# chrisquince/DESMAN

Hardware: AMD Instinct MI355X
Metric: Gibbs iterations/sec (VxS updates/s) at V=10k S=64 G=8 (higher is better)
Workload: dtype f64; 1 GPU; synthetic V=10000 x S=64, G=8, full Gibbs iteration, 1 chain per GPU (configs[2]); V=10000, S=64, G=8, chains=1, tau_rng=mt19937

## Files before the change

### desman_amd/_lib.py

```python
import ctypes as C
import os

import numpy as np

_HERE = os.path.dirname(os.path.abspath(__file__))
LIB_PATH = os.environ.get("DESMAN_HIP_LIB") or os.path.join(_HERE, "lib", "libdesman_hip.so")
AB_LIB_PATH = os.path.join(_HERE, "lib", "libdesman_hip_ab.so")
HEADER_PATH = os.path.join(os.path.dirname(_HERE), "include", "desman_hip.h")

DSM_OK = 0
RNG_MT19937, RNG_PHILOX = 0, 1
STATS_AGG = 2
K_NAMES = ("stats", "dirichlet", "tau", "finalize", "mt", "nmft_a", "nmft_gamma", "nmft_b", "stats2", "stats_big", "stats_pat")


class DesmanHipError(RuntimeError):
    pass


_i64p = np.ctypeslib.ndpointer(np.int64, flags="C_CONTIGUOUS")
_f64p = np.ctypeslib.ndpointer(np.float64, flags="C_CONTIGUOUS")
_u64p = np.ctypeslib.ndpointer(np.uint64, flags="C_CONTIGUOUS")
_u32p = np.ctypeslib.ndpointer(np.uint32, flags="C_CONTIGUOUS")
_i32p = np.ctypeslib.ndpointer(np.int32, flags="C_CONTIGUOUS")
_vp, _i, _d = C.c_void_p, C.c_int, C.c_double

SIGNATURES = {
    "dsm_last_error": (C.c_char_p, []),
    "dsm_device_count": (_i, []),
    "dsm_version": (C.c_char_p, []),
    "dsm_initRNG": (_i, []),
    "dsm_setRNG": (_i, [C.c_ulong]),
    "dsm_freeRNG": (_i, []),
    "dsm_sample_tau": (_i, [_i64p, _f64p, _f64p, _i64p, _i, _i, _i]),
    "c_initRNG": (None, []),
    "c_setRNG": (None, [C.c_ulong]),
    "c_freeRNG": (None, []),
    "c_sample_tau": (_i, [_i64p, _f64p, _f64p, _i64p, _i, _i, _i]),
    "dsm_getRNG_state": (_i, [_u32p]),
    "dsm_setRNG_state": (_i, [_u32p]),
    "dsm_ctx_create": (_i, [C.POINTER(_vp), _i]),
    "dsm_ctx_destroy": (_i, [_vp]),
    "dsm_ctx_sync": (_i, [_vp]),
    "dsm_ctx_set_counts": (_i, [_vp, _i64p, _i, _i]),
    "dsm_ctx_set_state": (_i, [_vp, _i64p, _f64p, _f64p, _i]),
    "dsm_ctx_get_state": (_i, [_vp, _vp, _vp, _vp]),
    "dsm_ctx_set_gamma_eta": (_i, [_vp, _vp, _vp]),
    "dsm_ctx_set_priors": (_i, [_vp, _d, _d, _d]),
    "dsm_ctx_seed": (_i, [_vp, C.c_ulong, C.c_uint64]),
    "dsm_ctx_set_tau_rng": (_i, [_vp, _i]),
    "dsm_ctx_get_mt_state": (_i, [_vp, _u32p]),
    "dsm_ctx_set_mt_state": (_i, [_vp, _u32p]),
    "dsm_mt_seed_state": (_i, [C.c_ulong, _u32p]),
    "dsm_ctx_debug_mt_fill": (_i, [_vp, C.c_size_t, _u32p]),
    "dsm_ctx_sample_tau": (_i, [_vp, C.POINTER(_i), _vp]),
    "dsm_ctx_sample_stats": (_i, [_vp, C.c_uint32, _u64p, _u64p]),
    "dsm_ctx_stats_spec": (_i, [_vp]),
    "dsm_ctx_sweep_stats": (_i, [_vp, C.POINTER(C.c_uint64), C.POINTER(C.c_uint64), _i]),
    "dsm_ctx_set_tau_screen": (_i, [_vp, _i]),
    "dsm_ctx_set_tau_neartie": (_i, [_vp, _i]),
    "dsm_ctx_set_nmft_fused": (_i, [_vp, _i]),
    "dsm_ctx_set_nmft_persist": (_i, [_vp, _i]),
    "dsm_ctx_tau_launch_info": (_i, [_vp, C.POINTER(_i), C.POINTER(_i)]),
    "dsm_ctx_debug_log2f": (_i, [_vp, _vp, _vp, C.c_size_t]),
    "dsm_debug_fdiv": (_i, [_i, _f64p, _f64p, _f64p, _i]),
    "dsm_release_device_caches": (_i, []),
    "dsm_ctx_force_stats_spec": (_i, [_vp, _i]),
    "dsm_ctx_debug_stage1": (_i, [_vp, C.c_uint32, _vp, _u64p]),
    "dsm_ctx_debug_binom": (_i, [_vp, _i, C.c_uint32, _f64p, C.c_uint64, _i, _u32p, _i]),
    "dsm_ctx_draw_gamma_eta": (_i, [_vp, C.c_uint32, _u64p, _u64p, _f64p, _f64p]),
    "dsm_ctx_loglik": (_i, [_vp, C.POINTER(_d), C.POINTER(_d)]),
    "dsm_ctx_gibbs_update": (_i, [_vp, _i]),
    "dsm_ctx_get_counters": (_i, [_vp, C.POINTER(C.c_uint64), C.POINTER(C.c_uint32)]),
    "dsm_ctx_set_counters": (_i, [_vp, C.c_uint64, C.c_uint32]),
    "dsm_ctx_get_screen_state": (_i, [_vp, _u32p]),
    "dsm_ctx_set_screen_state": (_i, [_vp, _u32p]),
    "dsm_ctx_gibbs_update_sharded": (_i, [_vp, _i, _i, _i, _vp, _vp]),
    "dsm_ctx_gibbs_update_sharded_comm": (_i, [_vp, _i, _i, _i, _vp]),
    "dsm_comm_unique_id": (_i, [_vp]),
    "dsm_comm_create": (_i, [C.POINTER(_vp), _vp, _i, _i, _i]),
    "dsm_comm_destroy": (_i, [_vp]),
    "dsm_comm_rank": (_i, [_vp]),
    "dsm_comm_world": (_i, [_vp]),
    "dsm_comm_allgather_f64": (_i, [_vp, _f64p, _f64p, C.c_size_t]),
    "dsm_comm_allreduce_f64": (_i, [_vp, _vp, C.c_size_t, _i]),
    "dsm_comm_barrier": (_i, [_vp]),
    "dsm_device_read": (_i, [_i, _vp, _vp, C.c_size_t]),
    "dsm_device_write": (_i, [_i, _vp, _vp, C.c_size_t]),
    "dsm_batch_gibbs_update": (_i, [C.POINTER(_vp), _i, _i]),
    "dsm_batch_update_tau": (_i, [C.POINTER(_vp), _i, _i, C.POINTER(_vp), C.POINTER(_vp)]),
    "dsm_batch_nmft_factorize": (_i, [C.POINTER(_vp), _i, _i, _d, _i, C.POINTER(_i), _vp]),
    "dsm_ctx_update_tau": (_i, [_vp, _i, _f64p, _f64p]),
    "dsm_ctx_get_trace": (_i, [_vp, _vp, _vp, _vp, _vp, _vp]),
    "dsm_ctx_get_star": (_i, [_vp, _vp, _vp, _vp, C.POINTER(_d), C.POINTER(_i)]),
    "dsm_ctx_get_tau_sum": (_i, [_vp, _i64p]),
    "dsm_ctx_get_tau_at": (_i, [_vp, _i, _i64p]),
    "dsm_nmft_set": (_i, [_vp, _f64p, _f64p, _i]),
    "dsm_nmft_get": (_i, [_vp, _vp, _vp]),
    "dsm_nmft_factorize": (_i, [_vp, _i, _d, _i, C.POINTER(_i), _vp]),
    "dsm_nmft_objective": (_i, [_vp, C.POINTER(_d)]),
    "dsm_nmft_debug_path": (_i, [_vp, _i, C.POINTER(_i)]),
    "dsm_nmft_get_tau": (_i, [_vp, _i64p]),
    "dsm_lrt_step": (_i, [_i, _f64p, _i32p, _i32p, _f64p, _d, _i, _i, _f64p, _f64p, _f64p]),
    "dsm_assign_tau": (_i, [_i, _i64p, _i, _i, _i, _f64p, _f64p, C.c_uint64, _vp, _vp, _vp, _vp, _vp]),
    "dsm_ctx_assign_tau": (_i, [_vp, _f64p, _f64p, _i, C.c_uint64, _vp, _vp, _vp, _vp, _vp]),
    "dsm_assign_debug_set_chunk": (_i, [_i]),
    "dsm_fit_gamma": (_i, [_i, _i64p, _i, _i, _i, _i64p, _f64p, _i, _d, _i, _vp, _vp, _vp, _vp, _vp, _vp]),
    "dsm_ctx_fit_gamma": (_i, [_vp, _i, _vp, _f64p, _i, _d, _i, _vp, _vp, _vp, _vp, _vp, _vp]),
    "dsm_abund_debug_set_chunk": (_i, [_i]),
    "dsm_fit_gamma_interval": (_i, [_i, _i64p, _i, _i, _i, _i64p, _f64p, _f64p, _d, _i, _d, _d, _vp, _vp, _vp]),
    "dsm_ctx_fit_gamma_interval": (_i, [_vp, _i, _vp, _f64p, _f64p, _d, _i, _d, _d, _vp, _vp, _vp]),
    "dsm_fit_gamma_eta": (_i, [_i, _i64p, _i, _i, _i, _i64p, _f64p, _i, _d, _vp, _vp, _vp, _vp, _vp, _vp, _vp, _vp, _vp]),
    "dsm_ctx_fit_gamma_eta": (_i, [_vp, _i, _vp, _f64p, _i, _d, _vp, _vp, _vp, _vp, _vp, _vp, _vp, _vp, _vp]),
    "dsm_abund_debug_set_eta_batch": (_i, [_i]),
    "dsm_abund_debug_set_eta_stage_max": (_i, [C.c_longlong]),
    "dsm_genes_create": (_i, [C.POINTER(_vp), _i]),
    "dsm_genes_destroy": (_i, [_vp]),
    "dsm_genes_set_data": (_i, [_vp, _vp, _i, _i, _i, _i32p, _f64p]),
    "dsm_genes_set_model": (_i, [_vp, _f64p, _f64p, _f64p, _i, _i, _f64p, _f64p, _f64p]),
    "dsm_genes_set_state": (_i, [_vp, _vp, _vp]),
    "dsm_genes_get_state": (_i, [_vp, _vp, _vp]),
    "dsm_genes_seed": (_i, [_vp, C.c_ulong, C.c_uint64]),
    "dsm_genes_set_gene_base": (_i, [_vp, _i]),
    "dsm_genes_get_mt_state": (_i, [_vp, _u32p]),
    "dsm_genes_set_mt_state": (_i, [_vp, _u32p]),
    "dsm_genes_nmft_tau": (_i, [_vp, _vp, _f64p, _i, _d, _vp]),
    "dsm_genes_sweep_all": (_i, [_vp, _vp, _i, _vp, _vp, _vp]),
    "dsm_genes_step_candidates": (_i, [_vp, _i, _i, _f64p, _vp]),
    "dsm_genes_step_choose": (_i, [_vp, _i, _i, _i]),
    "dsm_genes_update": (_i, [_vp, _i, _i, _vp, _vp, _vp, _vp]),
    "dsm_genes_loglik": (_i, [_vp, _vp]),
    "dsm_genes_get_star": (_i, [_vp, _vp, _vp]),
    "dsm_genes_set_star": (_i, [_vp, _vp, _vp]),
    "dsm_genes_debug_tile": (_i, [_vp, C.POINTER(_i), C.POINTER(_i), C.POINTER(_i), C.POINTER(C.c_size_t)]),
    "dsm_kl_assign": (_i, [_i, _f64p, _f64p, _f64p, _i, _i, _i, _i, _d, C.POINTER(_i), C.POINTER(_d)]),
    "dsm_ctx_set_timing": (_i, [_vp, _i]),
    "dsm_ctx_get_timing": (_i, [_vp, _vp, _vp]),
    "dsm_kernel_name": (C.c_char_p, [_i]),
}

EXCHANGE_FN = C.CFUNCTYPE(C.c_int, C.c_void_p, C.c_void_p, C.c_size_t, C.c_void_p, C.c_size_t)
_lib = None


def _digest(a):
    try:
        import xxhash
        return xxhash.xxh3_128_digest(memoryview(a).cast("B"))
    except ImportError:
        import hashlib
        return hashlib.blake2b(memoryview(a).cast("B"), digest_size=16).digest()


def load():
    global _lib
    if _lib is None:
        if not os.path.exists(LIB_PATH):
            raise DesmanHipError(
                "libdesman_hip.so not built (%s); run `python -c 'import __graft_entry__ as g; g.build()'` "
                "or `make -C desman_amd/csrc`.  There is no CPU fallback." % LIB_PATH)
        try:
            lib = C.CDLL(LIB_PATH)
        except OSError as e:
            raise DesmanHipError("cannot load %s: %s" % (LIB_PATH, e))
        for name, (res, args) in SIGNATURES.items():
            fn = getattr(lib, name)
            fn.restype = res
            fn.argtypes = args
        _lib = lib
    return _lib


def check(rc):
    if rc != DSM_OK:
        raise DesmanHipError("libdesman_hip: error %d: %s" % (rc, load().dsm_last_error().decode()))
    return rc


def mt_seed_state(seed):
    st = np.empty(625, dtype=np.uint32)
    check(load().dsm_mt_seed_state(int(seed) & 0xFFFFFFFFFFFFFFFF, st))
    return st


def release_device_caches():
    check(load().dsm_release_device_caches())


def debug_fdiv(kind, a, b):
    a = np.ascontiguousarray(a, dtype=np.float64).reshape(-1)
    b = np.ascontiguousarray(b, dtype=np.float64).reshape(-1)
    out = np.empty_like(a)
    check(load().dsm_debug_fdiv(int(kind), a, b, out, a.size))
    return out


def lrt_step(ffreq, maxA, maxB, eta, upperP, optimise, p, device=0):
    ffreq = np.ascontiguousarray(ffreq, dtype=np.float64)
    V = ffreq.shape[0]
    p = np.ascontiguousarray(p, dtype=np.float64).copy()
    MLL = np.empty(V); BLL = np.empty(V)
    check(load().dsm_lrt_step(int(device), ffreq, np.ascontiguousarray(maxA, dtype=np.int32),
                              np.ascontiguousarray(maxB, dtype=np.int32), np.ascontiguousarray(eta, dtype=np.float64),
                              float(upperP), int(bool(optimise)), V, p, MLL, BLL))
    return p, MLL, BLL


def device_count():
    return load().dsm_device_count()


ASSIGN_MAX_G = 10


def _assign_model(gamma, eta, S):
    gamma = np.ascontiguousarray(gamma, dtype=np.float64)
    eta = np.ascontiguousarray(eta, dtype=np.float64)
    if gamma.ndim != 2 or gamma.shape[0] != S or eta.shape != (4, 4):
        raise ValueError("assign_tau: gamma must be [S=%d, G] and eta [4, 4]; got %s, %s" % (S, gamma.shape, eta.shape))
    return gamma, eta
# ... 187 lines not shown
        self.G = gamma.shape[1]

    def get_state(self):
        tau = np.empty((self.V, self.G, 4), dtype=np.int64)
        gamma = np.empty((self.S, self.G))
        eta = np.empty((4, 4))
        check(self.lib.dsm_ctx_get_state(self._h, _ptr(tau), _ptr(gamma), _ptr(eta)))
        return tau, gamma, eta

    def set_gamma_eta(self, gamma=None, eta=None):
        g = None if gamma is None else np.ascontiguousarray(gamma, dtype=np.float64)
        e = None if eta is None else np.ascontiguousarray(eta, dtype=np.float64)
        check(self.lib.dsm_ctx_set_gamma_eta(self._h, _ptr(g), _ptr(e)))

    def set_priors(self, alpha=0.1, delta=0.1, epsilon=1e-6):
        check(self.lib.dsm_ctx_set_priors(self._h, alpha, delta, epsilon))

    def seed(self, mt_seed, ctr_seed=None):
        if ctr_seed is None:
            ctr_seed = (int(mt_seed) * 0x9E3779B97F4A7C15 + 0x243F6A8885A308D3) & 0xFFFFFFFFFFFFFFFF
        check(self.lib.dsm_ctx_seed(self._h, int(mt_seed) & 0xFFFFFFFFFFFFFFFF, int(ctr_seed)))

    def get_mt_state(self):
        st = np.empty(625, dtype=np.uint32)
        check(self.lib.dsm_ctx_get_mt_state(self._h, st))
        return st

    def checkpoint(self):
        tau, gamma, eta = self.get_state()
        key, it = self.counters()
        try:
            mt = self.get_mt_state()
        except DesmanHipError:
            mt = np.zeros(0, dtype=np.uint32)
        return dict(tau=tau, gamma=gamma, eta=eta, mt_state=mt, ctr_seed=np.uint64(key), iter_ctr=np.uint32(it), screen=self.screen_state())

    def counters(self):
        key, it = C.c_uint64(0), C.c_uint32(0)
        check(self.lib.dsm_ctx_get_counters(self._h, C.byref(key), C.byref(it)))
        return int(key.value), int(it.value)

    def screen_state(self):
        out = np.zeros(2, dtype=np.uint32)
        check(self.lib.dsm_ctx_get_screen_state(self._h, out))
        return out

    def set_screen_state(self, words):
        check(self.lib.dsm_ctx_set_screen_state(self._h, np.ascontiguousarray(words, dtype=np.uint32)))

    def restore(self, ck):
        self.set_state(np.ascontiguousarray(ck["tau"], dtype=np.int64), np.ascontiguousarray(ck["gamma"], dtype=np.float64),
                       np.ascontiguousarray(ck["eta"], dtype=np.float64))
        mt = np.asarray(ck["mt_state"], dtype=np.uint32)
        if mt.size == 625:
            self.set_mt_state(np.ascontiguousarray(mt))
        check(self.lib.dsm_ctx_set_counters(self._h, int(ck["ctr_seed"]), int(ck["iter_ctr"])))
        self.set_screen_state(ck["screen"] if "screen" in ck else np.zeros(2, dtype=np.uint32))

    def set_mt_state(self, st):
        check(self.lib.dsm_ctx_set_mt_state(self._h, np.ascontiguousarray(st, dtype=np.uint32)))

    def debug_mt_fill(self, n):
        out = np.empty(int(n), dtype=np.uint32)
        check(self.lib.dsm_ctx_debug_mt_fill(self._h, int(n), out))
        return out

    def set_tau_rng(self, mode):
        check(self.lib.dsm_ctx_set_tau_rng(self._h, int(mode)))

    def assign_tau(self, gamma, eta, seed=None):
        gamma, eta = _assign_model(gamma, eta, self.S)
        G = gamma.shape[1]
        out = _assign_out(self.V, G, seed)
        check(self.lib.dsm_ctx_assign_tau(self._h, gamma, eta, G, int(seed or 0) & 0xFFFFFFFFFFFFFFFF, _ptr(out["map_state"]),
                                          _ptr(out["conf"]), _ptr(out["logz"]), _ptr(out["marg"]), _ptr(out.get("draw_state"))))
        return out

    def fit_gamma(self, eta, tau=None, max_iter=FIT_MAX_ITER, tol=FIT_TOL, presence=False):
        eta = _fit_eta(eta)
        t = None if tau is None else _fit_tau(tau, self.V)
        G = self.G if t is None else t.shape[1]
        out = _fit_out(self.S, G, presence)
        check(self.lib.dsm_ctx_fit_gamma(self._h, G, _ptr(t), eta, int(max_iter), float(tol), int(bool(presence)), _ptr(out["gamma"]),
                                         _ptr(out["loglik"]), _ptr(out["deviance"]), _ptr(out["iters"]), _ptr(out["converged"]),
                                         _ptr(out.get("lr_absent"))))
        return out

    def fit_gamma_eta(self, eta0, tau=None, max_iter=FIT_MAX_ITER, tol=FIT_TOL):
        eta0 = _fit_eta(eta0)
        t = None if tau is None else _fit_tau(tau, self.V)
        G = self.G if t is None else t.shape[1]
        out, scal, ptrs = _fit_eta_out(self.S, G)
        check(self.lib.dsm_ctx_fit_gamma_eta(self._h, G, _ptr(t), eta0, int(max_iter), float(tol), *ptrs))
        return _fit_eta_result(out, scal)

    def fit_gamma_interval(self, eta, gamma_hat, tau=None, level=0.95, q=None, max_iter=FIT_MAX_ITER, tol=FIT_TOL, ctol=FIT_CTOL):
        eta = _fit_eta(eta)
        t = None if tau is None else _fit_tau(tau, self.V)
        G = self.G if t is None else t.shape[1]
        g, q, out = _interval_args(gamma_hat, self.S, G, level, q)
        check(self.lib.dsm_ctx_fit_gamma_interval(self._h, G, _ptr(t), eta, g, q, int(max_iter), float(tol), float(ctol), _ptr(out["lo"]),
                                                  _ptr(out["hi"]), _ptr(out["flags"])))
        return out

    def sample_tau(self, want_logp=False):
        n = _i(0)
        logp = np.empty((self.V, self.G, 4)) if want_logp else None
        check(self.lib.dsm_ctx_sample_tau(self._h, C.byref(n), _ptr(logp)))
        return (n.value, logp) if want_logp else n.value

    def sample_stats(self, it):
        mu = np.zeros((self.S, self.G), dtype=np.uint64)
        E = np.zeros((4, 4), dtype=np.uint64)
        check(self.lib.dsm_ctx_sample_stats(self._h, int(it), mu, E))
        return mu, E

    def debug_log2f(self, x):
        x = np.ascontiguousarray(x, dtype=np.float32)
        out = np.empty_like(x)
        check(self.lib.dsm_ctx_debug_log2f(self._h, x.ctypes.data, out.ctypes.data, x.size))
        return out

    def set_tau_neartie(self, mode=-1):
        check(self.lib.dsm_ctx_set_tau_neartie(self._h, int(mode)))

    def set_tau_screen(self, on):
        check(self.lib.dsm_ctx_set_tau_screen(self._h, 1 if on else 0))

    def tau_launch_info(self):
        a, b = _i(0), _i(0)
        check(self.lib.dsm_ctx_tau_launch_info(self._h, C.byref(a), C.byref(b)))
        return a.value, b.value

    def set_nmft_persist(self, mode=-1):
        check(self.lib.dsm_ctx_set_nmft_persist(self._h, int(mode)))

    def set_nmft_fused(self, mode=-1):
        check(self.lib.dsm_ctx_set_nmft_fused(self._h, int(mode)))

    def sweep_stats(self, reset=False):
        a, b = C.c_uint64(0), C.c_uint64(0)
        check(self.lib.dsm_ctx_sweep_stats(self._h, C.byref(a), C.byref(b), 1 if reset else 0))
        return a.value, b.value

    def stats_spec(self):
        r = self.lib.dsm_ctx_stats_spec(self._h)
        if r < 0:
            check(r)
        return r

    def force_stats_spec(self, spec=0):
        check(self.lib.dsm_ctx_force_stats_spec(self._h, int(spec)))

    def debug_stage1(self, it):
        nt = np.zeros((self.S, 1 << self.G), dtype=np.uint32)
        E = np.zeros((4, 4), dtype=np.uint64)
        check(self.lib.dsm_ctx_debug_stage1(self._h, int(it), nt.ctypes.data, E))
        return nt, E

    def debug_binom(self, kind, n, w, seed, nsamp, spec=STATS_AGG):
        w4 = np.zeros(4)
        w4[:len(w)] = w
        out = np.zeros((nsamp, 4) if kind == 2 else nsamp, dtype=np.uint32)
        check(self.lib.dsm_ctx_debug_binom(self._h, int(kind), int(n), w4, int(seed), int(nsamp), out.reshape(-1), int(spec)))
        return out

    def draw_gamma_eta(self, it, sum_mu, esum):
        g = np.empty((self.S, self.G)); e = np.empty((4, 4))
        check(self.lib.dsm_ctx_draw_gamma_eta(self._h, int(it), np.ascontiguousarray(sum_mu, dtype=np.uint64),
                                              np.ascontiguousarray(esum, dtype=np.uint64), g, e))
        return g, e

    def loglik(self):
        ll, lp = _d(0), _d(0)
        check(self.lib.dsm_ctx_loglik(self._h, C.byref(ll), C.byref(lp)))
        return ll.value, lp.value

    def gibbs_update(self, n_iter):
        check(self.lib.dsm_ctx_gibbs_update(self._h, int(n_iter)))
        self.n_trace = int(n_iter)

    def gibbs_update_sharded(self, n_iter, v_offset, v_total, exchange):
        err = []

        def cb(user, tab, n_tab, vec, n_vec):
            try:
                exchange(tab or 0, int(n_tab), vec, int(n_vec))
                return 0
            except BaseException as e:
                err.append(e)
                return 1
        fn = EXCHANGE_FN(cb)
        rc = self.lib.dsm_ctx_gibbs_update_sharded(self._h, int(n_iter), int(v_offset), int(v_total), C.cast(fn, _vp), None)
        if err:
            raise err[0]
        check(rc)
        self.n_trace = int(n_iter)

    def gibbs_update_sharded_comm(self, n_iter, v_offset, v_total, comm):
        check(self.lib.dsm_ctx_gibbs_update_sharded_comm(self._h, int(n_iter), int(v_offset), int(v_total), comm._h))
        self.n_trace = int(n_iter)

    @staticmethod
    def batch_gibbs_update(ctxs, n_iter):
        ctxs = list(ctxs)
        arr = (_vp * len(ctxs))(*[c._h.value for c in ctxs])
        check(load().dsm_batch_gibbs_update(arr, len(ctxs), int(n_iter)))
        for c in ctxs:
            c.n_trace = int(n_iter)

    def update_tau(self, gamma_store, eta_store):
        g = np.ascontiguousarray(gamma_store, dtype=np.float64)
        e = np.ascontiguousarray(eta_store, dtype=np.float64)
        check(self.lib.dsm_ctx_update_tau(self._h, g.shape[0], g, e))
        self.n_trace = g.shape[0]

    def get_trace(self):
        n = self.n_trace
        ll = np.empty(n); lp = np.empty(n); nch = np.empty(n, dtype=np.int32)
        g = np.empty((n, self.S, self.G)); e = np.empty((n, 4, 4))
        check(self.lib.dsm_ctx_get_trace(self._h, _ptr(ll), _ptr(lp), _ptr(nch), _ptr(g), _ptr(e)))
        return dict(ll=ll, lp=lp, nchange=nch, gamma=g, eta=e)

    def get_star(self):
        tau = np.empty((self.V, self.G, 4), dtype=np.int64)
        g = np.empty((self.S, self.G)); e = np.empty((4, 4))
        lp, it = _d(0), _i(0)
        check(self.lib.dsm_ctx_get_star(self._h, _ptr(tau), _ptr(g), _ptr(e), C.byref(lp), C.byref(it)))
        return dict(tau=tau, gamma=g, eta=e, lp=lp.value, it=it.value)

    def get_tau_sum(self):
        out = np.empty((self.V, self.G, 4), dtype=np.int64)
        check(self.lib.dsm_ctx_get_tau_sum(self._h, out))
        return out

    def get_tau_at(self, it):
        out = np.empty((self.V, self.G, 4), dtype=np.int64)
        check(self.lib.dsm_ctx_get_tau_at(self._h, int(it), out))
        return out

    def nmft_set(self, tau, gamma):
        tau = np.ascontiguousarray(tau, dtype=np.float64)
        gamma = np.ascontiguousarray(gamma, dtype=np.float64)
        G = gamma.shape[0]
        if tau.shape != (4 * self.V, G) or gamma.shape[1] != self.S:
            raise ValueError("NMFT factor shapes do not match the count tensor")
        check(self.lib.dsm_nmft_set(self._h, tau, gamma, G))
        self.nG = G

    def nmft_get(self):
        tau = np.empty((4 * self.V, self.nG)); gamma = np.empty((self.nG, self.S))
        check(self.lib.dsm_nmft_get(self._h, _ptr(tau), _ptr(gamma)))
        return tau, gamma

    def nmft_factorize(self, max_iter=5000, min_change=1e-5, fix_gamma=False):
        n = _i(0)
        tr = np.full(max_iter + 1, np.nan)
        check(self.lib.dsm_nmft_factorize(self._h, int(max_iter), float(min_change), int(bool(fix_gamma)),
                                          C.byref(n), _ptr(tr)))
        return n.value, tr[: n.value + 1]

    @staticmethod
    def batch_update_tau(ctxs, gamma_stores, eta_stores):
        ctxs = list(ctxs)
        gs = [np.ascontiguousarray(g, dtype=np.float64) for g in gamma_stores]
        es = [np.ascontiguousarray(e, dtype=np.float64) for e in eta_stores]
        n = gs[0].shape[0]
        if any(g.shape[0] != n for g in gs) or any(e.shape[0] != n for e in es):
            raise ValueError("batch_update_tau: traces of equal length expected")
        arr = (_vp * len(ctxs))(*[c._h.value for c in ctxs])
        gp = (_vp * len(ctxs))(*[g.ctypes.data for g in gs])
        ep = (_vp * len(ctxs))(*[e.ctypes.data for e in es])
        check(load().dsm_batch_update_tau(arr, len(ctxs), int(n), gp, ep))
        for c in ctxs:
            c.n_trace = int(n)

    @staticmethod
    def batch_nmft_factorize(ctxs, max_iter=5000, min_change=1e-5, fix_gamma=False):
        ctxs = list(ctxs)
        arr = (_vp * len(ctxs))(*[c._h.value for c in ctxs])
        n = (_i * len(ctxs))()
        tr = np.full((len(ctxs), max_iter + 1), np.nan)
        check(load().dsm_batch_nmft_factorize(arr, len(ctxs), int(max_iter), float(min_change), int(bool(fix_gamma)), n,
                                              tr.ctypes.data_as(_vp)))
        return [(int(n[k]), tr[k, : n[k] + 1].copy()) for k in range(len(ctxs))]

    def nmft_objective(self):
        d = _d(0)
        check(self.lib.dsm_nmft_objective(self._h, C.byref(d)))
        return d.value

    def nmft_debug_path(self, fix_gamma=False):
        out = (_i * 8)()
        check(self.lib.dsm_nmft_debug_path(self._h, int(bool(fix_gamma)), out))
        fam, nt, kb, ncb, nwv, grid, lds, flags = (int(x) for x in out)
        return {"family": ("two-pass", "mfma", "split", "persist")[fam], "NT": nt, "KB": kb, "NCB": ncb, "NWV": nwv, "grid": grid,
                "lds": lds, "xpar": bool(flags & 1), "gstep": bool(flags & 2), "VT": (flags >> 8) & 255, "cus": flags >> 16}

    def nmft_get_tau(self):
        out = np.empty((self.V, self.nG, 4), dtype=np.int64)
        check(self.lib.dsm_nmft_get_tau(self._h, out))
        return out

    def set_timing(self, on):
        check(self.lib.dsm_ctx_set_timing(self._h, int(bool(on))))

# ... 134 lines not shown
```

### desman_amd/csrc/api.hip

```cpp
#include <math.h>
#include <stdarg.h>
#include <stdio.h>
#include <string.h>

#include <algorithm>
#include <mutex>
#include <numeric>
#include <thread>

#include "dsm_host.h"
#include "log_table.h"

static thread_local char g_err[512] = "";

void dsm_set_error(const char *fmt, ...)
{
    va_list ap;
    va_start(ap, fmt);
    vsnprintf(g_err, sizeof g_err, fmt, ap);
    va_end(ap);
}

extern "C" const char *dsm_last_error(void) { return g_err; }
extern "C" const char *dsm_version(void) { return "desman_hip 0.1 (gfx950)"; }
// ... 42 lines not shown
        c->k_ms[s.k] += ms;
        c->free_events.push_back(s.e0);
        c->free_events.push_back(s.e1);
    }
    c->spans.clear();
    return DSM_OK;
}

extern "C" int dsm_ctx_set_timing(dsm_ctx *c, int on)
{
    if (!c) return DSM_ERR_ARG;
    int r = collect_spans(c);
    c->timing = on != 0;
    for (int k = 0; k < DSM_K_COUNT; ++k) { c->k_ms[k] = 0; c->k_launches[k] = 0; }
    return r;
}

extern "C" int dsm_ctx_get_timing(dsm_ctx *c, double *ms_total, int64_t *launches)
{
    if (!c) return DSM_ERR_ARG;
    int r = collect_spans(c);
    if (r) return r;
    for (int k = 0; k < DSM_K_COUNT; ++k) {
        if (ms_total) ms_total[k] = c->k_ms[k];
        if (launches) launches[k] = c->k_launches[k];
    }
    return DSM_OK;
}

template <typename T>
static int dev_alloc(T **p, size_t n)
{
    if (*p) { (void)hipFree(*p); *p = nullptr; }
    if (n == 0) n = 1;
    hipError_t e = hipMalloc((void **)p, n * sizeof(T));
    if (e != hipSuccess) { dsm_set_error("hipMalloc(%zu B) failed: %s", n * sizeof(T), hipGetErrorString(e)); return DSM_ERR_NOMEM; }
    return DSM_OK;
}
template <typename T>
static void dev_free(T **p) { if (*p) { (void)hipFree(*p); *p = nullptr; } }

template <typename T>
struct Scratch {
    T *p = nullptr;
    ~Scratch() { if (p) (void)hipFree(p); }
    int alloc(size_t n) { return dev_alloc(&p, n); }
    operator T *() const { return p; }
    Scratch() = default;
    Scratch(const Scratch &) = delete;
    Scratch &operator=(const Scratch &) = delete;
};

#define TRY(x) do { int _r = (x); if (_r != DSM_OK) return _r; } while (0)
#define BIND(c) HIP_TRY(hipSetDevice((c)->device))

static int need(dsm_ctx *c, bool counts, bool state)
{
    if (!c) { dsm_set_error("null context"); return DSM_ERR_ARG; }
    if (counts && !c->cnt_vs) { dsm_set_error("no count tensor: call dsm_ctx_set_counts first"); return DSM_ERR_STATE; }
    if (state && !c->have_state) { dsm_set_error("no chain state: call dsm_ctx_set_state first"); return DSM_ERR_STATE; }
    return DSM_OK;
}

static int esum_reset(dsm_ctx *c)
{
    HIP_TRY(hipMemsetAsync(c->esum, 0, (16 + 16 * DSM_ESUM_PARTS) * sizeof(unsigned long long), c->stream));
    return DSM_OK;
}

static int reset_blk_order(dsm_ctx *c)
{
    static const std::vector<uint32_t> ident = [] { std::vector<uint32_t> v((size_t)2 * DSM_MAX_GRID); for (size_t i = 0; i < v.size(); ++i) v[i] = (uint32_t)(i % DSM_MAX_GRID); return v; }();
    c->blk_order_n[0] = c->blk_order_n[1] = 0;
    if (!c->blk_order) return DSM_OK;
    HIP_TRY(hipMemcpyAsync(c->blk_order, ident.data(), ident.size() * sizeof(uint32_t), hipMemcpyHostToDevice, c->stream));
    return DSM_OK;
}

extern "C" int dsm_ctx_create(dsm_ctx **out, int device)
{
    if (!out) return DSM_ERR_ARG;
    *out = nullptr;
    int n = dsm_device_count();
    if (n <= 0) { dsm_set_error("no HIP device visible"); return DSM_ERR_NODEVICE; }
    if (device < 0 || device >= n) { dsm_set_error("device %d out of range (0..%d)", device, n - 1); return DSM_ERR_ARG; }
    HIP_TRY(hipSetDevice(device));
    hipDeviceProp_t prop;
    HIP_TRY(hipGetDeviceProperties(&prop, device));
    if (strncmp(prop.gcnArchName, "gfx950", 6) != 0) {
        dsm_set_error("device %d is %s; this library is built for gfx950 only", device, prop.gcnArchName);
        return DSM_ERR_NODEVICE;
    }
    dsm_ctx *c = new dsm_ctx();
    c->device = device;
    HIP_TRY(hipStreamCreateWithFlags(&c->stream, hipStreamNonBlocking));
    if (getenv("DESMAN_HIP_ONE_STREAM")) c->stream_rng = c->stream;
    else {
        int lo = 0, hi = 0;
        HIP_TRY(hipDeviceGetStreamPriorityRange(&lo, &hi));
        HIP_TRY(hipStreamCreateWithPriority(&c->stream_rng, hipStreamNonBlocking, hi));
    }
    for (int i = 0; i < 2; ++i) {
        HIP_TRY(hipEventCreateWithFlags(&c->ev_u_ready[i], hipEventDisableTiming));
        HIP_TRY(hipEventCreateWithFlags(&c->ev_u_free[i], hipEventDisableTiming));
    }
    TRY(dev_alloc(&c->mt_state, 625));
    TRY(dev_alloc(&c->ll_partial, 2 * DSM_MAX_GRID));
    TRY(dev_alloc(&c->nchange, 2));
    TRY(dev_alloc(&c->sweep_stats, 2));
    HIP_TRY(hipMemsetAsync(c->sweep_stats, 0, 2 * sizeof(unsigned long long), c->stream));
    TRY(dev_alloc(&c->step_cnt, (size_t)2 * 2 * DSM_MAX_GRID));
    HIP_TRY(hipMemsetAsync(c->step_cnt, 0, (size_t)2 * 2 * DSM_MAX_GRID * sizeof(uint32_t), c->stream));
    TRY(dev_alloc(&c->blk_order, (size_t)2 * DSM_MAX_GRID));
    TRY(reset_blk_order(c));
    TRY(dev_alloc(&c->screen_ctl, 4));
    HIP_TRY(hipMemsetAsync(c->screen_ctl, 0, 4 * sizeof(uint32_t), c->stream));
    TRY(dev_alloc(&c->prior, 2 * (DSM_MAX_S + 4)));
    TRY(dev_alloc(&c->scalars, 8));
    TRY(dev_alloc(&c->star, 2));
    TRY(dev_alloc(&c->eta, 16));
    TRY(dev_alloc(&c->eta_new, 16));
    TRY(dev_alloc(&c->eta_star, 16));
    TRY(dev_alloc(&c->esum, 16 + 16 * DSM_ESUM_PARTS));
    TRY(dev_alloc(&c->log_tab, 2 * DSM_LOG_TAB_N + DSM_EXP_TAB_N));
    HIP_TRY(hipMemcpyAsync(c->log_tab, dsm_log_table_host, sizeof dsm_log_table_host, hipMemcpyHostToDevice, c->stream));
    HIP_TRY(hipMemcpyAsync(c->log_tab + 2 * DSM_LOG_TAB_N, dsm_exp_table_host, sizeof dsm_exp_table_host, hipMemcpyHostToDevice, c->stream));
    HIP_TRY(hipMemsetAsync(c->nchange, 0, 2 * sizeof(int), c->stream));
    TRY(esum_reset(c));
    HIP_TRY(hipStreamSynchronize(c->stream));
    *out = c;
    return DSM_OK;
}

static void free_traces(dsm_ctx *c)
{
    dev_free(&c->tau_trace); dev_free(&c->ll_trace); dev_free(&c->lp_trace); dev_free(&c->nchange_trace);
    dev_free(&c->gamma_trace); dev_free(&c->eta_trace); dev_free(&c->gamma_in); dev_free(&c->eta_in);
    c->in_cap = 0;
    c->n_trace = 0;
    c->trace_cap = 0;
}

extern "C" int dsm_ctx_destroy(dsm_ctx *c)
{
    if (!c) return DSM_OK;
    (void)hipSetDevice(c->device);
    (void)hipStreamSynchronize(c->stream);
    collect_spans(c);
    for (auto e : c->free_events) (void)hipEventDestroy(e);
    free_traces(c);
    dev_free(&c->cnt_vs); dev_free(&c->items); dev_free(&c->nitems); dev_free(&c->tau);
    dev_free(&c->pat_rep); dev_free(&c->pat_x); dev_free(&c->pat_list); c->pat_rep_len = c->pat_x_len = 0;
    if (c->h_rare) { (void)hipHostFree(c->h_rare); c->h_rare = nullptr; }
    dev_free(&c->s2_scratch);
    dev_free(&c->blk_tab); stats_release_ntab(c); dev_free(&c->big_list); dev_free(&c->big_count);
    dev_free(&c->gamma); dev_free(&c->eta);
    dev_free(&c->eta_new); dev_free(&c->sum_mu); dev_free(&c->esum); dev_free(&c->mt_state); dev_free(&c->mt_jstates); dev_free(&c->u_raw);
    dev_free(&c->ll_partial); dev_free(&c->nchange); dev_free(&c->sweep_stats); dev_free(&c->step_cnt); dev_free(&c->blk_order); dev_free(&c->screen_ctl); dev_free(&c->prior); dev_free(&c->prior_all); dev_free(&c->scalars); dev_free(&c->star);
    dev_free(&c->gamma_star); dev_free(&c->eta_star); dev_free(&c->log_tab); dev_free(&c->shard_vec); dev_free(&c->np_part); if (c->np_bar) { (void)hipFree(c->np_bar); c->np_bar = nullptr; } dev_free(&c->F); dev_free(&c->ntau); dev_free(&c->ntau2); dev_free(&c->ngam); dev_free(&c->ngam_raw);
    dev_free(&c->npart); dev_free(&c->nstat); dev_free(&c->ngam2); dev_free(&c->ngam_raw2);
    for (int i = 0; i < 2; ++i) { (void)hipEventDestroy(c->ev_u_ready[i]); (void)hipEventDestroy(c->ev_u_free[i]); }
    if (c->stream_rng != c->stream) (void)hipStreamDestroy(c->stream_rng);
    (void)hipStreamDestroy(c->stream);
    delete c;
    return DSM_OK;
}

extern "C" int dsm_ctx_sync(dsm_ctx *c)
{
    if (!c) return DSM_ERR_ARG;
    BIND(c);
    HIP_TRY(hipStreamSynchronize(c->stream));
    HIP_TRY(hipStreamSynchronize(c->stream_rng));
    return DSM_OK;
}

extern "C" int dsm_ctx_set_counts(dsm_ctx *c, const int64_t *variants, int V, int S)
{
    if (!c || !variants || V < 1 || S < 1) { dsm_set_error("set_counts: bad arguments"); return DSM_ERR_ARG; }
    if (S > DSM_MAX_S) { dsm_set_error("S=%d exceeds DSM_MAX_S=%d", S, DSM_MAX_S); return DSM_ERR_UNSUPPORTED; }
    if ((int64_t)V * S >= ((int64_t)1 << 32)) { dsm_set_error("V*S must be below 2^32"); return DSM_ERR_UNSUPPORTED; }
    BIND(c);
    HIP_TRY(hipStreamSynchronize(c->stream));
    HIP_TRY(hipStreamSynchronize(c->stream_rng));
    const size_t n = (size_t)V * S;
    c->V = V; c->S = S;
    c->have_state = false;
    c->G = 0;
    TRY(dev_alloc(&c->cnt_vs, n * 4));
    TRY(dev_alloc(&c->nitems, (size_t)S));
    TRY(dev_alloc(&c->tau, (size_t)V));
    dev_free(&c->F); dev_free(&c->ntau); dev_free(&c->ntau2); dev_free(&c->ngam); dev_free(&c->ngam_raw); c->nG = 0;
    free_traces(c);
    Scratch<int64_t> d_in; Scratch<int> d_flag; Scratch<double> d_part; Scratch<unsigned long long> d_depth;
    const int nblk = (int)((n + 255) / 256 < 1024 ? (n + 255) / 256 : 1024);
    TRY(d_in.alloc(n * 4));
    TRY(d_flag.alloc(1));
    TRY(d_part.alloc((size_t)nblk));
    TRY(d_depth.alloc((size_t)S));
    HIP_TRY(hipMemcpyAsync(d_in, variants, n * 4 * sizeof(int64_t), hipMemcpyHostToDevice, c->stream));
    HIP_TRY(hipMemsetAsync(d_flag, 0, sizeof(int), c->stream));
    HIP_TRY(hipMemsetAsync(d_depth, 0, (size_t)S * sizeof(unsigned long long), c->stream));
    TRY(k_convert_counts(c, d_in, d_flag, d_part, nblk, d_depth));
    std::vector<double> part(nblk);
    std::vector<unsigned long long> dep((size_t)S);
    int flag = 0;
    HIP_TRY(hipMemcpyAsync(part.data(), d_part, nblk * sizeof(double), hipMemcpyDeviceToHost, c->stream));
    HIP_TRY(hipMemcpyAsync(dep.data(), d_depth, (size_t)S * sizeof(unsigned long long), hipMemcpyDeviceToHost, c->stream));
    HIP_TRY(hipMemcpyAsync(&flag, d_flag, sizeof(int), hipMemcpyDeviceToHost, c->stream));
    HIP_TRY(hipStreamSynchronize(c->stream));
    c->items_built = false;
    c->max_items = 0;
    c->blk_gmax = 0;
    c->stats_grid = 0;
    dev_free(&c->pat_x); c->pat_x_len = 0;
    TRY(reset_blk_order(c));
    HIP_TRY(hipMemsetAsync(c->screen_ctl, 0, 4 * sizeof(uint32_t), c->stream));
    dev_free(&c->items);
    c->depth.assign((size_t)S, 0);
    c->max_depth = 0;
    for (int s = 0; s < S; ++s) { c->depth[s] = (int64_t)dep[s]; c->max_depth = std::max<uint64_t>(c->max_depth, dep[s]); }
    if (flag) {
        dev_free(&c->cnt_vs); dev_free(&c->items);
        dsm_set_error("set_counts: negative count or depth above 2^31-1");
        return DSM_ERR_ARG;
    }
    double s = 0.0;
    for (double p : part) s += p;
    c->ll_const = s;
    return DSM_OK;
}

int build_stats_items(dsm_ctx *c)
{
    const int V = c->V, S = c->S;
    std::vector<int32_t> cnt((size_t)V * S * 4);
    HIP_TRY(hipMemcpyAsync(cnt.data(), c->cnt_vs, cnt.size() * sizeof(int32_t), hipMemcpyDeviceToHost, c->stream));
    HIP_TRY(hipStreamSynchronize(c->stream));
    const int64_t cells = (int64_t)V * S;
    const int CH = cells <= 65536 ? 64 : cells <= 262144 ? 128 : 0;
    c->chunked = CH != 0;
    std::vector<int32_t> nit(S);
    std::vector<std::vector<std::pair<int32_t, int32_t>>> lst((size_t)S);
    std::vector<int32_t> top(S, 0);
    for (int s = 0; s < S; ++s) lst[s].reserve((size_t)V * 2);
    for (int v = 0; v < V; ++v) {
        const int32_t *row = cnt.data() + (size_t)v * S * 4;
        for (int s = 0; s < S; ++s)
            for (int b = 0; b < 4; ++b) {
                const int64_t x = row[s * 4 + b];
                if (x <= 0) continue;
                if (!CH) {
                    lst[s].emplace_back((int32_t)x, v * 4 + b);
                    if (x > top[s]) top[s] = (int32_t)x;
                } else {
                    for (int64_t j = 0; j * CH < x; ++j) {
                        const int32_t nrd = (int32_t)(x - j * CH < CH ? x - j * CH : CH);
                        lst[s].emplace_back(nrd | (int32_t)(j << 12), v * 4 + b);
                        if (nrd > top[s]) top[s] = nrd;
                    }
                }
            }
    }
    int max_items = 0;
    for (int s = 0; s < S; ++s) max_items = std::max(max_items, (int)lst[s].size());
    c->item_stride = max_items > 0 ? max_items : 1;
    std::vector<int32_t> items((size_t)S * c->item_stride * 2, 0);
    TRY(dev_alloc(&c->items, items.size()));
    std::vector<int32_t> first;
    const int32_t rd_mask = CH ? 0xfff : 0x7fffffff;
    for (int s = 0; s < S; ++s) {
        const auto &l = lst[s];
        nit[s] = (int32_t)l.size();
        int32_t *dst = items.data() + (size_t)s * c->item_stride * 2;
        if (top[s] <= (1 << 20)) {
            first.assign((size_t)top[s] + 2, 0);
            for (const auto &e : l) first[e.first & rd_mask]++;
            int32_t run = 0;
            for (int32_t cval = top[s]; cval >= 1; --cval) { const int32_t h = first[cval]; first[cval] = run; run += h; }
            for (const auto &e : l) { const int32_t k = first[e.first & rd_mask]++; dst[2 * k] = e.second; dst[2 * k + 1] = e.first; }
        } else {
            std::vector<std::pair<int32_t, int32_t>> t(l);
            std::stable_sort(t.begin(), t.end(), [](const std::pair<int32_t, int32_t> &p, const std::pair<int32_t, int32_t> &q) { return p.first > q.first; });
            for (size_t k = 0; k < t.size(); ++k) { dst[2 * k] = t[k].second; dst[2 * k + 1] = t[k].first; }
        }
    }
    c->max_items = max_items;
    c->nitems_h = nit;
    c->blk_gmax = 0;
    HIP_TRY(hipMemcpyAsync(c->items, items.data(), items.size() * sizeof(int32_t), hipMemcpyHostToDevice, c->stream));
    HIP_TRY(hipMemcpyAsync(c->nitems, nit.data(), (size_t)S * sizeof(int32_t), hipMemcpyHostToDevice, c->stream));
    HIP_TRY(hipStreamSynchronize(c->stream));
    c->items_built = true;
    return DSM_OK;
}

static int ensure_state_buffers(dsm_ctx *c, int G)
{
    if (G < 1 || G > DSM_MAX_G) { dsm_set_error("G=%d outside 1..%d", G, DSM_MAX_G); return DSM_ERR_UNSUPPORTED; }
    if (G != c->G || !c->gamma) {
        c->G = G;
        const size_t sg = (size_t)c->S * G;
        TRY(dev_alloc(&c->gamma, sg));
        TRY(dev_alloc(&c->gamma_star, sg));
        TRY(dev_alloc(&c->sum_mu, sg));
        HIP_TRY(hipMemsetAsync(c->sum_mu, 0, sg * sizeof(unsigned long long), c->stream));
        c->stats_grid = 0;
        c->u_cap = (size_t)c->V * G;
        c->u_chunk_words = c->u_cap * std::max<size_t>(1, std::min<size_t>(DSM_U_CHUNK, ((size_t)16 << 20) / std::max<size_t>(1, c->u_cap)));
        TRY(dev_alloc(&c->u_raw, 2 * c->u_chunk_words));
        free_traces(c);
    }
    return DSM_OK;
}

extern "C" int dsm_ctx_set_state(dsm_ctx *c, const int64_t *tau, const double *gamma, const double *eta, int G)
{
    TRY(need(c, true, false));
    if (!tau || !gamma || !eta) { dsm_set_error("set_state: null pointer"); return DSM_ERR_ARG; }
    BIND(c);
    HIP_TRY(hipStreamSynchronize(c->stream));
    TRY(ensure_state_buffers(c, G));
    const size_t nt = (size_t)c->V * G * 4;
    Scratch<int64_t> d_t;
    TRY(d_t.alloc(nt));
    HIP_TRY(hipMemcpyAsync(d_t, tau, nt * sizeof(int64_t), hipMemcpyHostToDevice, c->stream));
    TRY(k_pack_tau(c, d_t, c->tau, c->V, G));
    HIP_TRY(hipMemcpyAsync(c->gamma, gamma, (size_t)c->S * G * sizeof(double), hipMemcpyHostToDevice, c->stream));
    c->tau_rare_n = tau_rare_from_host(gamma, c->S, G);
    HIP_TRY(hipMemcpyAsync(c->eta, eta, 16 * sizeof(double), hipMemcpyHostToDevice, c->stream));
    HIP_TRY(hipStreamSynchronize(c->stream));
    c->have_state = true;
    return DSM_OK;
}

extern "C" int dsm_ctx_set_gamma_eta(dsm_ctx *c, const double *gamma, const double *eta)
{
    TRY(need(c, true, true));
    BIND(c);
    if (gamma) HIP_TRY(hipMemcpyAsync(c->gamma, gamma, (size_t)c->S * c->G * sizeof(double), hipMemcpyHostToDevice, c->stream));
    if (gamma) c->tau_rare_n = tau_rare_from_host(gamma, c->S, c->G);
    if (eta) HIP_TRY(hipMemcpyAsync(c->eta, eta, 16 * sizeof(double), hipMemcpyHostToDevice, c->stream));
    HIP_TRY(hipStreamSynchronize(c->stream));
    return DSM_OK;
}

static int fetch_tau(dsm_ctx *c, const uint64_t *d_packed, int64_t *host_onehot)
{
    const size_t nt = (size_t)c->V * c->G * 4;
    Scratch<int64_t> d_t;
    TRY(d_t.alloc(nt));
    TRY(k_unpack_tau(c, d_packed, d_t, c->V, c->G));
    HIP_TRY(hipMemcpyAsync(host_onehot, d_t, nt * sizeof(int64_t), hipMemcpyDeviceToHost, c->stream));
    HIP_TRY(hipStreamSynchronize(c->stream));
    return DSM_OK;
}

extern "C" int dsm_ctx_get_state(dsm_ctx *c, int64_t *tau, double *gamma, double *eta)
{
    TRY(need(c, true, true));
    BIND(c);
    if (tau) TRY(fetch_tau(c, c->tau, tau));
    if (gamma) HIP_TRY(hipMemcpyAsync(gamma, c->gamma, (size_t)c->S * c->G * sizeof(double), hipMemcpyDeviceToHost, c->stream));
    if (eta) HIP_TRY(hipMemcpyAsync(eta, c->eta, 16 * sizeof(double), hipMemcpyDeviceToHost, c->stream));
    HIP_TRY(hipStreamSynchronize(c->stream));
    return DSM_OK;
}

extern "C" int dsm_ctx_set_priors(dsm_ctx *c, double alpha, double delta, double epsilon)
{
    if (!c || !(alpha > 0) || !(delta > 0) || !(epsilon >= 0)) { dsm_set_error("set_priors: bad value"); return DSM_ERR_ARG; }
    c->alpha = alpha; c->delta = delta; c->epsilon = epsilon;
    return DSM_OK;
}

static void mt_seed_host(uint32_t *st, unsigned long seed)
{
    if (seed == 0) seed = 4357;
    st[0] = (uint32_t)(seed & 0xffffffffUL);
    for (int i = 1; i < 624; ++i) st[i] = 1812433253u * (st[i - 1] ^ (st[i - 1] >> 30)) + (uint32_t)i;
    st[624] = 624;
}

static int seed_mt(dsm_ctx *c, unsigned long seed)
{
    uint32_t st[625];
    mt_seed_host(st, seed);
    HIP_TRY(hipStreamSynchronize(c->stream_rng));
    HIP_TRY(hipMemcpyAsync(c->mt_state, st, sizeof st, hipMemcpyHostToDevice, c->stream));
    HIP_TRY(hipStreamSynchronize(c->stream));
    c->mt_seeded = true;
    return DSM_OK;
}

extern "C" int dsm_ctx_seed(dsm_ctx *c, unsigned long mt_seed, uint64_t ctr_seed)
{
    if (!c) return DSM_ERR_ARG;
    BIND(c);
    c->ctr_seed = ctr_seed;
    c->iter_ctr = 0;
    return seed_mt(c, mt_seed);
}

extern "C" int dsm_ctx_get_screen_state(dsm_ctx *c, uint32_t *out2)
{
    if (!c || !out2) { dsm_set_error("get_screen_state: null argument"); return DSM_ERR_ARG; }
    BIND(c);
    HIP_TRY(hipMemcpyAsync(out2, c->screen_ctl, 2 * sizeof(uint32_t), hipMemcpyDeviceToHost, c->stream));
    HIP_TRY(hipStreamSynchronize(c->stream));
    return DSM_OK;
}
extern "C" int dsm_ctx_set_screen_state(dsm_ctx *c, const uint32_t *in2)
{
    if (!c || !in2) { dsm_set_error("set_screen_state: null argument"); return DSM_ERR_ARG; }
    BIND(c);
    HIP_TRY(hipStreamSynchronize(c->stream));
    HIP_TRY(hipMemcpy(c->screen_ctl, in2, 2 * sizeof(uint32_t), hipMemcpyHostToDevice));
    return DSM_OK;
}

extern "C" int dsm_ctx_get_counters(dsm_ctx *c, uint64_t *ctr_seed, uint32_t *iter_ctr)
{
    if (!c || !ctr_seed || !iter_ctr) { dsm_set_error("get_counters: null argument"); return DSM_ERR_ARG; }
    *ctr_seed = c->ctr_seed; *iter_ctr = c->iter_ctr;
    return DSM_OK;
}
extern "C" int dsm_ctx_set_counters(dsm_ctx *c, uint64_t ctr_seed, uint32_t iter_ctr)
{
    if (!c) { dsm_set_error("set_counters: null context"); return DSM_ERR_ARG; }
    c->ctr_seed = ctr_seed; c->iter_ctr = iter_ctr;
    return DSM_OK;
}

extern "C" int dsm_mt_seed_state(unsigned long seed, uint32_t *state625)
{
    if (!state625) return DSM_ERR_ARG;
    mt_seed_host(state625, seed);
    return DSM_OK;
}

extern "C" int dsm_ctx_get_mt_state(dsm_ctx *c, uint32_t *state625)
{
    if (!c || !state625) return DSM_ERR_ARG;
    if (!c->mt_seeded) { dsm_set_error("tau RNG not seeded"); return DSM_ERR_STATE; }
    BIND(c);
    HIP_TRY(hipStreamSynchronize(c->stream_rng));
    HIP_TRY(hipMemcpyAsync(state625, c->mt_state, 625 * sizeof(uint32_t), hipMemcpyDeviceToHost, c->stream));
    HIP_TRY(hipStreamSynchronize(c->stream));
    return DSM_OK;
}

extern "C" int dsm_ctx_set_mt_state(dsm_ctx *c, const uint32_t *state625)
{
    if (!c || !state625 || state625[624] > 624) { dsm_set_error("set_mt_state: bad state"); return DSM_ERR_ARG; }
    BIND(c);
    HIP_TRY(hipStreamSynchronize(c->stream_rng));
    HIP_TRY(hipMemcpyAsync(c->mt_state, state625, 625 * sizeof(uint32_t), hipMemcpyHostToDevice, c->stream));
    HIP_TRY(hipStreamSynchronize(c->stream));
    c->mt_seeded = true;
    return DSM_OK;
}

extern "C" int dsm_ctx_debug_mt_fill(dsm_ctx *c, size_t n, uint32_t *out)
{
    if (!c || (!out && n)) { dsm_set_error("debug_mt_fill: bad arguments"); return DSM_ERR_ARG; }
    if (!c->mt_seeded) { dsm_set_error("tau RNG not seeded"); return DSM_ERR_STATE; }
    if (n == 0) return DSM_OK;
    BIND(c);
    Scratch<uint32_t> d;
    TRY(d.alloc(n));
    HIP_TRY(hipStreamSynchronize(c->stream_rng));
    TRY(k_mt_fill(c, d, n, c->stream));
    HIP_TRY(hipMemcpyAsync(out, d, n * sizeof(uint32_t), hipMemcpyDeviceToHost, c->stream));
    HIP_TRY(hipStreamSynchronize(c->stream));
    return DSM_OK;
}

extern "C" int dsm_ctx_set_tau_rng(dsm_ctx *c, int mode)
{
    if (!c || (mode != DSM_RNG_MT19937 && mode != DSM_RNG_PHILOX)) { dsm_set_error("bad rng mode"); return DSM_ERR_ARG; }
    c->tau_rng = mode;
    return DSM_OK;
}

struct SweepWords {
    dsm_ctx *c;
    int total, filled = 0, nchunk = 0;
    int first[2] = {0, 0}, len[2] = {0, 0};
    int max_len = 1;
    SweepWords(dsm_ctx *ctx, int n_sweeps) : c(ctx), total(n_sweeps)
    {
        const size_t per = std::max<size_t>(1, c->u_cap);
        max_len = (int)std::max<size_t>(1, std::min<size_t>(DSM_U_CHUNK, c->u_chunk_words / per));
    }
    bool active() const { return c->tau_rng == DSM_RNG_MT19937; }
    int fill_next()
    {
        static const int grow[] = {1, 2, 3, 4, 6, 8};
        int want = grow[std::min(nchunk, 5)];
        want = std::min(std::min(want, max_len), total - filled);
        const int slot = nchunk & 1;
        uint32_t *buf = c->u_raw + (size_t)slot * c->u_chunk_words;
        HIP_TRY(hipStreamWaitEvent(c->stream_rng, c->ev_u_free[slot], 0));
        TRY(k_mt_fill(c, buf, (size_t)want * c->u_cap, c->stream_rng));
        HIP_TRY(hipEventRecord(c->ev_u_ready[slot], c->stream_rng));
        first[slot] = filled; len[slot] = want;
        filled += want; ++nchunk;
        return DSM_OK;
    }
    int prefetch()
    {
        if (!active() || filled > 0 || total < 1) return DSM_OK;
        if (!c->mt_seeded) { dsm_set_error("tau RNG not seeded: call dsm_ctx_seed / dsm_setRNG"); return DSM_ERR_STATE; }
        return fill_next();
    }
    int acquire(int it, const uint32_t **u)
    {
        *u = nullptr;
        if (!active()) return DSM_OK;
        if (!c->mt_seeded) { dsm_set_error("tau RNG not seeded: call dsm_ctx_seed / dsm_setRNG"); return DSM_ERR_STATE; }
        if (it >= filled) TRY(fill_next());
        int slot = (it >= first[0] && it < first[0] + len[0] && len[0]) ? 0 : 1;
        if (!(it >= first[slot] && it < first[slot] + len[slot])) { dsm_set_error("sweep words asked out of order"); return DSM_ERR_STATE; }
        if (it == first[slot]) {
            if (filled < total) TRY(fill_next());
            HIP_TRY(hipStreamWaitEvent(c->stream, c->ev_u_ready[slot], 0));
        }
        *u = c->u_raw + (size_t)slot * c->u_chunk_words + (size_t)(it - first[slot]) * c->u_cap;
        return DSM_OK;
    }
    int release(int it)
    {
        if (!active()) return DSM_OK;
        for (int slot = 0; slot < 2; ++slot)
            if (len[slot] && it == first[slot] + len[slot] - 1) HIP_TRY(hipEventRecord(c->ev_u_free[slot], c->stream));
        return DSM_OK;
    }
};

extern "C" int dsm_ctx_sample_tau(dsm_ctx *c, int *nchange, double *logp_out)
{
    TRY(need(c, true, true));
    BIND(c);
    Scratch<double> d_logp;
    const size_t nl = (size_t)c->V * c->G * 4;
    if (logp_out) TRY(d_logp.alloc(nl));
    const uint32_t *u = nullptr;
    SweepWords words(c, 1);
    HIP_TRY(hipMemsetAsync(c->nchange, 0, sizeof(int), c->stream));
    TRY(words.acquire(0, &u));
    TRY(k_tau_sweep(c, 1, c->gamma, c->eta, c->eta, nullptr, d_logp, c->iter_ctr++, nullptr, u));
    TRY(words.release(0));
    int n = 0;
    HIP_TRY(hipMemcpyAsync(&n, c->nchange, sizeof(int), hipMemcpyDeviceToHost, c->stream));
    if (logp_out) HIP_TRY(hipMemcpyAsync(logp_out, d_logp, nl * sizeof(double), hipMemcpyDeviceToHost, c->stream));
    HIP_TRY(hipMemsetAsync(c->nchange, 0, sizeof(int), c->stream));
    HIP_TRY(hipStreamSynchronize(c->stream));
    if (nchange) *nchange = n;
    return DSM_OK;
}

extern "C" int dsm_ctx_sample_stats(dsm_ctx *c, uint32_t iter, uint64_t *sum_mu, uint64_t *esum)
{
    TRY(need(c, true, true));
    BIND(c);
    const size_t sg = (size_t)c->S * c->G;
    HIP_TRY(hipMemsetAsync(c->sum_mu, 0, sg * sizeof(unsigned long long), c->stream));
    TRY(stats_ensure_ntab(c));
    TRY(esum_reset(c));
    TRY(k_stats(c, iter));
    TRY(k_esum_fold(c));
    if (sum_mu) HIP_TRY(hipMemcpyAsync(sum_mu, c->sum_mu, sg * sizeof(uint64_t), hipMemcpyDeviceToHost, c->stream));
    if (esum) HIP_TRY(hipMemcpyAsync(esum, c->esum, 16 * sizeof(uint64_t), hipMemcpyDeviceToHost, c->stream));
    HIP_TRY(hipMemsetAsync(c->sum_mu, 0, sg * sizeof(unsigned long long), c->stream));
    TRY(esum_reset(c));
    HIP_TRY(hipStreamSynchronize(c->stream));
    return DSM_OK;
}

extern "C" int dsm_ctx_stats_spec(dsm_ctx *c)
{
    if (!c || c->G < 1) { dsm_set_error("stats_spec: no chain state"); return DSM_ERR_STATE; }
    return stats_spec(c);
}

extern "C" int dsm_ctx_force_stats_spec(dsm_ctx *c, int spec)
{
    if (!c || spec < 0 || spec > 4) { dsm_set_error("force_stats_spec: 0 (rule), 1, 2, 3 or 4"); return DSM_ERR_ARG; }
    c->force_stats_spec = spec;
    return DSM_OK;
}

extern "C" int dsm_ctx_debug_stage1(dsm_ctx *c, uint32_t iter, uint32_t *ntab, uint64_t *esum)
{
    TRY(need(c, true, true));
    if (stats_spec(c) < 2) { dsm_set_error("debug_stage1: the aggregated specification does not apply to this shape (force it with dsm_ctx_force_stats_spec)"); return DSM_ERR_UNSUPPORTED; }
    BIND(c);
    TRY(esum_reset(c));
    TRY(k_stats_stage1(c, iter));
    TRY(k_esum_fold(c));
    const size_t NH = (size_t)1 << c->G, S = (size_t)c->S;
    const size_t ld = (size_t)c->ntab_ld;
    std::vector<uint32_t> t((size_t)c->ntab_rep * NH * ld);
    HIP_TRY(hipMemcpyAsync(t.data(), c->ntab, t.size() * sizeof(uint32_t), hipMemcpyDeviceToHost, c->stream));
    if (esum) HIP_TRY(hipMemcpyAsync(esum, c->esum, 16 * sizeof(uint64_t), hipMemcpyDeviceToHost, c->stream));
    HIP_TRY(hipMemsetAsync(c->ntab, 0, t.size() * sizeof(uint32_t), c->stream));
    TRY(esum_reset(c));
    HIP_TRY(hipMemsetAsync(c->big_count, 0, DSM_BIG_NT * DSM_BIG_NL * DSM_BIG_STRIDE * sizeof(uint32_t), c->stream));
    HIP_TRY(hipStreamSynchronize(c->stream));
    if (ntab)
        for (size_t h = 0; h < NH; ++h)
            for (size_t s = 0; s < S; ++s) {
                uint32_t v = 0;
                for (int r = 0; r < c->ntab_rep; ++r) v += t[((size_t)r * NH + ((h * DSM_NTAB_HMUL + (s >> 4) * DSM_NTAB_SWZ) & (NH - 1))) * ld + s];
                ntab[s * NH + h] = v;
            }
    return DSM_OK;
}

extern "C" int dsm_ctx_debug_binom(dsm_ctx *c, int kind, uint32_t n, const double *w4, uint64_t seed, int nsamp, uint32_t *out, int spec)
{
    if (!c || !w4 || !out || nsamp < 1 || kind < 0 || kind > 2 || spec < 2 || spec > 3) { dsm_set_error("debug_binom: bad arguments"); return DSM_ERR_ARG; }
    BIND(c);
    const size_t len = (size_t)nsamp * (kind == 2 ? 4 : 1);
    Scratch<uint32_t> d;
    TRY(d.alloc(len));
    TRY(k_binom_test(c, kind, n, w4, seed, nsamp, d, spec));
    HIP_TRY(hipMemcpyAsync(out, d, len * sizeof(uint32_t), hipMemcpyDeviceToHost, c->stream));
    HIP_TRY(hipStreamSynchronize(c->stream));
    return DSM_OK;
}

extern "C" int dsm_ctx_draw_gamma_eta(dsm_ctx *c, uint32_t iter, const uint64_t *sum_mu, const uint64_t *esum,
                                      double *gamma_out, double *eta_out)
{
    TRY(need(c, true, true));
    if (!sum_mu || !esum) { dsm_set_error("draw_gamma_eta: null sums"); return DSM_ERR_ARG; }
    BIND(c);
    const size_t sg = (size_t)c->S * c->G;
    Scratch<double> d_g, d_e;
    TRY(d_g.alloc(sg));
    TRY(d_e.alloc(16));
    HIP_TRY(hipMemcpyAsync(c->sum_mu, sum_mu, sg * sizeof(uint64_t), hipMemcpyHostToDevice, c->stream));
    HIP_TRY(hipMemcpyAsync(c->esum, esum, 16 * sizeof(uint64_t), hipMemcpyHostToDevice, c->stream));
    TRY(k_dirichlet(c, iter, d_g, nullptr, d_e, nullptr, c->prior, -1, 0, nullptr));
    if (gamma_out) HIP_TRY(hipMemcpyAsync(gamma_out, d_g, sg * sizeof(double), hipMemcpyDeviceToHost, c->stream));
    if (eta_out) HIP_TRY(hipMemcpyAsync(eta_out, d_e, 16 * sizeof(double), hipMemcpyDeviceToHost, c->stream));
    HIP_TRY(hipStreamSynchronize(c->stream));
    return DSM_OK;
}

static int eval_state(dsm_ctx *c, const double *gamma, const double *eta, uint64_t *trace_slot, int star_mode)
{
    int nb = 0;
    TRY(k_prior(c, gamma, eta, c->prior));
    TRY(k_tau_sweep(c, 2, gamma, eta, eta, trace_slot, nullptr, 0, &nb, nullptr));
    return k_finalize(c, nb, -1, star_mode, c->prior, gamma, eta);
}

extern "C" int dsm_ctx_loglik(dsm_ctx *c, double *ll, double *lp)
{
    TRY(need(c, true, true));
    BIND(c);
    double sc[2];
    TRY(eval_state(c, c->gamma, c->eta, nullptr, 2));
    HIP_TRY(hipMemcpyAsync(sc, c->scalars, sizeof sc, hipMemcpyDeviceToHost, c->stream));
    HIP_TRY(hipStreamSynchronize(c->stream));
    if (ll) *ll = sc[0];
    if (lp) *lp = sc[1];
    return DSM_OK;
}

static int alloc_traces(dsm_ctx *c, int n)
{
    const size_t sg = (size_t)c->S * c->G;
    if (n > c->trace_cap || !c->tau_trace) {
        free_traces(c);
        const int want = n;
        if (n < 512 && (size_t)513 * c->V * sizeof(uint64_t) <= ((size_t)1 << 30)) n = 512;
        TRY(dev_alloc(&c->tau_trace, (size_t)(n + 1) * c->V));
        TRY(dev_alloc(&c->ll_trace, (size_t)n));
        TRY(dev_alloc(&c->lp_trace, (size_t)n));
        TRY(dev_alloc(&c->nchange_trace, (size_t)n));
        TRY(dev_alloc(&c->gamma_trace, (size_t)n * sg));
        TRY(dev_alloc(&c->eta_trace, (size_t)n * 16));
        c->trace_cap = n;
        n = want;
    }
    c->n_trace = n;
    return DSM_OK;
}

thread_local BatchCtl g_batch;

struct Chains {
    dsm_ctx *const *c;
    int K;
    bool batched;
    struct Home { hipStream_t stream, stream_rng; bool timing; int nmft_fused; };
    std::vector<Home> home;
    dsm_ctx *lead() const { return c[0]; }
    ~Chains()
    {
        if (home.empty()) return;
        (void)hipStreamSynchronize(lead()->stream);
        (void)hipStreamSynchronize(lead()->stream_rng);
        for (size_t k = 0; k < home.size(); ++k) {
            c[k]->stream = home[k].stream; c[k]->stream_rng = home[k].stream_rng; c[k]->timing = home[k].timing; c[k]->nmft_fused = home[k].nmft_fused;
        }
    }
    template <class Fits> int open(bool state, bool nmft, Fits fits)
    {
        if (!c || K < 1 || K > DSM_MAX_BATCH) { dsm_set_error("batch of %d chains (1..%d)", K, DSM_MAX_BATCH); return DSM_ERR_ARG; }
        for (int k = 0; k < K; ++k) {
            TRY(need(c[k], true, state));
            const dsm_ctx *a = c[0], *b = c[k];
            if (b->device != a->device || b->V != a->V || b->S != a->S) { dsm_set_error("batch: chain %d differs from chain 0 in device or shape", k); return DSM_ERR_ARG; }
            TRY(fits(a, b, k));
            for (int j = 0; j < k; ++j) if (c[j] == b) { dsm_set_error("batch: chain %d listed twice", k); return DSM_ERR_ARG; }
        }
        BIND(lead());
        for (int k = 0; batched && k < K; ++k) {
            HIP_TRY(hipStreamSynchronize(c[k]->stream));
            HIP_TRY(hipStreamSynchronize(c[k]->stream_rng));
            home.push_back(Home{c[k]->stream, c[k]->stream_rng, c[k]->timing, c[k]->nmft_fused});
            c[k]->stream = lead()->stream; c[k]->stream_rng = lead()->stream_rng; c[k]->timing = false;
            if (nmft) c[k]->nmft_fused = home[0].nmft_fused;
        }
        return DSM_OK;
    }
    template <class F> int each(F f) const
    {
        for (int k = 0; k < K; ++k) TRY(f(c[k], k));
        return DSM_OK;
    }
    template <class F> int launch(F f) const
    {
        int r = DSM_OK;
        for (int k = 0; k < K && r == DSM_OK; ++k) {
            if (batched) g_batch = BatchCtl{K, k};
            r = f(c[k], k);
        }
        g_batch = BatchCtl{};
        return r;
    }
};

static int same_G_and_rng(const dsm_ctx *a, const dsm_ctx *b, int k)
{
    if (b->G != a->G || b->tau_rng != a->tau_rng) { dsm_set_error("batch: chain %d differs from chain 0 in shape or tau RNG", k); return DSM_ERR_ARG; }
    return DSM_OK;
}

static double *prior_slot(dsm_ctx *c, int it) { return c->prior + (it & 1) * (DSM_MAX_S + 4); }

static int gibbs_update(dsm_ctx *const *ctxs, int K, bool batched, int n_iter)
{
    if (n_iter < 0) { dsm_set_error("n_iter < 0"); return DSM_ERR_ARG; }
    Chains ch{ctxs, K, batched};
    TRY(ch.open(true, false, [](const dsm_ctx *a, const dsm_ctx *b, int k) -> int {
        TRY(same_G_and_rng(a, b, k));
        if (stats_spec(b) == stats_spec(a)) return DSM_OK;
        dsm_set_error("batch: chain %d runs mu/E specification %d, chain 0 specification %d (different tables or different dsm_ctx_force_stats_spec)", k, stats_spec(b), stats_spec(a));
        return DSM_ERR_ARG;
    }));
    dsm_ctx *const lead = ch.lead();
    const int spec = stats_spec(lead);
    const bool agg = spec >= 2;
    const bool fuse_s2 = agg && lead->G < 10;
    const size_t sg = (size_t)lead->S * lead->G;
    std::vector<SweepWords> words;
    words.reserve(K);
    std::vector<int> nb_prev(K, 0);
    std::vector<uint32_t> ic(K);
    std::vector<const uint32_t *> u(K, nullptr);
    TRY(ch.each([&](dsm_ctx *c, int) -> int {
        TRY(alloc_traces(c, n_iter));
        HIP_TRY(hipMemsetAsync(c->nchange, 0, sizeof(int), c->stream));
        TRY(eval_state(c, c->gamma, c->eta, c->tau_trace, 1));
        TRY(stats_ensure_ntab(c));
        if (!batched) TRY(k_tau_neartie_hint(c));
        words.emplace_back(c, n_iter);
        return DSM_OK;
    }));
    TRY(ch.launch([&](dsm_ctx *, int k) { return words[k].prefetch(); }));
    for (int it = 0; it < n_iter; ++it) {
        if (!batched && it && (it & 63) == 0 && lead->tau_neartie_mode == -1) { TRY(k_tau_rare_count(lead, true)); TRY(k_tau_neartie_hint(lead)); }
        TRY(ch.launch([&](dsm_ctx *c, int k) { ic[k] = c->iter_ctr++; return agg ? k_stats_stage1(c, ic[k]) : k_stats_v1(c, ic[k]); }));
        if (agg && !fuse_s2) TRY(ch.launch([&](dsm_ctx *c, int k) { return k_stats_stage2(c, ic[k]); }));
        TRY(ch.launch([&](dsm_ctx *c, int k) {
            return k_dirichlet(c, ic[k], c->gamma, c->gamma_trace + (size_t)it * sg, c->eta_new, c->eta_trace + (size_t)it * 16,
                               prior_slot(c, it), it - 1, nb_prev[k], prior_slot(c, it - 1), fuse_s2 ? 1 : 0);
        }));
        TRY(ch.launch([&](dsm_ctx *, int k) { return words[k].acquire(it, &u[k]); }));
        TRY(ch.launch([&](dsm_ctx *c, int k) {
            return k_tau_sweep(c, 3, c->gamma, c->eta, c->eta_new, c->tau_trace + (size_t)(it + 1) * c->V, nullptr, ic[k], &nb_prev[k], u[k]);
        }));
        TRY(ch.each([&](dsm_ctx *c, int k) -> int {
            TRY(words[k].release(it));
            std::swap(c->eta, c->eta_new);
            return DSM_OK;
        }));
    }
    const bool want_rare = !batched && n_iter > 0 && lead->tau_neartie_mode == -1;
    if (want_rare && !lead->h_rare) HIP_TRY(hipHostMalloc((void **)&lead->h_rare, sizeof(int), hipHostMallocDefault));
    if (n_iter > 0)
        TRY(ch.each([&](dsm_ctx *c, int k) {
            return k_finalize(c, nb_prev[k], n_iter - 1, 0, prior_slot(c, n_iter - 1), c->gamma_trace + (size_t)(n_iter - 1) * sg,
                              c->eta_trace + (size_t)(n_iter - 1) * 16, 0, want_rare ? c->h_rare : nullptr);
        }));
    HIP_TRY(hipStreamSynchronize(lead->stream));
    if (want_rare) lead->tau_rare_n = *lead->h_rare;
    return DSM_OK;
}

extern "C" int dsm_ctx_gibbs_update(dsm_ctx *c, int n_iter) { return gibbs_update(&c, 1, false, n_iter); }

extern "C" int dsm_batch_gibbs_update(dsm_ctx *const *ctxs, int K, int n_iter) { return gibbs_update(ctxs, K, true, n_iter); }

struct dsm_comm;
int comm_enqueue_exchange(dsm_comm *m, uint32_t *tab, size_t n_tab, double *vec, size_t n_vec, hipStream_t stream);
int comm_device(const dsm_comm *m);

static int gibbs_update_sharded(dsm_ctx *c, int n_iter, int v_offset, int v_total, dsm_exchange_fn exchange, void *user, dsm_comm *comm)
{
    TRY(need(c, true, true));
    c->tau_neartie_on = false;
    if (n_iter < 0 || (!exchange && !comm) || v_offset < 0 || v_total < v_offset + c->V) { dsm_set_error("gibbs_update_sharded: bad arguments"); return DSM_ERR_ARG; }
    if (comm && comm_device(comm) != c->device) { dsm_set_error("gibbs_update_sharded: the communicator lives on device %d, the context on %d", comm_device(comm), c->device); return DSM_ERR_ARG; }
    if (c->tau_rng != DSM_RNG_PHILOX) { dsm_set_error("gibbs_update_sharded: needs counter-based tau uniforms (DSM_RNG_PHILOX)"); return DSM_ERR_STATE; }
    BIND(c);
    const int keep_force = c->force_stats_spec;
    if (c->force_stats_spec < 2) c->force_stats_spec = DSM_STATS_AGG;
    struct Guard { dsm_ctx *c; int f; ~Guard() { c->shard_on = false; c->force_stats_spec = f; } } guard{c, keep_force};
    if (stats_spec(c) < 2) { dsm_set_error("gibbs_update_sharded: the aggregated mu/E pass does not apply to this shape (G <= 16)"); return DSM_ERR_UNSUPPORTED; }
    if (!c->shard_vec) TRY(dev_alloc(&c->shard_vec, (size_t)18));
    c->shard_on = true; c->shard_voff = v_offset; c->shard_vtot = v_total;
    TRY(alloc_traces(c, n_iter));
    const size_t sg = (size_t)c->S * c->G;
    HIP_TRY(hipMemsetAsync(c->nchange, 0, sizeof(int), c->stream));
    TRY(esum_reset(c));
    auto swap_vec = [&](uint32_t *tab, size_t n_tab) -> int {
        if (comm) return comm_enqueue_exchange(comm, tab, n_tab, c->shard_vec, (size_t)18, c->stream);
        HIP_TRY(hipStreamSynchronize(c->stream));
        if (exchange(user, tab, n_tab, c->shard_vec, (size_t)18) != 0) { dsm_set_error("gibbs_update_sharded: the exchange callback failed"); return DSM_ERR_STATE; }
        return DSM_OK;
    };
    {
        int nb = 0;
        TRY(k_prior(c, c->gamma, c->eta, c->prior));
        TRY(k_tau_sweep(c, 2, c->gamma, c->eta, c->eta, c->tau_trace, nullptr, 0, &nb, nullptr));
        TRY(k_shard_pack(c, nb));
        TRY(swap_vec(nullptr, 0));
        TRY(k_finalize(c, nb, -1, 1, c->prior, c->gamma, c->eta));
        TRY(esum_reset(c));
    }
    TRY(stats_ensure_ntab(c));
    double *const P[2] = {c->prior, c->prior + (DSM_MAX_S + 4)};
    int nb_prev = 0;
    for (int it = 0; it < n_iter; ++it) {
        const uint32_t ic = c->iter_ctr++;
        const bool fuse_s2 = c->G < 10;
        TRY(k_stats_stage1(c, ic));
        TRY(k_shard_pack(c, nb_prev));
        TRY(swap_vec(c->ntab, c->ntab_len));
        TRY(k_shard_unpack(c));
        if (!fuse_s2) TRY(k_stats_stage2(c, ic));
        TRY(k_dirichlet(c, ic, c->gamma, c->gamma_trace + (size_t)it * sg, c->eta_new, c->eta_trace + (size_t)it * 16,
                        P[it & 1], it - 1, nb_prev, P[(it - 1) & 1], fuse_s2 ? 1 : 0));
        TRY(k_tau_sweep(c, 3, c->gamma, c->eta, c->eta_new, c->tau_trace + (size_t)(it + 1) * c->V, nullptr, ic, &nb_prev, nullptr));
        std::swap(c->eta, c->eta_new);
    }
    if (n_iter > 0) {
        TRY(k_shard_pack(c, nb_prev));
        TRY(swap_vec(nullptr, 0));
        TRY(k_finalize(c, nb_prev, n_iter - 1, 0, P[(n_iter - 1) & 1], c->gamma_trace + (size_t)(n_iter - 1) * sg,
                       c->eta_trace + (size_t)(n_iter - 1) * 16));
        TRY(esum_reset(c));
    }
    HIP_TRY(hipStreamSynchronize(c->stream));
    return DSM_OK;
}

extern "C" int dsm_ctx_gibbs_update_sharded(dsm_ctx *c, int n_iter, int v_offset, int v_total, dsm_exchange_fn exchange, void *user)
{
    if (!exchange) { dsm_set_error("gibbs_update_sharded: no exchange callback"); return DSM_ERR_ARG; }
    return gibbs_update_sharded(c, n_iter, v_offset, v_total, exchange, user, nullptr);
}

extern "C" int dsm_ctx_gibbs_update_sharded_comm(dsm_ctx *c, int n_iter, int v_offset, int v_total, dsm_comm *comm)
{
    if (!comm) { dsm_set_error("gibbs_update_sharded_comm: no communicator"); return DSM_ERR_ARG; }
    return gibbs_update_sharded(c, n_iter, v_offset, v_total, nullptr, nullptr, comm);
}

extern "C" int dsm_device_read(int device, const void *dev, void *host, size_t bytes)
{
    HIP_TRY(hipSetDevice(device));
    HIP_TRY(hipMemcpy(host, dev, bytes, hipMemcpyDeviceToHost));
    return DSM_OK;
}
extern "C" int dsm_device_write(int device, void *dev, const void *host, size_t bytes)
{
    HIP_TRY(hipSetDevice(device));
    HIP_TRY(hipMemcpy(dev, host, bytes, hipMemcpyHostToDevice));
    return DSM_OK;
}

static int tau_inputs(dsm_ctx *c, int n_iter, const double *gamma_store, const double *eta_store)
{
    const size_t sg = (size_t)c->S * c->G;
    if (n_iter > c->in_cap || !c->gamma_in) {
        TRY(dev_alloc(&c->gamma_in, (size_t)n_iter * sg));
        TRY(dev_alloc(&c->eta_in, (size_t)n_iter * 16));
        TRY(dev_alloc(&c->prior_all, (size_t)n_iter * (c->S + 4)));
        c->in_cap = n_iter;
    }
    HIP_TRY(hipMemcpyAsync(c->gamma_in, gamma_store, (size_t)n_iter * sg * sizeof(double), hipMemcpyHostToDevice, c->stream));
    HIP_TRY(hipMemcpyAsync(c->eta_in, eta_store, (size_t)n_iter * 16 * sizeof(double), hipMemcpyHostToDevice, c->stream));
    HIP_TRY(hipMemcpyAsync(c->gamma_trace, c->gamma_in, (size_t)n_iter * sg * sizeof(double), hipMemcpyDeviceToDevice, c->stream));
    HIP_TRY(hipMemcpyAsync(c->eta_trace, c->eta_in, (size_t)n_iter * 16 * sizeof(double), hipMemcpyDeviceToDevice, c->stream));
    HIP_TRY(hipMemsetAsync(c->nchange, 0, sizeof(int), c->stream));
    TRY(eval_state(c, c->gamma_in, c->eta_in, c->tau_trace, 1));
    TRY(k_prior_batch(c, c->gamma_in, c->eta_in, n_iter, c->prior_all));
    HIP_TRY(hipMemsetAsync(c->nchange, 0, 2 * sizeof(int), c->stream));
    return DSM_OK;
}

static int update_tau(dsm_ctx *const *ctxs, int K, bool batched, int n_iter, const double *const *gamma_stores, const double *const *eta_stores)
{
    if (n_iter < 1 || !gamma_stores || !eta_stores) { dsm_set_error("update_tau: bad arguments"); return DSM_ERR_ARG; }
    Chains ch{ctxs, K, batched};
    TRY(ch.open(true, false, [&](const dsm_ctx *a, const dsm_ctx *b, int k) {
        if (!gamma_stores[k] || !eta_stores[k]) { dsm_set_error("update_tau: bad arguments"); return DSM_ERR_ARG; }
        return same_G_and_rng(a, b, k);
    }));
    const size_t sg = (size_t)ch.lead()->S * ch.lead()->G;
    std::vector<SweepWords> words;
    words.reserve(K);
    TRY(ch.each([&](dsm_ctx *c, int) -> int { TRY(alloc_traces(c, n_iter)); words.emplace_back(c, n_iter); return DSM_OK; }));
    TRY(ch.launch([&](dsm_ctx *, int k) { return words[k].prefetch(); }));
    TRY(ch.each([&](dsm_ctx *c, int k) { return tau_inputs(c, n_iter, gamma_stores[k], eta_stores[k]); }));
    std::vector<int> nb_prev(K, 0);
    std::vector<const uint32_t *> u(K, nullptr);
    for (int it = 0; it < n_iter; ++it) {
// ... 495 lines not shown
```

### desman_amd/csrc/dsm_host.h

```cpp
#pragma once
#include <hip/hip_runtime.h>
#include <stdint.h>
#include <string>
#include <vector>

#include "../../include/desman_hip.h"

#define DSM_MAX_GRID 4096
#define DSM_ESUM_PARTS 64
#define DSM_BIG_NL 64
#define DSM_BIG_STRIDE 16
#define DSM_BIG_NT 3
#define DSM_U_CHUNK 8

#define DSM_STATS_AGG 2
#define DSM_MAX_BATCH 8

void dsm_set_error(const char *fmt, ...);

#ifdef DSM_AB_SWITCHES
#define DSM_AB_ENV(name) getenv(name)
#else
#define DSM_AB_ENV(name) ((const char *)nullptr)
#endif

struct BatchCtl { int K = 0, k = 0; };
extern thread_local BatchCtl g_batch;
template <class P> struct BatchArgs { P p[DSM_MAX_BATCH]; };
#define LAUNCH_OR_COLLECT(PT, P, NORMAL, BATCHED)                                          \
    do {                                                                                    \
        if (g_batch.K == 0) { NORMAL; }                                                     \
        else {                                                                              \
            static thread_local BatchArgs<PT> acc;                                          \
            acc.p[g_batch.k] = (P);                                                         \
            if (g_batch.k == g_batch.K - 1) { const int K = g_batch.K; (void)K; BATCHED; }  \
        }                                                                                   \
    } while (0)

#define HIP_TRY(expr)                                                                       \
    do {                                                                                    \
        hipError_t _e = (expr);                                                             \
        if (_e != hipSuccess) {                                                             \
            dsm_set_error("%s failed: %s (%s:%d)", #expr, hipGetErrorString(_e), __FILE__, \
                          __LINE__);                                                        \
            return DSM_ERR_HIP;                                                             \
        }                                                                                   \
    } while (0)

struct TimedSpan { int k; hipEvent_t e0, e1; };

struct dsm_ctx {
    int device = 0;
    hipStream_t stream = nullptr;
    hipStream_t stream_rng = nullptr;
    hipEvent_t ev_u_ready[2] = {nullptr, nullptr}, ev_u_free[2] = {nullptr, nullptr};
    int V = 0, S = 0, G = 0;
    int32_t *cnt_vs = nullptr;
    int32_t *items = nullptr;
    int32_t *nitems = nullptr;
    int max_items = 0;
    bool items_built = false;
    uint64_t max_depth = 0;
    int force_stats_spec = 0;
    uint32_t *ntab = nullptr;
    size_t ntab_len = 0;
    unsigned long long *pat_rep = nullptr;
    uint32_t *pat_x = nullptr;
    uint32_t *pat_list = nullptr;
    size_t pat_rep_len = 0, pat_x_len = 0;
    uint32_t pat_gen = 0;
    uint32_t *s2_scratch = nullptr;
    uint32_t *ntab_raw = nullptr;
    int ntab_ld = 0;
    int ntab_rep = 1;
    unsigned long long *big_list = nullptr;
    uint32_t *big_count = nullptr;
    size_t big_cap = 0;
    int stats_grid = 0;
    int stats_grid_key = -1;
    int item_stride = 1;
    bool chunked = false;
    int32_t *blk_tab = nullptr;
    int blk_n = 0, blk_gmax = 0;
    std::vector<int64_t> depth;
    std::vector<int32_t> nitems_h;
    double ll_const = 0.0;
    uint64_t *tau = nullptr;
    double *gamma = nullptr;
    double *eta = nullptr;
    double *eta_new = nullptr;
    bool have_state = false;
    double alpha = 0.1, delta = 0.1, epsilon = 1e-6;
    unsigned long long *sum_mu = nullptr;
    unsigned long long *esum = nullptr;
    uint32_t *mt_state = nullptr;
    uint32_t *mt_jstates = nullptr;
    bool mt_seeded = false;
    uint32_t *u_raw = nullptr;
    size_t u_cap = 0;
    size_t u_chunk_words = 0;
    bool mt_attr_set = false;
    uint64_t ctr_seed = 0x243F6A8885A308D3ull;
    uint32_t iter_ctr = 0;
    int tau_rng = DSM_RNG_MT19937;
    double *ll_partial = nullptr;
    int *nchange = nullptr;
    unsigned long long *sweep_stats = nullptr;
    uint32_t *blk_order = nullptr;
    int tau_resident = 0, tau_resident_key = -1;
    int blk_order_n[2] = {0, 0};
    uint32_t *step_cnt = nullptr;
    uint32_t *screen_ctl = nullptr;
    bool tau_screen = true;
    int tau_neartie_mode = -1;
    bool tau_neartie_on = false;
    int tau_rare_n = 0;
    int *h_rare = nullptr;
    double *prior_all = nullptr;
    double *prior = nullptr;
    double *scalars = nullptr;
    double *log_tab = nullptr;
    int n_trace = 0, trace_cap = 0;
    uint64_t *tau_trace = nullptr;
    double *ll_trace = nullptr, *lp_trace = nullptr;
    int *nchange_trace = nullptr;
    double *gamma_trace = nullptr;
    double *eta_trace = nullptr;
    double *gamma_in = nullptr, *eta_in = nullptr;
    int in_cap = 0;
    double *star = nullptr;
    double *gamma_star = nullptr;
    double *eta_star = nullptr;
    bool shard_on = false;
    int shard_voff = 0, shard_vtot = 0;
    double *shard_vec = nullptr;
    double *F = nullptr;
    double *ntau = nullptr;
    double *ntau2 = nullptr;
    double *ngam = nullptr;
    double *ngam_raw = nullptr;
    int npart_cols = 0;
    double *npart = nullptr;
    double *nstat = nullptr;
    double *ndiv_trace = nullptr;
    int nG = 0;
    int nmft_blocks = 0;
    int nmft_persist = -1;
    double *np_part = nullptr;
    size_t np_cap = 0;
    unsigned *np_bar = nullptr;
    int nmft_fix_gamma = 0;
    int nmft_fused = -1;
    double *ngam2 = nullptr, *ngam_raw2 = nullptr;
    int nmft_gstep = 0, nmft_gstep_parity = 0, nmft_gstep_max_iter = 0;
    double nmft_gstep_min_change = 0.0;
    bool timing = false;
    std::vector<TimedSpan> spans;
    std::vector<hipEvent_t> free_events;
    double k_ms[DSM_K_COUNT] = {0};
    int64_t k_launches[DSM_K_COUNT] = {0};
};

struct KTimer {
    dsm_ctx *c; int k; hipStream_t st; hipEvent_t e0 = nullptr, e1 = nullptr;
    KTimer(dsm_ctx *ctx, int kid, hipStream_t stream = nullptr);
    ~KTimer();
};

int k_convert_counts(dsm_ctx *c, const int64_t *d_in, int *d_flag, double *d_partial, int nblk, unsigned long long *d_depth);
int k_pack_tau(dsm_ctx *c, const int64_t *d_onehot, uint64_t *d_packed, int V, int G);
int k_unpack_tau(dsm_ctx *c, const uint64_t *d_packed, int64_t *d_onehot, int V, int G);
int k_tau_sum(dsm_ctx *c, const uint64_t *trace, int n, int64_t *d_sum);
int k_mt_fill(dsm_ctx *c, uint32_t *out, size_t n, hipStream_t stream);
int k_stats_v1(dsm_ctx *c, uint32_t iter);
int k_log2f_test(dsm_ctx *c, const float *d_in, float *d_out, size_t n);
int build_stats_items(dsm_ctx *c);

#define DSM_NTAB_HMUL 0x9E3779B1u
#define DSM_NTAB_SWZ 17u
int stats_ensure_ntab(dsm_ctx *c);
void stats_release_ntab(dsm_ctx *c);
void mt_jump_release();
int stats_ntab_rep(const dsm_ctx *c);
int stats_spec(const dsm_ctx *c);
static inline int stats_draw_version(int spec) { return spec == 4 ? 2 : spec; }
int k_tau_neartie_hint(dsm_ctx *c);
int k_tau_rare_count(dsm_ctx *c, bool wait);
int tau_rare_from_host(const double *gamma, int S, int G);
int k_stats(dsm_ctx *c, uint32_t iter);
int k_stats_stage1(dsm_ctx *c, uint32_t iter);
int k_stats_stage2(dsm_ctx *c, uint32_t iter);
int k_binom_test(dsm_ctx *c, int kind, uint32_t n, const double *w, uint64_t seed, int nsamp, uint32_t *d_out, int spec);
int k_esum_fold(dsm_ctx *c);
int k_dirichlet(dsm_ctx *c, uint32_t iter, double *gamma_out, double *gamma_trace, double *eta_out, double *eta_trace,
                double *prior_out, int fin_it, int fin_nblocks, const double *fin_prior, int do_s2 = 0);
int k_prior(dsm_ctx *c, const double *gamma, const double *eta, double *prior_out);
int k_prior_batch(dsm_ctx *c, const double *gamma, const double *eta, int n, double *prior_out);
struct TauFinalRider { int nblocks, it; const double *prior, *gamma_src, *eta_src; };
int k_tau_sweep(dsm_ctx *c, int mode, const double *gamma, const double *eta_sweep,
                const double *eta_ll, uint64_t *trace_slot, double *d_logp, uint32_t iter, int *nblocks,
                const uint32_t *u_raw, int slot = 0, const TauFinalRider *rider = nullptr);
int tau_launch_info(dsm_ctx *c, int *launched, int *resident);
int k_shard_pack(dsm_ctx *c, int nblocks);
int k_shard_unpack(dsm_ctx *c);
int k_finalize(dsm_ctx *c, int nblocks, int it, int star_mode, const double *prior, const double *gamma_src,
               const double *eta_src, int slot = 0, int *rare_out = nullptr);

int k_nmft_freq(dsm_ctx *c);
int k_nmft_clamp(dsm_ctx *c);
int k_nmft_pass_a(dsm_ctx *c);
int k_nmft_gamma(dsm_ctx *c, int max_iter, double min_change, int fix_gamma, int adjust, int parity);
int k_nmft_reduce(dsm_ctx *c);
bool nmft_gstep_applies(const dsm_ctx *c, int fix_gamma);
int k_nmft_pass_b(dsm_ctx *c, int adjust);
int k_nmft_get_tau(dsm_ctx *c, uint64_t *d_packed);
int nmft_grid(dsm_ctx *c);
bool nmft_use_wave(const dsm_ctx *c);
bool nmft_use_mfma(const dsm_ctx *c);
bool nmft_use_wide(const dsm_ctx *c);
int nmft_wide_grid(const dsm_ctx *c);
int nmft_mfma_grid(const dsm_ctx *c, bool fix = false);
int k_nmft_wave(dsm_ctx *c, int adjust, int do_update);
int k_nmft_persist(dsm_ctx *c, int max_iter, double min_change, int fix_gamma, int adjust, int *used);
int nmft_debug_path(const dsm_ctx *c, int fix_gamma, int out[8]);
```

### desman_amd/csrc/dsm_stage2.h

```cpp
#pragma once
#include "dsm_binom.h"
#include "log_table.h"

#define S2_MAX_NODES 32
#define S2_MAX_LEVELS 6
#define S2_TAB_ENTRIES 1024
struct S2Plan {
    int nlevels, tab_entries;
    int level_start[S2_MAX_LEVELS + 2];
    signed char lo[S2_MAX_NODES], hi[S2_MAX_NODES], child[S2_MAX_NODES];
    unsigned char idx[S2_MAX_NODES];
    short off[S2_MAX_NODES];
};

struct Stage2Params {
    uint32_t *ntab;
    int rep, ld;
    const double *gamma;
    unsigned long long *sum_mu;
    const double *log_tab;
    int S, G;
    uint32_t k0, k1, iter;
    uint32_t hmul, swz;
    uint32_t *big_count;
    int nsplit;
    uint32_t *scratch, *ticket;
};

S2Plan make_stage2_plan(int G);

#define S2_SMEM_BYTES (DSM_LOG_TAB_N * 16 + DSM_EXP_TAB_N * 8 + DSM_RCP_TAB_N * 8 + 32 * 8 + S2_TAB_ENTRIES * 4 + 32 * 4 + 5 * S2_MAX_NODES * 4)

#ifdef DSM_AB_SWITCHES
__device__ unsigned long long s2_clk[1024 * 8];
#define S2_CLK(row, k) do { if (threadIdx.x == 0 && blockIdx.y == 0 && (row) < 1024) s2_clk[(size_t)(row) * 8 + (k)] = __builtin_amdgcn_s_memrealtime(); } while (0)
#else
#define S2_CLK(row, k) do { } while (0)
#endif
template <int SPEC>
__device__ __forceinline__ const uint32_t *stage2_sample(const Stage2Params &p, const S2Plan &pl, int s, char *smem, bool to_global, int part = 0)
{
    const int G = p.G, tid = threadIdx.x, nthr = blockDim.x;
    double2 *ltab = reinterpret_cast<double2 *>(smem);
    double *etab = reinterpret_cast<double *>(ltab + DSM_LOG_TAB_N);
    double *rcp = etab + DSM_EXP_TAB_N;
    double *gs = rcp + DSM_RCP_TAB_N;
    uint32_t *tab = reinterpret_cast<uint32_t *>(gs + 32);
    uint32_t *leaf = tab + S2_TAB_ENTRIES;
    int *n_lo = reinterpret_cast<int *>(leaf + 32);
    int *n_hi = n_lo + S2_MAX_NODES, *n_off = n_hi + S2_MAX_NODES, *n_idx = n_off + S2_MAX_NODES, *n_child = n_idx + S2_MAX_NODES;

    const int nsplit = p.nsplit > 1 ? p.nsplit : 1;
    S2_CLK(s, 0);
    uint32_t pre_n = 0;
    bool pre_ok = false;
    {
        const int total0 = 1 << G, share0 = nsplit > 1 ? (total0 + nsplit - 1) / nsplit : total0;
        const int j0 = (nsplit > 1 ? part * share0 : 0) + tid, jh0 = nsplit > 1 ? min(total0, part * share0 + share0) : total0;
        if (p.rep == 1 && j0 < jh0 && j0 != 0) {
            pre_n = p.ntab[(size_t)(((uint32_t)j0 * p.hmul + ((uint32_t)s >> 4) * p.swz) & ((1u << G) - 1u)) * (size_t)p.ld + s];
            pre_ok = true;
        }
    }
    if (s == 0 && part == 0 && tid < DSM_BIG_NT * DSM_BIG_NL && p.big_count) p.big_count[tid * DSM_BIG_STRIDE] = 0u;
    if (tid < DSM_LOG_TAB_N) ltab[tid] = reinterpret_cast<const double2 *>(p.log_tab)[tid];
    if (tid < DSM_EXP_TAB_N) etab[tid] = p.log_tab[2 * DSM_LOG_TAB_N + tid];
    for (int k = tid; k < DSM_RCP_TAB_N; k += nthr) rcp[k] = k ? 1.0 / (double)k : 0.0;
    if (tid < 32) {
        gs[tid] = (tid < G) ? p.gamma[(size_t)s * G + tid] : 0.0; leaf[tid] = 0u;
        n_lo[tid] = pl.lo[tid]; n_hi[tid] = pl.hi[tid]; n_off[tid] = pl.off[tid]; n_idx[tid] = pl.idx[tid];
        n_child[tid] = pl.child[tid];
    }
    for (int i = tid; i < S2_TAB_ENTRIES; i += nthr) tab[i] = 0u;
    __syncthreads();
    S2_CLK(s, 1);

    const int nlev = pl.nlevels > 1 ? pl.nlevels - 1 : pl.nlevels;
    for (int level = 0; level < nlev; ++level) {
        const int n0 = pl.level_start[level], n1 = pl.level_start[level + 1];
        const int base = pl.off[n0];
        const int total = (level == 0) ? (1 << G) : (pl.off[n1 - 1] + (1 << (pl.hi[n1 - 1] - pl.lo[n1 - 1]))) - base;
        const int share = (level == 0 && nsplit > 1) ? (total + nsplit - 1) / nsplit : total;
        const int j_lo = (level == 0 && nsplit > 1) ? part * share : 0, j_hi = (level == 0 && nsplit > 1) ? min(total, j_lo + share) : total;
        for (int j = j_lo + tid; j < j_hi; j += nthr) {
            int i = n0;
            for (int k = n0 + 1; k < n1; ++k) if (j + base >= pl.off[k]) i = k;
            const int lo = n_lo[i], hi = n_hi[i], w = hi - lo;
            const uint32_t Hs = (uint32_t)(j + base - n_off[i]);
            if (Hs == 0) continue;
            uint32_t n;
            if (level == 0) {
                uint32_t *cell = p.ntab + (size_t)((Hs * p.hmul + ((uint32_t)s >> 4) * p.swz) & ((1u << G) - 1u)) * (size_t)p.ld + s;
                const size_t cstride = ((size_t)1 << G) * (size_t)p.ld;
                if (p.rep == 8) {
                    uint32_t m[8];
#pragma unroll
                    for (int r = 0; r < 8; ++r) m[r] = __builtin_nontemporal_load(cell + r * cstride);
                    n = 0;
#pragma unroll
                    for (int r = 0; r < 8; ++r) { n += m[r]; if (m[r]) cell[r * cstride] = 0u; }
                } else {
                    n = (pre_ok && j == j_lo + tid) ? pre_n : *cell;
                    if (n) *cell = 0u;
                    for (int r = 1; r < p.rep; ++r) {
                        const uint32_t m = cell[r * cstride];
                        if (m) { cell[r * cstride] = 0u; n += m; }
                    }
                }
            } else n = tab[base + j];
            if (w == 1) {
                if (level == 0) leaf[lo] = n;
                continue;
            }
            if (!n) continue;
            const int wl = w / 2, wh = w - wl, mid = lo + wl;
            const int ch = n_child[i];
            uint32_t *L = tab + n_off[ch], *R = tab + n_off[ch + 1];
            const uint32_t HL = Hs & ((1u << wl) - 1u), HR = Hs >> wl;
            if (wl == 1) L = leaf + lo - 1;
            if (wh == 1) R = leaf + mid - 1;
            if (!HR) { atomicAdd(&L[HL], n); continue; }
            if (!HL) { atomicAdd(&R[HR], n); continue; }
            double wL = 0.0, wR = 0.0;
            for (int jj = 0; jj < wl; ++jj) if ((HL >> jj) & 1u) wL = wL + gs[lo + jj];
            for (int jj = 0; jj < wh; ++jj) if ((HR >> jj) & 1u) wR = wR + gs[mid + jj];
            Xo128 rng = xo_seed(Hs, (uint32_t)s | ((uint32_t)n_idx[i] << 16) | ((uint32_t)level << 24), p.iter, DSM_STREAM_STA2,
                                p.k0, p.k1);
            bool dummy = false;
            const uint32_t k = binom<true, SPEC>(rng, n, wL, wR, rcp, ltab, dummy, DSM_BINV_MEAN_CAP_S2);
            if (k) atomicAdd(&L[HL], k);
            if (n - k) atomicAdd(&R[HR], n - k);
        }
        __syncthreads();
        if (level < 4) S2_CLK(s, 2 + level);
        if (level == 0 && nsplit > 1) {
            const int l1 = pl.level_start[1], l2 = pl.level_start[2];
            const int b1 = pl.off[l1], n1 = (pl.off[l2 - 1] + (1 << (pl.hi[l2 - 1] - pl.lo[l2 - 1]))) - b1;
            uint32_t *row = p.scratch + (size_t)s * S2_TAB_ENTRIES;
            uint32_t sink = 0;
            for (int i = tid; i < n1; i += nthr) { const uint32_t v = tab[b1 + i]; if (v) sink += atomicAdd(&row[i], v); }
            asm volatile("" :: "v"(sink));
            __syncthreads();
            __shared__ int last_wg;
            if (tid == 0) last_wg = (atomicAdd(&p.ticket[s], 1u) == (uint32_t)(nsplit - 1)) ? 1 : 0;
            __syncthreads();
            if (!last_wg) return leaf;
            for (int i = tid; i < n1; i += nthr) tab[b1 + i] = atomicExch(&row[i], 0u);
            if (tid == 0) p.ticket[s] = 0u;
            __syncthreads();
        }
    }
    if (to_global && tid < G && leaf[tid]) p.sum_mu[(size_t)s * G + tid] += leaf[tid];
    return leaf;
}
```

### desman_amd/csrc/kernels_gibbs.hip

```cpp
#include <string.h>

#include <mutex>

#include "dsm_device.h"
#include "dsm_host.h"
#include "dsm_stage2.h"
#include "log_table.h"

__global__ __launch_bounds__(256) void convert_counts_kernel(const int64_t *__restrict__ in,
                                                             int32_t *__restrict__ cnt_vs, int V, int S,
                                                             int *flag, double *partial,
                                                             unsigned long long *__restrict__ depth)
{
    __shared__ double red[256];
    __shared__ unsigned long long dep[DSM_MAX_S];
    for (int i = threadIdx.x; i < S; i += 256) dep[i] = 0ull;
    __syncthreads();
    const size_t n = (size_t)V * S;
    double acc = 0.0;
    for (size_t i = (size_t)blockIdx.x * 256 + threadIdx.x; i < n; i += (size_t)gridDim.x * 256) {
        int4 c;
        int64_t x[4];
        int64_t tot = 0;
        bool bad = false;
// ... 390 lines not shown
    else if (tid >= GMAX && tid < GMAX + 16) { if (acc[tid]) atomicAdd(&esum[tid - GMAX], acc[tid]); }
}

#ifndef DSM_NT_RARE
#define DSM_NT_RARE 0.01f
#endif
struct FinalParams {
    const double *ll_partial; int nblocks;
    double ll_const, tau_prior;
    const double *prior; int S;
    int *nchange;
    int it;
    double *ll_trace, *lp_trace; int *nchange_trace;
    double *star;
    const double *gamma_src; double *gamma_star; int SG;
    const double *eta_src; double *eta_star;
    int star_mode;
    double *scalars;
    const double *ll_given;
    const uint32_t *step_cnt;
    unsigned long long *sweep_stats;
    uint32_t *screen_ctl;
    uint32_t *blk_order;
    int *rare_out; int G;
};

__device__ void finalize_body(const FinalParams &p, double *red, double *redp, int *flag, int tid, int nthr)
{
    double a = 0.0, b = 0.0;
    for (int i = tid; i < p.nblocks; i += nthr) a += p.ll_partial[i];
    for (int i = tid; i < p.S + 4; i += nthr) b += p.prior[i];
    red[tid] = a; redp[tid] = b;
    __syncthreads();
    for (int o = nthr / 2; o >= 1; o >>= 1) {
        if (tid < o) { red[tid] += red[tid + o]; redp[tid] += redp[tid + o]; }
        __syncthreads();
    }
    if (tid == 0) {
        const double ll = p.ll_given ? p.ll_given[0] : p.ll_const + red[0];
        const double lp = ll + redp[0] + p.tau_prior;
        p.scalars[0] = ll; p.scalars[1] = lp;
        const int nch = p.ll_given ? (int)p.ll_given[1] : *p.nchange;
        if (!p.ll_given) *p.nchange = 0;
        if (p.it >= 0) { p.ll_trace[p.it] = ll; p.lp_trace[p.it] = lp; p.nchange_trace[p.it] = nch; }
        int f = 0;
        if (p.star_mode == 1 || (p.star_mode == 0 && lp > p.star[0])) { p.star[0] = lp; p.star[1] = (double)(p.it + 1); f = 1; }
        *flag = f;
    }
    __syncthreads();
    if (*flag) {
        for (int i = tid; i < p.SG; i += nthr) p.gamma_star[i] = p.gamma_src[i];
        if (tid < 16) p.eta_star[tid] = p.eta_src[tid];
    }
    if (p.step_cnt) {
        __syncthreads();
        unsigned long long steps = 0, exact = 0;
        unsigned plain = 0;
        for (int i = tid; i < p.nblocks; i += nthr) {
            const uint32_t a = p.step_cnt[2 * i], b = p.step_cnt[2 * i + 1];
            steps += a;
            if (b == 0xFFFFFFFFu) { plain = 1; exact += a; } else exact += b;
        }
        red[tid] = (double)steps; redp[tid] = (double)exact;
        __syncthreads();
        for (int o = nthr / 2; o >= 1; o >>= 1) {
            if (tid < o) { red[tid] += red[tid + o]; redp[tid] += redp[tid + o]; }
            __syncthreads();
        }
        const unsigned any_plain = __syncthreads_or((int)plain);
        if (tid == 0 && red[0] > 0.0) {
            p.sweep_stats[0] += (unsigned long long)red[0];
            p.sweep_stats[1] += (unsigned long long)redp[0];
            if (any_plain) { if (p.screen_ctl[0] > 0) p.screen_ctl[0] -= 1; }
            else if (5.0 * redp[0] > 4.0 * red[0]) p.screen_ctl[0] = 15;
        }
        if (p.blk_order) {
            __syncthreads();
            int *cnt = reinterpret_cast<int *>(red);
            const int per = (p.nblocks + nthr - 1) / nthr, lo = tid * per, hi = min(p.nblocks, lo + per);
            auto cold = [&](int i) { const uint32_t b = p.step_cnt[2 * i + 1]; return b != 0u && b != 0xFFFFFFFFu; };
            int nc = 0;
            for (int i = lo; i < hi; ++i) nc += cold(i) ? 1 : 0;
            int incl = nc;
            for (int o = 1; o < 64; o <<= 1) { const int y = __shfl_up(incl, o, 64); if ((tid & 63) >= o) incl += y; }
            if ((tid & 63) == 63) cnt[tid >> 6] = incl;
            __syncthreads();
            int before = incl - nc, total = 0;
            for (int k = 0; k < nthr / 64; ++k) { const int x = cnt[k]; if (k < (tid >> 6)) before += x; total += x; }
            int pc = before, pw = total + (lo - before);
            for (int i = lo; i < hi; ++i) { if (cold(i)) p.blk_order[pc++] = (uint32_t)i; else p.blk_order[pw++] = (uint32_t)i; }
        }
    }
}

__global__ __launch_bounds__(256) void finalize_kernel(FinalParams p)
{
    __shared__ double red[256], redp[256];
    __shared__ int flag;
    finalize_body(p, red, redp, &flag, threadIdx.x, 256);
    if (p.rare_out) {
        __syncthreads();
        if (threadIdx.x == 0) flag = 0;
        __syncthreads();
        for (int g = threadIdx.x; g < p.G; g += 256) {
            double m = 0.0;
            for (int s = 0; s < p.S; ++s) m = fmax(m, p.gamma_src[(size_t)s * p.G + g]);
            if ((float)m <= (float)DSM_NT_RARE) atomicAdd(&flag, 1);
        }
        __syncthreads();
        if (threadIdx.x == 0) *p.rare_out = flag;
    }
}

__device__ double gamma_variate(double shape, uint32_t idx, uint32_t iter, uint32_t k0, uint32_t k1)
{
    const double a = (shape < 1.0) ? shape + 1.0 : shape;
    const double d = a - 1.0 / 3.0;
    const double c = 1.0 / sqrt(9.0 * d);
    double res = 0.0, uboost = 1.0;
    for (uint32_t attempt = 0; attempt < 4096u; ++attempt) {
        uint32_t r0[4], r1[4];
        philox4x32_10(idx, 2u * attempt, iter, DSM_STREAM_DIRI, k0, k1, r0);
        philox4x32_10(idx, 2u * attempt + 1u, iter, DSM_STREAM_DIRI, k0, k1, r1);
        const double u1 = u01_open(r0[0], r0[1]), u2 = u01_open(r0[2], r0[3]);
        const double u3 = u01_open(r1[0], r1[1]);
        uboost = u01_open(r1[2], r1[3]);
        const double x = sqrt(-2.0 * log(u1)) * cos(6.283185307179586 * u2);
        double vv = 1.0 + c * x;
        if (vv <= 0.0) continue;
        vv = vv * vv * vv;
        const double x2 = x * x;
        if (u3 < 1.0 - 0.0331 * x2 * x2 || log(u3) < 0.5 * x2 + d * (1.0 - vv + log(vv))) {
            res = d * vv;
            break;
        }
    }
    if (shape < 1.0) res *= pow(uboost, 1.0 / shape);
    return res;
}

struct DirParams {
    unsigned long long *sum_mu, *esum;
    int S, G;
    double alpha, delta, epsilon, lgc_gamma, lgc_eta;
    uint32_t k0, k1, iter;
    int zero_after;
    double *gamma_out, *gamma_trace, *eta_out, *eta_trace, *rowprior;
    int do_fin;
    FinalParams fin;
    int do_s2;
    Stage2Params s2;
};

__device__ __forceinline__ void dirichlet_body(const DirParams &q, const S2Plan &plan)
{
    unsigned long long *__restrict__ sum_mu = q.sum_mu, *__restrict__ esum = q.esum;
    const int S = q.S, G = q.G;
    const double alpha = q.alpha, delta = q.delta, epsilon = q.epsilon, lgc_gamma = q.lgc_gamma, lgc_eta = q.lgc_eta;
    const uint32_t k0 = q.k0, k1 = q.k1, iter = q.iter;
    const int zero_after = q.zero_after;
    double *__restrict__ gamma_out = q.gamma_out, *__restrict__ gamma_trace = q.gamma_trace;
    double *__restrict__ eta_out = q.eta_out, *__restrict__ eta_trace = q.eta_trace, *__restrict__ rowprior = q.rowprior;
    const int do_fin = q.do_fin, do_s2 = q.do_s2;
    const FinalParams &fin = q.fin;
    const Stage2Params &s2 = q.s2;
    __shared__ __attribute__((aligned(16))) char smem_d[S2_SMEM_BYTES];
    if (do_fin && (int)blockIdx.x == S + 4) {
        double *red = reinterpret_cast<double *>(smem_d), *redp = red + 256;
        int *flag = reinterpret_cast<int *>(redp + 256);
        finalize_body(fin, red, redp, flag, threadIdx.x, 256);
        return;
    }
    const int row = blockIdx.x;
    const bool is_gamma = row < S;
    const uint32_t *leaf = nullptr;
    if (do_s2 && is_gamma)
        leaf = do_s2 >= 3 ? stage2_sample<3>(s2, plan, row, smem_d, false) : stage2_sample<2>(s2, plan, row, smem_d, false);
    if (!is_gamma) {
        static_assert(DSM_ESUM_PARTS * 4 == 256, "one thread per (copy, observed base)");
        unsigned long long *ef = reinterpret_cast<unsigned long long *>(smem_d);
        if (threadIdx.x < 4) ef[threadIdx.x] = 0ull;
        __syncthreads();
        const int ob = threadIdx.x & 3, k = threadIdx.x >> 2;
        unsigned long long *pp = esum + 16 + k * 16 + ob * 4 + (row - S);
        const unsigned long long v = *pp;
        if (v) { *pp = 0ull; atomicAdd(&ef[ob], v); }
        __syncthreads();
    }
    S2_CLK(row, 6);
    if (threadIdx.x >= 64) return;
    const int lane = threadIdx.x;
    const int n = is_gamma ? G : 4;
    const int SG = S * G;
    double y = 0.0;
    if (lane < n) {
        double shape;
        uint32_t vid;
        if (is_gamma) { vid = (uint32_t)(row * G + lane); shape = alpha + (double)(sum_mu[vid] + (leaf ? (unsigned long long)leaf[lane] : 0ull)); }
        else { const int a = row - S; vid = (uint32_t)(SG + a * 4 + lane); shape = delta + (double)(esum[lane * 4 + a] + reinterpret_cast<const unsigned long long *>(smem_d)[lane]); }
        y = gamma_variate(shape, vid, iter, k0, k1);
        if (zero_after) { if (is_gamma) sum_mu[row * G + lane] = 0ull; else esum[lane * 4 + (row - S)] = 0ull; }
    }
    double x = y / group_allreduce_sum<64>(y);
    if (is_gamma) {
        if (lane < n && x < epsilon) x = epsilon;
        x = x / group_allreduce_sum<64>(lane < n ? x : 0.0);
    }
    const double a1 = is_gamma ? alpha : delta;
    const double lsum = group_allreduce_sum<64>(lane < n ? (a1 - 1.0) * log(x) : 0.0);
    if (lane == 0) rowprior[row] = (is_gamma ? lgc_gamma : lgc_eta) + lsum;
    if (lane < n) {
        if (is_gamma) { gamma_out[row * G + lane] = x; if (gamma_trace) gamma_trace[row * G + lane] = x; }
        else { eta_out[(row - S) * 4 + lane] = x; if (eta_trace) eta_trace[(row - S) * 4 + lane] = x; }
    }
    S2_CLK(row, 7);
}
#ifdef DSM_AB_SWITCHES
extern "C" int dsm_debug_s2_clocks(unsigned long long *out, int nrows)
{
    if (nrows > 1024) nrows = 1024;
    if (hipMemcpyFromSymbol(out, HIP_SYMBOL(s2_clk), (size_t)nrows * 8 * sizeof(unsigned long long)) != hipSuccess) return -1;
    return 8;
}
#endif

struct DirBatch { DirParams p[DSM_MAX_BATCH]; S2Plan plan; };
__global__ __launch_bounds__(256) void dirichlet_kernel(DirParams q, S2Plan plan) { dirichlet_body(q, plan); }
__global__ __launch_bounds__(256) void dirichlet_kernel_b(DirBatch b) { dirichlet_body(b.p[blockIdx.y], b.plan); }
static_assert(sizeof(DirBatch) <= 4096, "kernarg segment");

__global__ __launch_bounds__(256) void prior_kernel(const double *__restrict__ gamma, const double *__restrict__ eta,
                                                    int S, int G, double alpha, double delta, double lgc_gamma,
                                                    double lgc_eta, double *__restrict__ rowprior)
{
    for (int r = blockIdx.x * 256 + threadIdx.x; r < S + 4; r += gridDim.x * 256) {
        double lsum = 0.0;
        if (r < S) { for (int g = 0; g < G; ++g) lsum += (alpha - 1.0) * log(gamma[(size_t)r * G + g]); rowprior[r] = lgc_gamma + lsum; }
        else { for (int b = 0; b < 4; ++b) lsum += (delta - 1.0) * log(eta[(r - S) * 4 + b]); rowprior[r] = lgc_eta + lsum; }
    }
}

struct TauParams {
    const int32_t *cnt_vs;
    uint64_t *tau;
    uint64_t *trace;
    const double *gamma, *eta_sweep, *eta_ll;
    const uint32_t *u_raw;
    double *logp;
    double *ll_partial;
    const double *log_tab;
    int *nchange;
    uint32_t *step_cnt;
    const uint32_t *screen_ctl;
    int screen;
    int nt_skip;
    int V, S, G;
    int v_off;
    uint32_t k0, k1, iter;
    const uint32_t *order;
    int do_fin;
    FinalParams fin;
};

#ifdef TAU_NO_LEAN
#define TAU_LEAN(LPV, NSL) false
#else
#ifdef TAU_LEAN2
#define TAU_LEAN(LPV, NSL) ((LPV) >= 32 && ((NSL) == 2 || (NSL) == 3 || (NSL) == 6 || (NSL) == 8))
#else
#define TAU_LEAN(LPV, NSL) ((LPV) >= 32 && ((NSL) == 3 || (NSL) == 6 || (NSL) == 8))
#endif
#endif

template <int LPV, int NSL, bool SWEEP, bool LL, bool NT = false>
__device__ __forceinline__ void tau_body(const TauParams &p)
{
    extern __shared__ __attribute__((aligned(16))) char smem_t[];
    const int nblk = (int)gridDim.x - p.do_fin;
    if (p.do_fin && (int)blockIdx.x == nblk) {
        double *fr = reinterpret_cast<double *>(smem_t);
        finalize_body(p.fin, fr, fr + 256, reinterpret_cast<int *>(fr + 512), threadIdx.x, 256);
        return;
    }
    constexpr bool LEAN = TAU_LEAN(LPV, NSL) && SWEEP;
    const int bid = p.order ? (int)p.order[blockIdx.x] : (int)blockIdx.x;
    constexpr int SP = LPV * NSL;
    constexpr int GPB = 256 / LPV;
    double *gT = reinterpret_cast<double *>(smem_t);
    double *eS = gT + (size_t)p.G * SP;
    double *eL = eS + 16;
    double *red = eL + 16;
    int *redi = reinterpret_cast<int *>(red + 4);
    double2 *ltab = reinterpret_cast<double2 *>(red + 6);
    float *gT32 = reinterpret_cast<float *>(ltab + DSM_LOG_TAB_N);
    float *eS32 = gT32 + (size_t)p.G * SP;
    uint32_t *gmaxb = reinterpret_cast<uint32_t *>(eS32 + 24);
    const int tid = threadIdx.x, G = p.G, S = p.S;
    if (tid < DSM_LOG_TAB_N) ltab[tid] = reinterpret_cast<const double2 *>(p.log_tab)[tid];
    if constexpr (NT) {
        if (tid < 32) gmaxb[tid] = 0u;
        __syncthreads();
    }
    for (int i = tid; i < G * SP; i += 256) {
        const int g = i / SP, s = i % SP;
        const double x = (s < S) ? p.gamma[(size_t)s * G + g] : 1.0;
        gT[i] = x;
        if (SWEEP) gT32[i] = (float)x;
        if constexpr (NT) { if (s < S && g < 32) atomicMax(&gmaxb[g], __float_as_uint((float)x)); }
    }
    if (tid < 16) { eS[tid] = p.eta_sweep[tid]; eL[tid] = p.eta_ll[tid]; if (SWEEP) eS32[tid] = (float)p.eta_sweep[tid]; }
    if (SWEEP && tid < 4) {
        float m = (float)p.eta_sweep[tid], mx = m;
        for (int a = 1; a < 4; ++a) { m = fminf(m, (float)p.eta_sweep[a * 4 + tid]); mx = fmaxf(mx, (float)p.eta_sweep[a * 4 + tid]); }
        eS32[16 + tid] = m;
        if constexpr (NT) eS32[20 + tid] = mx * 1.000001f;
    }
    __syncthreads();

    const int grp = tid / LPV, lig = tid % LPV;
    double ll_acc = 0.0;
    int nchg = 0;
    int n_steps = 0, n_exact = 0;
    const bool screen_on = SWEEP && p.logp == nullptr && p.screen && *p.screen_ctl == 0u;

    for (int v = bid * GPB + grp; v < p.V; v += nblk * GPB) {
        ISA_MARK("variant_setup");
        uint64_t t = p.tau[v];
        int xi[LEAN ? 1 : NSL][4];
        float xs[LEAN ? NSL : 1][4];
        double xf[LEAN ? 1 : NSL][4];
#pragma unroll
        for (int j = 0; j < NSL; ++j) {
            int ligl = lig;
            if constexpr (LEAN) asm volatile("" : "+v"(ligl));
            const int s = ligl + j * LPV;
            int4 c = make_int4(0, 0, 0, 0);
            if (s < S) c = reinterpret_cast<const int4 *>(p.cnt_vs)[(size_t)v * S + s];
            if constexpr (LEAN) {
                xs[j][0] = (float)c.x; xs[j][1] = (float)c.y; xs[j][2] = (float)c.z; xs[j][3] = (float)c.w;
            } else {
                xi[j][0] = c.x; xi[j][1] = c.y; xi[j][2] = c.z; xi[j][3] = c.w;
#pragma unroll
                for (int b = 0; b < 4; ++b) xf[j][b] = (double)(float)xi[j][b];
            }
        }
        if (SWEEP) {
            double l_cur = 0.0;
            double pre[LEAN ? 1 : NSL][4];
            dsm_f2 pre32[LEAN ? NSL : 1][2];
#pragma unroll
            for (int j = 0; j < NSL; ++j) {
                if constexpr (LEAN) { pre32[j][0] = (dsm_f2){0.0f, 0.0f}; pre32[j][1] = (dsm_f2){0.0f, 0.0f}; }
                else {
#pragma unroll
                    for (int b = 0; b < 4; ++b) pre[j][b] = 0.0;
                }
            }
            bool have_cur = false;
            n_steps += G;
            const bool screen = screen_on;
            float xtot = 0.0f;
            if (screen) {
#pragma unroll
                for (int j = 0; j < NSL; ++j)
#pragma unroll
                    for (int b = 0; b < 4; ++b) { if constexpr (LEAN) xtot += xs[j][b]; else xtot += (float)xi[j][b]; }
                float z1 = 0.0f, z2 = 0.0f, z3 = 0.0f;
                group_allreduce_sum4_f32<LPV>(xtot, z1, z2, z3);
                xtot *= 1.0001f;
            }
            for (int g = 0; g < G; ++g) {
                double gg[NSL];
                if constexpr (!LEAN) {
#pragma unroll
                    for (int j = 0; j < NSL; ++j) gg[j] = gT[g * SP + lig + j * LPV];
                }
                ISA_MARK("step_setup");
                const int told = (int)((t >> (2 * g)) & 3);
                uint32_t uw;
                const size_t ui = (size_t)v * G + g;
// ... 233 lines not shown
    HIP_TRY(hipGetLastError());
    return DSM_OK;
}

int k_pack_tau(dsm_ctx *c, const int64_t *d_onehot, uint64_t *d_packed, int V, int G)
{
    hipLaunchKernelGGL(pack_tau_kernel, dim3((V + 255) / 256), dim3(256), 0, c->stream, d_onehot, d_packed, V, G);
    HIP_TRY(hipGetLastError());
    return DSM_OK;
}

int k_unpack_tau(dsm_ctx *c, const uint64_t *d_packed, int64_t *d_onehot, int V, int G)
{
    const size_t n = (size_t)V * G;
    hipLaunchKernelGGL(unpack_tau_kernel, dim3((unsigned)((n + 255) / 256)), dim3(256), 0, c->stream, d_packed,
                       d_onehot, V, G);
    HIP_TRY(hipGetLastError());
    return DSM_OK;
}

int k_tau_sum(dsm_ctx *c, const uint64_t *trace, int n, int64_t *d_sum)
{
    const size_t m = (size_t)c->V * c->G;
    hipLaunchKernelGGL(tau_sum_kernel, dim3((unsigned)((m + 255) / 256)), dim3(256), 0, c->stream, trace, n, c->V,
                       c->G, d_sum);
    HIP_TRY(hipGetLastError());
    return DSM_OK;
}

int k_mt_fill(dsm_ctx *c, uint32_t *out, size_t n, hipStream_t stream)
{
    if (n == 0) return DSM_OK;
    KTimer tm(c, DSM_K_MT, stream);
    const size_t hog = (size_t)140 * 1024;
    if (!c->mt_attr_set) {
        HIP_TRY(hipFuncSetAttribute((const void *)mt_fill_wide_kernel, hipFuncAttributeMaxDynamicSharedMemorySize, (int)hog));
        c->mt_attr_set = true;
    }
    if (!g_batch.K && n >= 6 * MTJ_D) {
        size_t made = 0;
        { const int r = mt_fill_parallel(c, out, n, stream, &made); if (r != DSM_OK) return r; }
        out += made; n -= made;
        if (n == 0) return DSM_OK;
    }
    if (g_batch.K) {
        static thread_local BatchArgs<MtArgs> acc;
        acc.p[g_batch.k] = MtArgs{c->mt_state, out, n};
        if (g_batch.k == g_batch.K - 1)
            hipLaunchKernelGGL(mt_fill_wide_kernel_b, dim3(g_batch.K), dim3(1024), 0, stream, acc);
    } else
        hipLaunchKernelGGL(mt_fill_wide_kernel, dim3(1), dim3(1024), hog, stream, c->mt_state, out, n);
    HIP_TRY(hipGetLastError());
    return DSM_OK;
}

int k_stats_v1(dsm_ctx *c, uint32_t iter)
{
    if (!c->items_built) { int r = build_stats_items(c); if (r != DSM_OK) return r; }
    KTimer tm(c, DSM_K_STATS);
    if (c->max_items == 0) return DSM_OK;
    static const int sizes[] = {1, 2, 3, 4, 5, 6, 7, 8, 10, 12, 14, 16, 20, 24, 28, 32};
    int gm = 32;
    for (int z : sizes) if (c->G <= z) { gm = z; break; }
    const void *fn = nullptr;
    const bool exact = (c->G == gm);
#define STATS_FN(GM) if (gm == GM) fn = exact ? (const void *)stats_kernel<GM, true> : (const void *)stats_kernel<GM, (GM <= 8)>
    STATS_FN(1); STATS_FN(2); STATS_FN(3); STATS_FN(4); STATS_FN(5); STATS_FN(6); STATS_FN(7); STATS_FN(8);
    STATS_FN(10); STATS_FN(12); STATS_FN(14); STATS_FN(16); STATS_FN(20); STATS_FN(24); STATS_FN(28); STATS_FN(32);
#undef STATS_FN
    const int key = gm * 2 + (exact ? 1 : 0);
    if (c->blk_gmax != key) {
        int occ = 0;
        HIP_TRY(hipOccupancyMaxActiveBlocksPerMultiprocessor(&occ, fn, 256, 0));
        hipDeviceProp_t prop;
        HIP_TRY(hipGetDeviceProperties(&prop, c->device));
        if (occ < 1) occ = 1;
        const int S = c->S, budget = std::max(S, occ * prop.multiProcessorCount);
        double tot = 0.0;
        for (int s = 0; s < S; ++s) tot += (double)c->depth[s];
        std::vector<int32_t> nb(S, 1);
        int used = S;
        if (tot > 0)
            for (int s = 0; s < S; ++s) {
                int extra = (int)((double)(budget - S) * (double)c->depth[s] / tot);
                const int most = (c->nitems_h[s] + 255) / 256;
                if (1 + extra > most) extra = std::max(0, most - 1);
                nb[s] += extra; used += extra;
            }
        std::vector<int32_t> tab;
        tab.reserve((size_t)used * 3);
        int maxnb = 0;
        for (int s = 0; s < S; ++s) maxnb = std::max(maxnb, nb[s]);
        for (int j = 0; j < maxnb; ++j)
            for (int s = 0; s < S; ++s)
                if (j < nb[s]) { tab.push_back(s); tab.push_back(j); tab.push_back(nb[s]); }
        if (c->blk_tab) { (void)hipFree(c->blk_tab); c->blk_tab = nullptr; }
        HIP_TRY(hipMalloc((void **)&c->blk_tab, tab.size() * sizeof(int32_t)));
        HIP_TRY(hipMemcpyAsync(c->blk_tab, tab.data(), tab.size() * sizeof(int32_t), hipMemcpyHostToDevice, c->stream));
        HIP_TRY(hipStreamSynchronize(c->stream));
        c->blk_n = used;
        c->blk_gmax = key;
    }
    const dim3 grid(c->blk_n), block(256);
    const uint32_t k0 = (uint32_t)c->ctr_seed, k1 = (uint32_t)(c->ctr_seed >> 32);
#define LAUNCH_STATS(GM, EX)                                                                                          \
    hipLaunchKernelGGL((stats_kernel<GM, EX>), grid, block, 0, c->stream, reinterpret_cast<const int2 *>(c->items),   \
                       c->nitems, c->blk_tab, c->tau, c->gamma, c->eta,                                               \
                       c->V, c->S, c->G, c->item_stride, c->chunked ? 1 : 0, k0, k1, iter, c->sum_mu, c->esum)
#define STATS_CASE(GM) if (gm == GM) { if (exact) LAUNCH_STATS(GM, true); else LAUNCH_STATS(GM, (GM <= 8)); }
    STATS_CASE(1); STATS_CASE(2); STATS_CASE(3); STATS_CASE(4); STATS_CASE(5); STATS_CASE(6); STATS_CASE(7);
    STATS_CASE(8); STATS_CASE(10); STATS_CASE(12); STATS_CASE(14); STATS_CASE(16); STATS_CASE(20); STATS_CASE(24);
    STATS_CASE(28); STATS_CASE(32);
#undef STATS_CASE
#undef LAUNCH_STATS
    HIP_TRY(hipGetLastError());
    return DSM_OK;
}

static void dirichlet_consts(const dsm_ctx *c, double *lgc_gamma, double *lgc_eta)
{
    *lgc_gamma = lgamma(c->alpha * c->G) - c->G * lgamma(c->alpha);
    *lgc_eta = lgamma(c->delta * 4) - 4 * lgamma(c->delta);
}

static FinalParams make_final(dsm_ctx *c, int nblocks, int it, int star_mode, const double *prior, const double *gamma_src,
                              const double *eta_src, int slot = 0)
{
    FinalParams p;
    p.ll_partial = c->ll_partial + (size_t)slot * DSM_MAX_GRID; p.nblocks = nblocks;
    p.ll_const = c->ll_const;
    p.tau_prior = (double)(c->shard_on ? c->shard_vtot : c->V) * (double)c->G * log(1.0 / 4.0);
    p.ll_given = c->shard_on ? c->shard_vec : nullptr;
    p.prior = prior; p.S = c->S; p.nchange = c->nchange + slot; p.it = it;
    p.ll_trace = c->ll_trace; p.lp_trace = c->lp_trace; p.nchange_trace = c->nchange_trace;
    p.star = c->star; p.gamma_src = gamma_src; p.gamma_star = c->gamma_star; p.SG = c->S * c->G;
    p.eta_src = eta_src; p.eta_star = c->eta_star;
    p.star_mode = star_mode; p.scalars = c->scalars;
    p.step_cnt = c->step_cnt + (size_t)slot * 2 * DSM_MAX_GRID; p.sweep_stats = c->sweep_stats; p.screen_ctl = c->screen_ctl + slot;
    static const bool order_on = !(getenv("DESMAN_HIP_TAU_ORDER") && atoi(getenv("DESMAN_HIP_TAU_ORDER")) == 0);
    p.blk_order = nullptr;
    p.rare_out = nullptr; p.G = c->G;
    if (order_on && c->blk_order && nblocks > 0 && nblocks <= DSM_MAX_GRID) {
        if (c->tau_resident_key != c->S * 64 + c->G) {
            int launched = 0, resident = 0;
            if (tau_launch_info(c, &launched, &resident) == DSM_OK) { c->tau_resident = resident; c->tau_resident_key = c->S * 64 + c->G; }
        }
        if (c->tau_resident > 0 && nblocks > c->tau_resident) { p.blk_order = c->blk_order + (size_t)slot * DSM_MAX_GRID; c->blk_order_n[slot] = nblocks; }
        else c->blk_order_n[slot] = 0;
    }
    return p;
}

int k_dirichlet(dsm_ctx *c, uint32_t iter, double *gamma_out, double *gamma_trace, double *eta_out, double *eta_trace,
                double *prior_out, int fin_it, int fin_nblocks, const double *fin_prior, int do_s2)
{
    KTimer tm(c, DSM_K_DIRICH);
    double lg, le;
    dirichlet_consts(c, &lg, &le);
    const uint32_t k0 = (uint32_t)c->ctr_seed, k1 = (uint32_t)(c->ctr_seed >> 32);
    const int do_fin = fin_it >= 0 ? 1 : 0;
    FinalParams fin = {};
    if (do_fin)
        fin = make_final(c, fin_nblocks, fin_it, 0, fin_prior, c->gamma_trace + (size_t)fin_it * c->S * c->G,
                         c->eta_trace + (size_t)fin_it * 16);
    Stage2Params s2 = {};
    if (do_s2) {
        s2.ntab = c->ntab; s2.rep = c->ntab_rep; s2.ld = c->ntab_ld; s2.gamma = c->gamma; s2.sum_mu = c->sum_mu; s2.log_tab = c->log_tab;
        s2.S = c->S; s2.G = c->G; s2.k0 = k0; s2.k1 = k1; s2.iter = iter; s2.hmul = DSM_NTAB_HMUL; s2.swz = DSM_NTAB_SWZ;
        s2.big_count = c->big_count;
    }
    DirParams q;
    q.sum_mu = c->sum_mu; q.esum = c->esum; q.S = c->S; q.G = c->G;
    q.alpha = c->alpha; q.delta = c->delta; q.epsilon = c->epsilon; q.lgc_gamma = lg; q.lgc_eta = le;
    q.k0 = k0; q.k1 = k1; q.iter = iter; q.zero_after = 1;
    q.gamma_out = gamma_out; q.gamma_trace = gamma_trace; q.eta_out = eta_out; q.eta_trace = eta_trace; q.rowprior = prior_out;
    q.do_fin = do_fin; q.fin = fin; q.do_s2 = do_s2 ? stats_draw_version(stats_spec(c)) : 0; q.s2 = s2;
    if (g_batch.K == 0) {
        const S2Plan plan = do_s2 ? make_stage2_plan(c->G) : S2Plan{};
        hipLaunchKernelGGL(dirichlet_kernel, dim3(c->S + 4 + do_fin), dim3(256), 0, c->stream, q, plan);
    } else {
        static thread_local DirBatch acc;
        acc.p[g_batch.k] = q;
        if (g_batch.k == g_batch.K - 1) {
            acc.plan = do_s2 ? make_stage2_plan(c->G) : S2Plan{};
            hipLaunchKernelGGL(dirichlet_kernel_b, dim3(c->S + 4 + do_fin, g_batch.K), dim3(256), 0, c->stream, acc);
        }
    }
    HIP_TRY(hipGetLastError());
    return DSM_OK;
}

__global__ __launch_bounds__(256) void prior_batch_kernel(const double *__restrict__ gamma, const double *__restrict__ eta,
                                                          int n, int S, int G, double alpha, double delta,
                                                          double lgc_gamma, double lgc_eta, double *__restrict__ rowprior)
{
    const int rows = S + 4;
    for (size_t i = (size_t)blockIdx.x * 256 + threadIdx.x; i < (size_t)n * rows; i += (size_t)gridDim.x * 256) {
        const int it = (int)(i / rows), r = (int)(i % rows);
        double lsum = 0.0;
        if (r < S) {
            const double *g = gamma + ((size_t)it * S + r) * G;
            for (int k = 0; k < G; ++k) lsum += (alpha - 1.0) * log(g[k]);
            rowprior[i] = lgc_gamma + lsum;
        } else {
            const double *e = eta + (size_t)it * 16 + (r - S) * 4;
            for (int b = 0; b < 4; ++b) lsum += (delta - 1.0) * log(e[b]);
            rowprior[i] = lgc_eta + lsum;
        }
    }
}

int k_prior_batch(dsm_ctx *c, const double *gamma, const double *eta, int n, double *prior_out)
{
    double lg, le;
    dirichlet_consts(c, &lg, &le);
    const size_t tot = (size_t)n * (c->S + 4);
    const int grid = (int)std::min<size_t>((tot + 255) / 256, 1024);
    hipLaunchKernelGGL(prior_batch_kernel, dim3(grid), dim3(256), 0, c->stream, gamma, eta, n, c->S, c->G, c->alpha, c->delta,
                       lg, le, prior_out);
    HIP_TRY(hipGetLastError());
    return DSM_OK;
}

int k_prior(dsm_ctx *c, const double *gamma, const double *eta, double *prior_out)
{
    double lg, le;
    dirichlet_consts(c, &lg, &le);
    hipLaunchKernelGGL(prior_kernel, dim3(1), dim3(256), 0, c->stream, gamma, eta, c->S, c->G, c->alpha, c->delta, lg,
                       le, prior_out);
    HIP_TRY(hipGetLastError());
    return DSM_OK;
}

__global__ __launch_bounds__(256) void gamma_rare_kernel(const double *__restrict__ gamma, int S, int G, int *__restrict__ out)
{
    __shared__ int cnt;
    if (threadIdx.x == 0) cnt = 0;
    __syncthreads();
    for (int g = threadIdx.x; g < G; g += 256) {
        double m = 0.0;
        for (int s = 0; s < S; ++s) m = fmax(m, gamma[(size_t)s * G + g]);
        if ((float)m <= (float)DSM_NT_RARE) atomicAdd(&cnt, 1);
    }
    __syncthreads();
    if (threadIdx.x == 0) *out = cnt;
}
int k_tau_neartie_hint(dsm_ctx *c)
{
    c->tau_neartie_on = false;
    if (c->tau_neartie_mode == 0 || g_batch.K || c->shard_on || !c->tau_screen || c->G < 2) return DSM_OK;
    c->tau_neartie_on = c->tau_neartie_mode == 1 || (c->tau_rare_n > 0 && c->tau_rare_n < c->G);
    return DSM_OK;
}
int tau_rare_from_host(const double *gamma, int S, int G)
{
    int n = 0;
    for (int g = 0; g < G; ++g) {
        double m = 0.0;
        for (int s = 0; s < S; ++s) m = std::max(m, gamma[(size_t)s * G + g]);
        n += (float)m <= (float)DSM_NT_RARE;
    }
    return n;
}
int k_tau_rare_count(dsm_ctx *c, bool wait)
{
    if (!c->h_rare) HIP_TRY(hipHostMalloc((void **)&c->h_rare, sizeof(int), hipHostMallocDefault));
    hipLaunchKernelGGL(gamma_rare_kernel, dim3(1), dim3(256), 0, c->stream, c->gamma, c->S, c->G, c->nchange + 1);
    HIP_TRY(hipGetLastError());
    HIP_TRY(hipMemcpyAsync(c->h_rare, c->nchange + 1, sizeof(int), hipMemcpyDeviceToHost, c->stream));
    HIP_TRY(hipMemsetAsync(c->nchange + 1, 0, sizeof(int), c->stream));
    if (wait) { HIP_TRY(hipStreamSynchronize(c->stream)); c->tau_rare_n = *c->h_rare; }
    return DSM_OK;
}

template <int LPV, int NSL>
static void launch_tau(dsm_ctx *c, int mode, const TauParams &p, int grid, size_t sh)
{
    const int g2 = grid + p.do_fin;
    if (g_batch.K) {
        static thread_local BatchArgs<TauParams> acc;
        acc.p[g_batch.k] = p;
        if (g_batch.k == g_batch.K - 1)
            hipLaunchKernelGGL((tau_kernel_b<LPV, NSL, true, true>), dim3(g2, g_batch.K), dim3(256), sh, c->stream, acc);
        return;
    }
    if (mode == 3 && c->tau_neartie_on) hipLaunchKernelGGL((tau_kernel_nt<LPV, NSL>), dim3(g2), dim3(256), sh, c->stream, p);
    else if (mode == 3) hipLaunchKernelGGL((tau_kernel<LPV, NSL, true, true>), dim3(g2), dim3(256), sh, c->stream, p);
    else if (mode == 1) hipLaunchKernelGGL((tau_kernel<LPV, NSL, true, false>), dim3(g2), dim3(256), sh, c->stream, p);
    else hipLaunchKernelGGL((tau_kernel<LPV, NSL, false, true>), dim3(g2), dim3(256), sh, c->stream, p);
}

static int tau_shape(int S, int *lpv, int *nsl)
{
    int LPV, NSL;
    if (S <= 16) { LPV = 16; NSL = 1; }
    else if (S <= 32) { LPV = 16; NSL = 2; }
    else if (S <= 48) { LPV = 16; NSL = 3; }
    else if (S <= 64) { LPV = 32; NSL = 2; }
    else if (S > 64 && S <= 96) { LPV = 32; NSL = 3; }
    else {
        LPV = 64;
        const int need = (S + 63) / 64;
        NSL = need <= 4 ? need : (need <= 6 ? 6 : 8);
        if (need > 8) { dsm_set_error("S=%d exceeds DSM_MAX_S=%d", S, DSM_MAX_S); return DSM_ERR_UNSUPPORTED; }
    }
    *lpv = LPV; *nsl = NSL;
    return DSM_OK;
}
static size_t tau_lds_bytes(int G, int LPV, int NSL)
{
    return ((size_t)G * LPV * NSL + 16 + 16 + 6 + 2 * DSM_LOG_TAB_N) * sizeof(double) +
           ((size_t)G * LPV * NSL + 24 + 32) * sizeof(float);
}

int k_tau_sweep(dsm_ctx *c, int mode, const double *gamma, const double *eta_sweep, const double *eta_ll,
                uint64_t *trace_slot, double *d_logp, uint32_t iter, int *nblocks, const uint32_t *u_raw, int slot,
                const TauFinalRider *rider)
{
    KTimer tm(c, DSM_K_TAU);
    const int S = c->S, G = c->G, V = c->V;
    int LPV, NSL;
    { const int rc = tau_shape(S, &LPV, &NSL); if (rc != DSM_OK) return rc; }
    const int gpb = 256 / LPV;
    int grid = (V + gpb - 1) / gpb;
    if (grid > DSM_MAX_GRID) grid = DSM_MAX_GRID;
    {
        static const int genv = DSM_AB_ENV("DESMAN_HIP_TAU_GRID") ? atoi(DSM_AB_ENV("DESMAN_HIP_TAU_GRID")) : 0;
        if (genv > 0 && genv < grid) grid = genv;
    }
    if (grid < 1) grid = 1;
    TauParams p;
    p.cnt_vs = c->cnt_vs; p.tau = c->tau; p.trace = trace_slot;
// ... 94 lines not shown
```

### desman_amd/csrc/kernels_stats.hip

```cpp
#include "dsm_binom.h"
#include "dsm_host.h"
#include "log_table.h"

#include <string.h>

#include <algorithm>
#include <vector>

#ifdef DSM_AB_SWITCHES
#define STATS_DBG(p, mask) ((p).dbg & (mask))
#else
#define STATS_DBG(p, mask) 0
#endif
#ifdef DSM_AB_SWITCHES
#define S1_NCLK 16
__device__ unsigned long long s1_clk[8192 * S1_NCLK];
#define S1_CLK(k) do { if ((threadIdx.x & 63) == 0 && blockIdx.y == 0) s1_clk[(size_t)(blockIdx.x * 4 + (threadIdx.x >> 6)) * S1_NCLK + (k)] = __builtin_amdgcn_s_memrealtime(); } while (0)
extern "C" int dsm_debug_s1_clocks(unsigned long long *out, int nwaves)
{
    if (nwaves > 8192) nwaves = 8192;
    if (hipMemcpyFromSymbol(out, HIP_SYMBOL(s1_clk), (size_t)nwaves * S1_NCLK * sizeof(unsigned long long)) != hipSuccess) return -1;
    return S1_NCLK;
}
#else
// ... 425 lines not shown
}
template <int SPEC>
__global__ __launch_bounds__(1024) void stats_stage2_kernel_b(Stage2Batch b)
{
    __shared__ __attribute__((aligned(16))) char smem2[S2_SMEM_BYTES];
    stage2_sample<SPEC>(b.p[blockIdx.y], b.plan, blockIdx.x, smem2, true);
}

template <int SPEC>
__global__ __launch_bounds__(256) void binom_test_kernel(int kind, uint32_t n, double wa, double wb, double w2, double w3,
                                                         uint32_t k0, uint32_t k1, int nsamp, const double *log_tab,
                                                         uint32_t *out)
{
    __shared__ double2 ltab[DSM_LOG_TAB_N + DSM_EXP_TAB_N / 2];
    __shared__ double rcp[DSM_RCP_TAB_N];
    const int tid = threadIdx.x;
    ltab[tid] = reinterpret_cast<const double2 *>(log_tab)[tid];
    if (tid < DSM_EXP_TAB_N / 2) ltab[DSM_LOG_TAB_N + tid] = reinterpret_cast<const double2 *>(log_tab)[DSM_LOG_TAB_N + tid];
    for (int k = tid; k < DSM_RCP_TAB_N; k += blockDim.x) rcp[k] = k ? 1.0 / (double)k : 0.0;
    __syncthreads();
    const int i = blockIdx.x * 256 + tid;
    if (i >= nsamp) return;
    Xo128 rng = xo_seed((uint32_t)i, 0u, 0u, DSM_STREAM_TEST, k0, k1);
    bool dummy = false;
    if (kind != 2) out[i] = binom<true, SPEC>(rng, n, wa, wb, rcp, ltab, dummy, kind == 0 ? DSM_BINV_MEAN_CAP : DSM_BINV_MEAN_CAP_S2);
    else {
        const double W[4] = {wa, wb, w2, w3};
        uint32_t m[4];
        mult4<true, SPEC>(rng, n, W, m, rcp, ltab, dummy);
        out[i * 4 + 0] = m[0]; out[i * 4 + 1] = m[1]; out[i * 4 + 2] = m[2]; out[i * 4 + 3] = m[3];
    }
}

static int stats_agg_lpv(int S)
{
    int best = 64;
    for (int l : {32, 16}) if ((S + l - 1) / l * l < (S + best - 1) / best * best) best = l;
    return best;
}

int stats_spec(const dsm_ctx *c)
{
    int force = c->force_stats_spec;
    if (force == 0) {
        const char *e = getenv("DESMAN_HIP_STATS_SPEC");
        if (e && (e[0] == '1' || e[0] == '2' || e[0] == '3' || e[0] == '4') && e[1] == 0) force = e[0] - '0';
    }
    if (force == 1) return 1;
    if (c->G < 1 || c->G > 16) return 1;
    if (((size_t)1 << c->G) * (size_t)c->S * 4 > ((size_t)64 << 20)) return 1;
    if (c->max_depth >= ((uint64_t)1 << 32)) return 1;
    const bool pat_ok = c->G <= 8 && !c->shard_on;
    if (force == 4) return pat_ok ? 4 : 2;
    if (force >= 2) return force;
    double reads = 0.0;
    for (int64_t d : c->depth) reads += (double)d;
    const int lpv = stats_agg_lpv(c->S);
    const double cells = (double)c->V * (double)((c->S + lpv - 1) / lpv * lpv);
    const double g = (double)c->G;
    const double t1 = 25.0 + (0.25 + 0.02 * g + 0.0029 * g * g) * 1e-6 * reads;
    const double stage2 = 14.0 + (c->G >= 10 ? 0.012 * (double)(1u << c->G) : 0.0);
    const int rep = stats_ntab_rep(c);
    const double per = 3.0 * (double)c->V / (double)(1u << c->G);
    const double t2 = 24.0 + stage2 + 0.062e-3 * cells + (rep == 1 ? 0.03 * per : 0.003 * per / rep);
    if (pat_ok && force == 0 && t2 < t1) {
        const bool small_g = (c->G <= 2 && cells >= 0.5e6) || (c->G == 3 && cells >= 1.0e6);
        const bool mid_g = c->G >= 4 && cells >= 2.5e6 && 64.0 * (double)((size_t)1 << c->G) <= (double)c->V;
        if (small_g || mid_g) return 4;
    }
    return t2 < t1 ? DSM_STATS_AGG : 1;
}

int stats_ntab_rep(const dsm_ctx *c)
{
    const double per = 3.0 * (double)(c->shard_on ? c->shard_vtot : c->V) / (double)((size_t)1 << c->G);
    if (per <= 128.0) return 1;
    const double lines = (double)((((size_t)1 << c->G) * (size_t)c->S * 4 + 63) / 64);
    int rep = 2;
    while (lines * rep < 384.0 && rep < 64 && (size_t)(2 * rep) * ((size_t)1 << c->G) * (size_t)c->S * 4 <= ((size_t)64 << 20)) rep *= 2;
    return rep;
}

void stats_release_ntab(dsm_ctx *c)
{
    if (c->ntab_raw) (void)hipFree(c->ntab_raw);
    c->ntab_raw = nullptr; c->ntab = nullptr; c->ntab_len = 0;
}
static int ensure_ntab(dsm_ctx *c)
{
    const int rep = stats_ntab_rep(c), ld = c->S;
    const size_t need = (size_t)rep * ((size_t)1 << c->G) * (size_t)ld;
    if (c->ntab && c->ntab_len == need && c->ntab_ld == ld && c->ntab_rep == rep) return DSM_OK;
    stats_release_ntab(c);
    c->ntab_rep = rep; c->ntab_ld = ld;
    const char *eo = DSM_AB_ENV("DESMAN_HIP_NTAB_OFF");
    const size_t off = eo ? ((size_t)strtoull(eo, nullptr, 0) & ~(size_t)255) : 0;
    const size_t spare = off + 4096;
    hipError_t e = hipMalloc((void **)&c->ntab_raw, need * sizeof(uint32_t) + spare);
    if (e != hipSuccess) { dsm_set_error("hipMalloc(%zu B) failed: %s", need * 4 + spare, hipGetErrorString(e)); return DSM_ERR_NOMEM; }
    c->ntab = reinterpret_cast<uint32_t *>(((uintptr_t)c->ntab_raw + 4095) & ~(uintptr_t)4095) + off / 4;
    c->ntab_len = need;
    HIP_TRY(hipMemsetAsync(c->ntab, 0, need * sizeof(uint32_t), c->stream));
    return DSM_OK;
}

int stats_ensure_ntab(dsm_ctx *c)
{
    return stats_spec(c) < 2 ? DSM_OK : ensure_ntab(c);
}

static int ensure_big_list(dsm_ctx *c, size_t seg)
{
    const size_t need = seg * DSM_BIG_NT * DSM_BIG_NL;
    if (c->big_list && c->big_cap == need) return DSM_OK;
    if (c->big_list) { (void)hipFree(c->big_list); c->big_list = nullptr; }
    if (!c->big_count) {
        hipError_t e = hipMalloc((void **)&c->big_count, DSM_BIG_NT * DSM_BIG_NL * DSM_BIG_STRIDE * sizeof(uint32_t));
        if (e != hipSuccess) { dsm_set_error("hipMalloc failed: %s", hipGetErrorString(e)); return DSM_ERR_NOMEM; }
    }
    hipError_t e = hipMalloc((void **)&c->big_list, need * sizeof(unsigned long long));
    if (e != hipSuccess) { dsm_set_error("hipMalloc(%zu B) failed: %s", need * 8, hipGetErrorString(e)); return DSM_ERR_NOMEM; }
    c->big_cap = need;
    HIP_TRY(hipMemsetAsync(c->big_count, 0, DSM_BIG_NT * DSM_BIG_NL * DSM_BIG_STRIDE * sizeof(uint32_t), c->stream));
    return DSM_OK;
}

static int ensure_pat(dsm_ctx *c)
{
    const size_t nrep = (size_t)1 << (2 * c->G), nx = (size_t)c->V * 4 * (size_t)c->S;
    if (!c->pat_rep || c->pat_rep_len != nrep) {
        if (c->pat_rep) { (void)hipFree(c->pat_rep); c->pat_rep = nullptr; }
        hipError_t e = hipMalloc((void **)&c->pat_rep, nrep * sizeof(unsigned long long));
        if (e != hipSuccess) { dsm_set_error("hipMalloc(%zu B) failed: %s", nrep * 8, hipGetErrorString(e)); return DSM_ERR_NOMEM; }
        c->pat_rep_len = nrep;
        c->pat_gen = 0;
        HIP_TRY(hipMemsetAsync(c->pat_rep, 0xFF, nrep * sizeof(unsigned long long), c->stream));
    }
    if (!c->pat_list || c->pat_rep_len != nrep || c->pat_gen == 0) {
        if (c->pat_list) { (void)hipFree(c->pat_list); c->pat_list = nullptr; }
        hipError_t e = hipMalloc((void **)&c->pat_list, (nrep + 2) * sizeof(uint32_t));
        if (e != hipSuccess) { dsm_set_error("hipMalloc(%zu B) failed: %s", (nrep + 2) * 4, hipGetErrorString(e)); return DSM_ERR_NOMEM; }
        HIP_TRY(hipMemsetAsync(c->pat_list + nrep, 0, 2 * sizeof(uint32_t), c->stream));
    }
    if (!c->pat_x || c->pat_x_len != nx) {
        if (c->pat_x) { (void)hipFree(c->pat_x); c->pat_x = nullptr; }
        hipError_t e = hipMalloc((void **)&c->pat_x, nx * sizeof(uint32_t));
        if (e != hipSuccess) { dsm_set_error("hipMalloc(%zu B) failed: %s", nx * 4, hipGetErrorString(e)); return DSM_ERR_NOMEM; }
        c->pat_x_len = nx;
        HIP_TRY(hipMemsetAsync(c->pat_x, 0, nx * sizeof(uint32_t), c->stream));
    }
    return DSM_OK;
}

int k_stats_stage1(dsm_ctx *c, uint32_t iter)
{
    int r = ensure_ntab(c);
    if (r != DSM_OK) return r;
    const int S = c->S, G = c->G, V = c->V;
    const int LPV = stats_agg_lpv(S);
    const int NCH = (S + LPV - 1) / LPV, SP = NCH * LPV, NG = 64 / LPV;
    const int spec_full = stats_spec(c);
    const bool pat = spec_full == 4;
    const int spec = stats_draw_version(spec_full);
    const size_t sh = ((size_t)G * SP + (spec >= 3 ? 2 * DSM_LOG_TAB_N + DSM_EXP_TAB_N : 0) + DSM_RCP_TAB_N + 16) * sizeof(double) +
                      16 * 256 * sizeof(uint32_t);
    if (sh > 160 * 1024) { dsm_set_error("stats_agg: gamma tile (%zu B) exceeds LDS", sh); return DSM_ERR_UNSUPPORTED; }
    const void *fn = nullptr, *fn_b = nullptr;
#define AGG_CASE(L, SP_) if (LPV == L && spec == SP_) { fn = (const void *)stats_agg_kernel<L, SP_>; fn_b = (const void *)stats_agg_kernel_b<L, SP_>; }
    AGG_CASE(16, 2) AGG_CASE(32, 2) AGG_CASE(64, 2) AGG_CASE(16, 3) AGG_CASE(32, 3) AGG_CASE(64, 3)
#undef AGG_CASE
    if (pat) {
        fn = LPV == 16 ? (const void *)stats_pat_kernel<16> : LPV == 32 ? (const void *)stats_pat_kernel<32> : (const void *)stats_pat_kernel<64>;
        fn_b = LPV == 16 ? (const void *)stats_pat_kernel_b<16> : LPV == 32 ? (const void *)stats_pat_kernel_b<32> : (const void *)stats_pat_kernel_b<64>;
    }
    if (!fn) { dsm_set_error("stats_agg: no kernel for spec %d", spec); return DSM_ERR_UNSUPPORTED; }
    if (c->stats_grid == 0 || c->stats_grid_key != spec_full) {
        int occ = 0;
        HIP_TRY(hipOccupancyMaxActiveBlocksPerMultiprocessor(&occ, fn, 256, sh));
        hipDeviceProp_t prop;
        HIP_TRY(hipGetDeviceProperties(&prop, c->device));
        const int wgs = std::min(6, std::max(1, occ));
        const int n_xcd = prop.multiProcessorCount % 8 == 0 && prop.multiProcessorCount >= 64 ? 8 : 1;
        const long passes4 = (((long)V * NCH + NG - 1) / NG) / std::max(1L, (long)wgs * prop.multiProcessorCount);
        const int leave = (c->tau_rng == DSM_RNG_MT19937 && passes4 <= 12) ? n_xcd : 0;
        c->stats_grid = wgs * std::max(1, prop.multiProcessorCount - leave);
        c->stats_grid_key = spec_full;
    }
    const long ntask = ((long)V * NCH + NG - 1) / NG;
    const long max_waves = (long)c->stats_grid * 4 / (g_batch.K ? g_batch.K : 1);
    const long waves = std::min<long>(ntask, max_waves);
    const int grid = (int)std::max<long>(1, (waves + 3) / 4);
    const long per_wg = ((ntask + waves - 1) / waves) * 4 * 64 * 4;
    const size_t seg = (size_t)std::min<long>((long)V * S * 4, ((grid + DSM_BIG_NL - 1) / DSM_BIG_NL) * per_wg);
    r = ensure_big_list(c, seg);
    if (r != DSM_OK) return r;
    StatsAggParams p;
    p.cnt_vs = c->cnt_vs; p.tau = c->tau; p.gamma = c->gamma; p.eta = c->eta;
    p.V = V; p.S = S; p.G = G; p.big_seg = seg;
    p.v_off = c->shard_on ? c->shard_voff : 0; p.V_tot = c->shard_on ? c->shard_vtot : V;
    p.k0 = (uint32_t)c->ctr_seed; p.k1 = (uint32_t)(c->ctr_seed >> 32); p.iter = iter;
    p.ntab = c->ntab; p.rep = c->ntab_rep; p.ld = c->ntab_ld; p.esum = c->esum; p.log_tab = c->log_tab;
    p.xcd = 0;
    p.hmul = DSM_NTAB_HMUL; p.swz = DSM_NTAB_SWZ;
    p.big_list = c->big_list; p.big_count = c->big_count;
    p.pat_rep = nullptr; p.pat_x = nullptr; p.pat_list = nullptr; p.pat_n = nullptr;
    if (pat) {
        r = ensure_pat(c);
        if (r != DSM_OK) return r;
        p.pat_rep = c->pat_rep; p.pat_x = c->pat_x;
        KTimer tm(c, DSM_K_STATSPAT);
        const uint32_t hi = 0xFFFFFFFFu - (++c->pat_gen);
        const int words = 1 << (2 * G);
        uint32_t *n_this = c->pat_list + words + (c->pat_gen & 1u), *n_next = c->pat_list + words + ((c->pat_gen + 1u) & 1u);
        p.pat_list = c->pat_list; p.pat_n = n_this;
        if (G <= 6) hipLaunchKernelGGL(pat_rep_lds_kernel, dim3(std::max(1, std::min(64, V / 4096))), dim3(1024), 0, c->stream, c->tau, V, G, c->pat_rep, hi);
        else hipLaunchKernelGGL(pat_rep_kernel, dim3((V + 255) / 256), dim3(256), 0, c->stream, c->tau, V, G, c->pat_rep, hi);
        hipLaunchKernelGGL(pat_list_kernel, dim3((words + 255) / 256), dim3(256), 0, c->stream, c->pat_rep, words, hi, c->pat_list, n_this, n_next);
        const size_t ncell = (size_t)V * S;
        const int lpw = G <= 3 ? 64 : 32;
        const size_t lds = ((size_t)1 << (2 * G)) * 4 * lpw * sizeof(uint32_t);
        if (G <= 4 && lds <= 128 * 1024 && V >= 4096) {
            const int nchunk = (S + lpw - 1) / lpw;
            const int nvsplit = std::max(1, std::min(256 / nchunk, V / (16 * (64 / lpw) * 8)));
            const void *fl = lpw == 64 ? (const void *)pat_agg_lds_kernel<64> : (const void *)pat_agg_lds_kernel<32>;
            static bool attr_done[2] = {false, false};
            if (!attr_done[lpw == 32]) { HIP_TRY(hipFuncSetAttribute(fl, hipFuncAttributeMaxDynamicSharedMemorySize, 128 * 1024)); attr_done[lpw == 32] = true; }
            const int32_t *cv = c->cnt_vs; const uint64_t *tp = c->tau; const unsigned long long *rp = c->pat_rep; uint32_t *xp = c->pat_x;
            int Vv = V, Ss = S, Gg = G, nvs = nvsplit;
            void *args[] = {(void *)&cv, (void *)&tp, (void *)&Vv, (void *)&Ss, (void *)&Gg, (void *)&rp, (void *)&xp, (void *)&nvs};
            HIP_TRY(hipLaunchKernel(fl, dim3(nchunk * nvsplit), dim3(1024), args, lds, c->stream));
        } else
            hipLaunchKernelGGL(pat_agg_kernel, dim3((unsigned)std::min<size_t>((ncell + 255) / 256, 16384)), dim3(256), 0, c->stream,
                               c->cnt_vs, c->tau, V, S, G, c->pat_rep, c->pat_x);
        HIP_TRY(hipGetLastError());
    }
    {
        static const char *e = DSM_AB_ENV("DESMAN_HIP_LEAN_CAP");
        p.lean_cap = e ? atof(e) : DSM_LEAN_CAP;
        static const int dbg = DSM_AB_ENV("DESMAN_HIP_STATS_DBG") ? atoi(DSM_AB_ENV("DESMAN_HIP_STATS_DBG")) : 0;
        p.dbg = dbg;
        if (!(p.lean_cap > 0.0 && p.lean_cap <= DSM_BINV_MEAN_CAP)) p.lean_cap = DSM_LEAN_CAP;
    }
    const int big_wgs = 16;
    const int big_grid = DSM_BIG_NT * DSM_BIG_NL *
        (int)std::max<long>(1, std::min<long>((ntask * 64 * 4 / DSM_BIG_NL + 255) / 256, g_batch.K ? std::max(2, big_wgs / g_batch.K) : big_wgs));
    if (g_batch.K) {
        static thread_local BatchArgs<StatsAggParams> acc;
        acc.p[g_batch.k] = p;
        if (g_batch.k == g_batch.K - 1) {
            const dim3 g(grid, g_batch.K);
            void *args[] = {(void *)&acc};
            HIP_TRY(hipLaunchKernel(fn_b, g, dim3(256), args, sh, c->stream));
            if (spec >= 3) hipLaunchKernelGGL(stats_big_kernel_b<3>, dim3(big_grid, g_batch.K), dim3(256), 0, c->stream, acc);
            else hipLaunchKernelGGL(stats_big_kernel_b<2>, dim3(big_grid, g_batch.K), dim3(256), 0, c->stream, acc);
        }
        HIP_TRY(hipGetLastError());
        return DSM_OK;
    }
    {
        KTimer tm(c, DSM_K_STATS);
        void *args[] = {(void *)&p};
        HIP_TRY(hipLaunchKernel(fn, dim3(grid), dim3(256), args, sh, c->stream));
    }
    KTimer tm(c, DSM_K_STATSBIG);
    if (spec >= 3) hipLaunchKernelGGL(stats_big_kernel<3>, dim3(big_grid), dim3(256), 0, c->stream, p);
    else hipLaunchKernelGGL(stats_big_kernel<2>, dim3(big_grid), dim3(256), 0, c->stream, p);
    HIP_TRY(hipGetLastError());
    return DSM_OK;
}

S2Plan make_stage2_plan(int G)
{
    S2Plan pl;
    memset(&pl, 0, sizeof pl);
    int n = 0, off = 0;
    pl.lo[0] = 0; pl.hi[0] = G; pl.off[0] = 0; pl.idx[0] = 0; pl.child[0] = -1;
    n = 1;
    int lvl_begin = 0, lvl_end = 1, level = 0;
    pl.level_start[0] = 0;
    while (lvl_begin < lvl_end) {
        for (int i = lvl_begin; i < lvl_end; ++i) {
            const int w = pl.hi[i] - pl.lo[i];
            if (w == 1) { pl.child[i] = -1; continue; }
            const int wl = w / 2, mid = pl.lo[i] + wl;
            pl.child[i] = n;
            pl.lo[n] = pl.lo[i]; pl.hi[n] = mid; pl.off[n] = off; pl.idx[n] = 2 * pl.idx[i]; off += 1 << wl; ++n;
            pl.lo[n] = mid; pl.hi[n] = pl.hi[i]; pl.off[n] = off; pl.idx[n] = 2 * pl.idx[i] + 1; off += 1 << (w - wl); ++n;
        }
        lvl_begin = lvl_end; lvl_end = n;
        pl.level_start[++level] = lvl_begin;
    }
    pl.nlevels = level;
    pl.tab_entries = off;
    return pl;
}

int k_stats_stage2(dsm_ctx *c, uint32_t iter)
{
    KTimer tm(c, DSM_K_STATS2);
    Stage2Params p;
    p.ntab = c->ntab; p.rep = c->ntab_rep; p.ld = c->ntab_ld; p.gamma = c->gamma; p.sum_mu = c->sum_mu; p.log_tab = c->log_tab;
    p.S = c->S; p.G = c->G; p.hmul = DSM_NTAB_HMUL; p.swz = DSM_NTAB_SWZ;
    p.k0 = (uint32_t)c->ctr_seed; p.k1 = (uint32_t)(c->ctr_seed >> 32); p.iter = iter;
    p.big_count = c->big_count;
    const int nthr = c->G >= 10 ? 1024 : 256;
    const bool v3 = stats_draw_version(stats_spec(c)) >= 3;
    p.nsplit = 1; p.scratch = nullptr; p.ticket = nullptr;
    if (g_batch.K == 0 && c->G >= 11) {
        if (!c->s2_scratch) {
            hipError_t e = hipMalloc((void **)&c->s2_scratch, ((size_t)DSM_MAX_S * (S2_TAB_ENTRIES + 1)) * sizeof(uint32_t));
            if (e != hipSuccess) { dsm_set_error("hipMalloc failed: %s", hipGetErrorString(e)); return DSM_ERR_NOMEM; }
            HIP_TRY(hipMemsetAsync(c->s2_scratch, 0, ((size_t)DSM_MAX_S * (S2_TAB_ENTRIES + 1)) * sizeof(uint32_t), c->stream));
        }
        p.nsplit = c->G >= 12 ? 4 : 2;
        p.scratch = c->s2_scratch; p.ticket = c->s2_scratch + (size_t)DSM_MAX_S * S2_TAB_ENTRIES;
    }
    if (g_batch.K == 0) {
        if (v3) hipLaunchKernelGGL(stats_stage2_kernel<3>, dim3(c->S * p.nsplit), dim3(nthr), 0, c->stream, p, make_stage2_plan(c->G));
        else hipLaunchKernelGGL(stats_stage2_kernel<2>, dim3(c->S * p.nsplit), dim3(nthr), 0, c->stream, p, make_stage2_plan(c->G));
    } else {
        static thread_local Stage2Batch acc;
        acc.p[g_batch.k] = p;
        if (g_batch.k == g_batch.K - 1) {
            acc.plan = make_stage2_plan(c->G);
            if (v3) hipLaunchKernelGGL(stats_stage2_kernel_b<3>, dim3(c->S, g_batch.K), dim3(nthr), 0, c->stream, acc);
            else hipLaunchKernelGGL(stats_stage2_kernel_b<2>, dim3(c->S, g_batch.K), dim3(nthr), 0, c->stream, acc);
        }
    }
    HIP_TRY(hipGetLastError());
    return DSM_OK;
}

int k_stats(dsm_ctx *c, uint32_t iter)
{
    if (stats_spec(c) >= 2) {
        int r = k_stats_stage1(c, iter);
        if (r != DSM_OK) return r;
        return k_stats_stage2(c, iter);
    }
    return k_stats_v1(c, iter);
}

int k_binom_test(dsm_ctx *c, int kind, uint32_t n, const double *w, uint64_t seed, int nsamp, uint32_t *d_out, int spec)
{
    if (spec >= 3) hipLaunchKernelGGL(binom_test_kernel<3>, dim3((nsamp + 255) / 256), dim3(256), 0, c->stream, kind, n, w[0], w[1], w[2], w[3],
                                      (uint32_t)seed, (uint32_t)(seed >> 32), nsamp, c->log_tab, d_out);
    else hipLaunchKernelGGL(binom_test_kernel<2>, dim3((nsamp + 255) / 256), dim3(256), 0, c->stream, kind, n, w[0], w[1], w[2], w[3],
                       (uint32_t)seed, (uint32_t)(seed >> 32), nsamp, c->log_tab, d_out);
    HIP_TRY(hipGetLastError());
    return DSM_OK;
}
```

### include/desman_hip.h

```cpp
#ifndef DESMAN_HIP_H
#define DESMAN_HIP_H

#include <stdint.h>

#ifdef __cplusplus
extern "C" {
#endif

#define DSM_OK               0
#define DSM_ERR_HIP         -1
#define DSM_ERR_ARG         -2
#define DSM_ERR_STATE       -3
#define DSM_ERR_UNSUPPORTED -4
#define DSM_ERR_NOMEM       -5
#define DSM_ERR_NODEVICE    -6
#define DSM_ERR_COMM        -7

#define DSM_MAX_G  32
#define DSM_MAX_S  512

#define DSM_RNG_MT19937 0
#define DSM_RNG_PHILOX  1

const char *dsm_last_error(void);
int dsm_device_count(void);
const char *dsm_version(void);

int dsm_initRNG(void);
int dsm_setRNG(unsigned long seed);
int dsm_freeRNG(void);
int dsm_sample_tau(int64_t *tau, const double *pi, const double *eta,
                   const int64_t *variants, int nV, int nG, int nS);
void c_initRNG(void);
void c_setRNG(unsigned long seed);
void c_freeRNG(void);
int c_sample_tau(long *tau, double *pi, double *eta, long *variants, int nV, int nG, int nS);
int dsm_getRNG_state(uint32_t *state625);
int dsm_setRNG_state(const uint32_t *state625);

typedef struct dsm_ctx dsm_ctx;

int dsm_ctx_create(dsm_ctx **out, int device);
int dsm_ctx_destroy(dsm_ctx *ctx);
int dsm_ctx_sync(dsm_ctx *ctx);

int dsm_ctx_set_counts(dsm_ctx *ctx, const int64_t *variants, int V, int S);

int dsm_ctx_set_state(dsm_ctx *ctx, const int64_t *tau, const double *gamma,
                      const double *eta, int G);
int dsm_ctx_get_state(dsm_ctx *ctx, int64_t *tau, double *gamma, double *eta);
int dsm_ctx_set_gamma_eta(dsm_ctx *ctx, const double *gamma, const double *eta);

int dsm_ctx_set_priors(dsm_ctx *ctx, double alpha, double delta, double epsilon);

int dsm_ctx_seed(dsm_ctx *ctx, unsigned long mt_seed, uint64_t ctr_seed);
int dsm_ctx_set_tau_rng(dsm_ctx *ctx, int mode );
int dsm_ctx_get_mt_state(dsm_ctx *ctx, uint32_t *state625);
int dsm_ctx_set_mt_state(dsm_ctx *ctx, const uint32_t *state625);
int dsm_ctx_debug_mt_fill(dsm_ctx *ctx, size_t n, uint32_t *out);
int dsm_mt_seed_state(unsigned long seed, uint32_t *state625);

int dsm_ctx_sample_tau(dsm_ctx *ctx, int *nchange, double *logp_out);

int dsm_ctx_sample_stats(dsm_ctx *ctx, uint32_t iter, uint64_t *sum_mu, uint64_t *esum);
int dsm_ctx_stats_spec(dsm_ctx *ctx);
int dsm_ctx_force_stats_spec(dsm_ctx *ctx, int spec);
int dsm_ctx_debug_stage1(dsm_ctx *ctx, uint32_t iter, uint32_t *ntab, uint64_t *esum);
int dsm_ctx_debug_binom(dsm_ctx *ctx, int kind, uint32_t n, const double *w4, uint64_t seed, int nsamp,
                        uint32_t *out, int spec);

int dsm_ctx_draw_gamma_eta(dsm_ctx *ctx, uint32_t iter, const uint64_t *sum_mu,
                           const uint64_t *esum, double *gamma_out, double *eta_out);

int dsm_ctx_loglik(dsm_ctx *ctx, double *ll, double *lp);

int dsm_ctx_gibbs_update(dsm_ctx *ctx, int n_iter);
int dsm_batch_gibbs_update(dsm_ctx *const *ctxs, int n_ctx, int n_iter);
int dsm_ctx_update_tau(dsm_ctx *ctx, int n_iter, const double *gamma_store,
                       const double *eta_store);
int dsm_batch_update_tau(dsm_ctx *const *ctxs, int n_ctx, int n_iter, const double *const *gamma_stores,
                         const double *const *eta_stores);

int dsm_ctx_get_trace(dsm_ctx *ctx, double *ll, double *lp, int32_t *nchange,
                      double *gamma_store, double *eta_store);
int dsm_ctx_get_star(dsm_ctx *ctx, int64_t *tau_star, double *gamma_star,
                     double *eta_star, double *lp_star, int *iter_star);
int dsm_ctx_get_tau_sum(dsm_ctx *ctx, int64_t *tau_sum);
int dsm_ctx_get_tau_at(dsm_ctx *ctx, int it, int64_t *tau);

int dsm_nmft_set(dsm_ctx *ctx, const double *tau, const double *gamma, int G);
int dsm_nmft_get(dsm_ctx *ctx, double *tau, double *gamma);
int dsm_nmft_factorize(dsm_ctx *ctx, int max_iter, double min_change, int fix_gamma,
                       int *n_done, double *div_trace);
int dsm_batch_nmft_factorize(dsm_ctx *const *ctxs, int n_ctx, int max_iter, double min_change, int fix_gamma,
                             int *n_done, double *div_traces);
int dsm_nmft_objective(dsm_ctx *ctx, double *div);
int dsm_nmft_debug_path(dsm_ctx *ctx, int fix_gamma, int out[8]);
int dsm_nmft_get_tau(dsm_ctx *ctx, int64_t *tau_onehot);

int dsm_lrt_step(int device, const double *ffreq, const int32_t *maxA, const int32_t *maxB,
                 const double *eta, double upperP, int optimise, int V, double *p_inout,
                 double *MLL, double *BLL);

#define DSM_ASSIGN_MAX_G 10
int dsm_assign_tau(int device, const int64_t *counts , int N, int S, int G, const double *gamma, const double *eta,
                   uint64_t seed, uint8_t *map_state, double *conf, double *logz, double *marg, uint8_t *draw_state);
int dsm_ctx_assign_tau(dsm_ctx *ctx, const double *gamma, const double *eta, int G, uint64_t seed, uint8_t *map_state,
                       double *conf, double *logz, double *marg, uint8_t *draw_state);
int dsm_assign_debug_set_chunk(int positions);

int dsm_fit_gamma(int device, const int64_t *counts , int V, int S, int G, const int64_t *tau ,
                  const double *eta, int max_iter, double tol, int presence, double *gamma, double *loglik, double *deviance,
                  int32_t *iters, int32_t *converged, double *lr_absent);
int dsm_ctx_fit_gamma(dsm_ctx *ctx, int G, const int64_t *tau , const double *eta, int max_iter, double tol,
                      int presence, double *gamma, double *loglik, double *deviance, int32_t *iters, int32_t *converged,
                      double *lr_absent);
int dsm_abund_debug_set_chunk(int samples);

int dsm_fit_gamma_interval(int device, const int64_t *counts , int V, int S, int G, const int64_t *tau ,
                           const double *eta, const double *gamma_hat , double q, int max_iter, double tol, double ctol,
                           double *lo, double *hi, int32_t *flags);
int dsm_ctx_fit_gamma_interval(dsm_ctx *ctx, int G, const int64_t *tau , const double *eta,
                               const double *gamma_hat, double q, int max_iter, double tol, double ctol, double *lo, double *hi,
                               int32_t *flags);

int dsm_fit_gamma_eta(int device, const int64_t *counts , int V, int S, int G, const int64_t *tau ,
                      const double *eta0, int max_iter, double tol, double *gamma, double *eta, double *loglik, double *loglik0,
                      double *deviance, int32_t *iters, int32_t *converged, int32_t *dead_rows, double *lr_eta);
int dsm_ctx_fit_gamma_eta(dsm_ctx *ctx, int G, const int64_t *tau , const double *eta0, int max_iter, double tol,
                          double *gamma, double *eta, double *loglik, double *loglik0, double *deviance, int32_t *iters,
                          int32_t *converged, int32_t *dead_rows, double *lr_eta);
int dsm_abund_debug_set_eta_batch(int steps);
int dsm_abund_debug_set_eta_stage_max(long long bytes);

typedef struct dsm_genes dsm_genes;
#define DSM_MAX_ETA 8

int dsm_genes_create(dsm_genes **out, int device);
int dsm_genes_destroy(dsm_genes *gs);
int dsm_genes_set_data(dsm_genes *gs, const int64_t *variants, int Vtot, int S, int C,
                       const int32_t *gene_off , const double *cov);
int dsm_genes_set_model(dsm_genes *gs, const double *gamma, const double *epsilon,
                        const double *delta, int G, int max_eta, const double *eta_log_prior,
                        const double *cov_const, const double *mult_const);
int dsm_genes_set_state(dsm_genes *gs, const int32_t *eta, const int64_t *tau);
int dsm_genes_get_state(dsm_genes *gs, int32_t *eta, int64_t *tau);
int dsm_genes_seed(dsm_genes *gs, unsigned long mt_seed, uint64_t ctr_seed);
int dsm_genes_set_gene_base(dsm_genes *gs, int gene_base);
int dsm_genes_get_mt_state(dsm_genes *gs, uint32_t *state625);
int dsm_genes_set_mt_state(dsm_genes *gs, const uint32_t *state625);

int dsm_genes_nmft_tau(dsm_genes *gs, const int32_t *eta_mask ,
                       const double *tau_init, int max_iter, double min_change, int32_t *n_iter);
int dsm_genes_sweep_all(dsm_genes *gs, const int32_t *eta_mask, int sweep, int32_t *nchange,
                        double *logvar, double *v_ll);
int dsm_genes_step_candidates(dsm_genes *gs, int c, int g, double *logvar, int *swept);
int dsm_genes_step_choose(dsm_genes *gs, int c, int g, int eta_value);
int dsm_genes_update(dsm_genes *gs, int n_iter, int reset_star, int32_t *eta_store,
                     double *gene_ll_trace, const uint32_t *u_tau_ext, const double *u_eta_ext);
int dsm_genes_loglik(dsm_genes *gs, double *gene_ll);
int dsm_genes_get_star(dsm_genes *gs, int32_t *eta_star, double *gene_llstar);
int dsm_genes_set_star(dsm_genes *gs, const int32_t *eta_star, const double *gene_llstar);
int dsm_genes_debug_tile(const dsm_genes *gs, int *lpv, int *nsl, int *groups_per_block, size_t *lds_bytes);

int dsm_kl_assign(int device, const double *cov, const double *delta, double *eta, int C, int S,
                  int G, int max_iter, double min_change, int *n_done, double *div);

#define DSM_K_STATS    0
#define DSM_K_DIRICH   1
#define DSM_K_TAU      2
#define DSM_K_FINAL    3
#define DSM_K_MT       4
#define DSM_K_NMFT_A   5
#define DSM_K_NMFT_G   6
#define DSM_K_NMFT_B   7
#define DSM_K_STATS2   8
#define DSM_K_STATSBIG 9
#define DSM_K_STATSPAT 10
#define DSM_K_COUNT    11
int dsm_ctx_sweep_stats(dsm_ctx *ctx, uint64_t *steps, uint64_t *exact_steps, int mode);
int dsm_ctx_debug_log2f(dsm_ctx *ctx, const float *in, float *out, size_t n);
int dsm_release_device_caches(void);
int dsm_debug_fdiv(int kind, const double *a, const double *b, double *out, int n);
int dsm_ctx_set_nmft_fused(dsm_ctx *ctx, int mode);
int dsm_ctx_set_nmft_persist(dsm_ctx *ctx, int mode);
int dsm_ctx_set_tau_screen(dsm_ctx *ctx, int on);
int dsm_ctx_set_tau_neartie(dsm_ctx *ctx, int mode);
int dsm_ctx_tau_launch_info(dsm_ctx *ctx, int *launched, int *resident);
int dsm_ctx_get_counters(dsm_ctx *ctx, uint64_t *ctr_seed, uint32_t *iter_ctr);
int dsm_ctx_set_counters(dsm_ctx *ctx, uint64_t ctr_seed, uint32_t iter_ctr);
int dsm_ctx_get_screen_state(dsm_ctx *ctx, uint32_t *out2);
int dsm_ctx_set_screen_state(dsm_ctx *ctx, const uint32_t *in2);
typedef int (*dsm_exchange_fn)(void *user, uint32_t *dev_tab, size_t n_tab, double *dev_vec, size_t n_vec);
int dsm_ctx_gibbs_update_sharded(dsm_ctx *ctx, int n_iter, int v_offset, int v_total, dsm_exchange_fn exchange, void *user);
typedef struct dsm_comm dsm_comm;
int dsm_comm_unique_id(void *id128);
int dsm_comm_create(dsm_comm **out, const void *id128, int rank, int world, int device);
int dsm_comm_destroy(dsm_comm *comm);
int dsm_comm_rank(const dsm_comm *comm);
int dsm_comm_world(const dsm_comm *comm);
int dsm_comm_allgather_f64(dsm_comm *comm, const double *send, double *recv, size_t n);
int dsm_comm_allreduce_f64(dsm_comm *comm, double *data, size_t n, int op);
int dsm_comm_barrier(dsm_comm *comm);
int dsm_ctx_gibbs_update_sharded_comm(dsm_ctx *ctx, int n_iter, int v_offset, int v_total, dsm_comm *comm);
int dsm_device_read(int device, const void *dev, void *host, size_t bytes);
int dsm_device_write(int device, void *dev, const void *host, size_t bytes);
int dsm_ctx_set_timing(dsm_ctx *ctx, int on);
int dsm_ctx_get_timing(dsm_ctx *ctx, double *ms_total ,
                       int64_t *launches );
const char *dsm_kernel_name(int k);

#ifdef __cplusplus
}
#endif
#endif
```

Measured before the change: 6.339 billion V*S updates/s.

## Skip stats_big kernel launch after quiet streak, serve big items in dirichlet

Tracks, through a device control word mirrored to pinned host memory, how many consecutive iterations produced no 'big' items. After a quiet run of 16 iterations the host stops launching the separate stats_big kernel, and the fused dirichlet/stage2 kernel instead processes any big items that do appear, using the previous gamma. The goal is to drop one kernel launch per iteration in the common case where no big items exist. The cost is extra shared memory, more complex stage2 code, a host read of pinned memory that may lag the device, and a retire protocol based on atomic counters.

```diff
diff --git a/desman_amd/_lib.py b/desman_amd/_lib.py
--- a/desman_amd/_lib.py
+++ b/desman_amd/_lib.py
@@ -66,6 +66,9 @@
     "dsm_debug_fdiv": (_i, [_i, _f64p, _f64p, _f64p, _i]),
     "dsm_release_device_caches": (_i, []),
     "dsm_ctx_force_stats_spec": (_i, [_vp, _i]),
+    "dsm_ctx_set_big_launch": (_i, [_vp, _i]),
+    "dsm_ctx_debug_big_served": (_i, [_vp, C.POINTER(C.c_uint64)]),
+    "dsm_ctx_debug_big_skipped": (_i, [_vp, C.POINTER(C.c_uint64), C.POINTER(C.c_uint32)]),
     "dsm_ctx_debug_stage1": (_i, [_vp, C.c_uint32, _vp, _u64p]),
     "dsm_ctx_debug_binom": (_i, [_vp, _i, C.c_uint32, _f64p, C.c_uint64, _i, _u32p, _i]),
     "dsm_ctx_draw_gamma_eta": (_i, [_vp, C.c_uint32, _u64p, _u64p, _f64p, _f64p]),
@@ -559,6 +562,19 @@
     def force_stats_spec(self, spec=0):
         check(self.lib.dsm_ctx_force_stats_spec(self._h, int(spec)))
 
+    def set_big_launch(self, mode=0):
+        check(self.lib.dsm_ctx_set_big_launch(self._h, int(mode)))
+
+    def big_served(self):
+        n = C.c_uint64(0)
+        check(self.lib.dsm_ctx_debug_big_served(self._h, C.byref(n)))
+        return int(n.value)
+
+    def big_skipped(self):
+        n, q = C.c_uint64(0), C.c_uint32(0)
+        check(self.lib.dsm_ctx_debug_big_skipped(self._h, C.byref(n), C.byref(q)))
+        return int(n.value), int(q.value)
+
     def debug_stage1(self, it):
         nt = np.zeros((self.S, 1 << self.G), dtype=np.uint32)
         E = np.zeros((4, 4), dtype=np.uint64)
diff --git a/desman_amd/csrc/api.hip b/desman_amd/csrc/api.hip
--- a/desman_amd/csrc/api.hip
+++ b/desman_amd/csrc/api.hip
@@ -218,6 +218,8 @@
     dev_free(&c->cnt_vs); dev_free(&c->items); dev_free(&c->nitems); dev_free(&c->tau);
     dev_free(&c->pat_rep); dev_free(&c->pat_x); dev_free(&c->pat_list); c->pat_rep_len = c->pat_x_len = 0;
     if (c->h_rare) { (void)hipHostFree(c->h_rare); c->h_rare = nullptr; }
+    if (c->h_big) { (void)hipHostFree(c->h_big); c->h_big = nullptr; }
+    dev_free(&c->big_ctl); dev_free(&c->gamma_entry);
     dev_free(&c->s2_scratch);
     dev_free(&c->blk_tab); stats_release_ntab(c); dev_free(&c->big_list); dev_free(&c->big_count);
     dev_free(&c->gamma); dev_free(&c->eta);
@@ -252,6 +254,7 @@
     const size_t n = (size_t)V * S;
     c->V = V; c->S = S;
     c->have_state = false;
+    c->big_known = false;
     c->G = 0;
     TRY(dev_alloc(&c->cnt_vs, n * 4));
     TRY(dev_alloc(&c->nitems, (size_t)S));
@@ -397,6 +400,7 @@
     HIP_TRY(hipMemcpyAsync(c->eta, eta, 16 * sizeof(double), hipMemcpyHostToDevice, c->stream));
     HIP_TRY(hipStreamSynchronize(c->stream));
     c->have_state = true;
+    c->big_known = false;
     return DSM_OK;
 }
 
@@ -465,6 +469,8 @@
     BIND(c);
     c->ctr_seed = ctr_seed;
     c->iter_ctr = 0;
+    c->big_skipped = 0;
+    if (c->big_ctl) HIP_TRY(hipMemsetAsync(c->big_ctl + 4, 0, 2 * sizeof(uint32_t), c->stream));
     return seed_mt(c, mt_seed);
 }
 
@@ -654,6 +660,31 @@
 {
     if (!c || spec < 0 || spec > 4) { dsm_set_error("force_stats_spec: 0 (rule), 1, 2, 3 or 4"); return DSM_ERR_ARG; }
     c->force_stats_spec = spec;
+    c->big_known = false;
+    return DSM_OK;
+}
+
+extern "C" int dsm_ctx_set_big_launch(dsm_ctx *c, int mode)
+{
+    if (!c || mode < 0 || mode > 2) { dsm_set_error("set_big_launch: 0 (rule), 1 (always) or 2 (never)"); return DSM_ERR_ARG; }
+    c->big_launch_mode = mode;
+    return DSM_OK;
+}
+extern "C" int dsm_ctx_debug_big_served(dsm_ctx *c, uint64_t *items)
+{
+    if (!c || !items) { dsm_set_error("debug_big_served: null pointer"); return DSM_ERR_ARG; }
+    *items = 0;
+    if (!c->big_ctl) return DSM_OK;
+    BIND(c);
+    HIP_TRY(hipMemcpyAsync(items, c->big_ctl + 4, sizeof(uint64_t), hipMemcpyDeviceToHost, c->stream));
+    HIP_TRY(hipStreamSynchronize(c->stream));
+    return DSM_OK;
+}
+extern "C" int dsm_ctx_debug_big_skipped(dsm_ctx *c, uint64_t *iterations, uint32_t *quiet_run)
+{
+    if (!c) { dsm_set_error("debug_big_skipped: null context"); return DSM_ERR_ARG; }
+    if (iterations) *iterations = c->big_skipped;
+    if (quiet_run) *quiet_run = (c->h_big && c->big_known) ? *(volatile uint32_t *)c->h_big : 0u;
     return DSM_OK;
 }
 
@@ -840,6 +871,27 @@
     std::vector<int> nb_prev(K, 0);
     std::vector<uint32_t> ic(K);
     std::vector<const uint32_t *> u(K, nullptr);
+    const bool big_scope = !batched && fuse_s2 && (spec == 2 || spec == 3) && !lead->shard_on && !lead->timing;
+    if (!batched && fuse_s2) {
+        dsm_ctx *c = lead;
+        if (!c->big_ctl) {
+            TRY(dev_alloc(&c->big_ctl, 8));
+            HIP_TRY(hipMemsetAsync(c->big_ctl, 0, 8 * sizeof(uint32_t), c->stream));
+            HIP_TRY(hipHostMalloc((void **)&c->h_big, 4 * sizeof(uint32_t), hipHostMallocDefault));
+            memset(c->h_big, 0, 4 * sizeof(uint32_t));
+            c->big_known = true;
+        }
+        if (!c->big_known) {
+            HIP_TRY(hipMemsetAsync(c->big_ctl, 0, 2 * sizeof(uint32_t), c->stream));
+            ((volatile uint32_t *)c->h_big)[0] = 0u;
+            c->big_known = true;
+        }
+        if (big_scope && n_iter > 0) {
+            if (c->gamma_entry_len != sg) { TRY(dev_alloc(&c->gamma_entry, sg)); c->gamma_entry_len = sg; }
+            HIP_TRY(hipMemcpyAsync(c->gamma_entry, c->gamma, sg * sizeof(double), hipMemcpyDeviceToDevice, c->stream));
+        }
+    }
+    constexpr uint32_t DSM_BIG_QUIET = 16;
     TRY(ch.each([&](dsm_ctx *c, int) -> int {
         TRY(alloc_traces(c, n_iter));
         HIP_TRY(hipMemsetAsync(c->nchange, 0, sizeof(int), c->stream));
@@ -852,11 +904,15 @@
     TRY(ch.launch([&](dsm_ctx *, int k) { return words[k].prefetch(); }));
     for (int it = 0; it < n_iter; ++it) {
         if (!batched && it && (it & 63) == 0 && lead->tau_neartie_mode == -1) { TRY(k_tau_rare_count(lead, true)); TRY(k_tau_neartie_hint(lead)); }
-        TRY(ch.launch([&](dsm_ctx *c, int k) { ic[k] = c->iter_ctr++; return agg ? k_stats_stage1(c, ic[k]) : k_stats_v1(c, ic[k]); }));
+        const bool big_skip = big_scope && lead->big_launch_mode != 1 &&
+                              (lead->big_launch_mode == 2 || ((volatile uint32_t *)lead->h_big)[0] >= DSM_BIG_QUIET);
+        if (big_skip) ++lead->big_skipped;
+        TRY(ch.launch([&](dsm_ctx *c, int k) { ic[k] = c->iter_ctr++; return agg ? k_stats_stage1(c, ic[k], !big_skip) : k_stats_v1(c, ic[k]); }));
         if (agg && !fuse_s2) TRY(ch.launch([&](dsm_ctx *c, int k) { return k_stats_stage2(c, ic[k]); }));
         TRY(ch.launch([&](dsm_ctx *c, int k) {
             return k_dirichlet(c, ic[k], c->gamma, c->gamma_trace + (size_t)it * sg, c->eta_new, c->eta_trace + (size_t)it * 16,
-                               prior_slot(c, it), it - 1, nb_prev[k], prior_slot(c, it - 1), fuse_s2 ? 1 : 0);
+                               prior_slot(c, it), it - 1, nb_prev[k], prior_slot(c, it - 1), fuse_s2 ? 1 : 0, (!batched && fuse_s2) ? 1 : 0,
+                               big_skip ? 0 : 1, it ? c->gamma_trace + (size_t)(it - 1) * sg : c->gamma_entry);
         }));
         TRY(ch.launch([&](dsm_ctx *, int k) { return words[k].acquire(it, &u[k]); }));
         TRY(ch.launch([&](dsm_ctx *c, int k) {
diff --git a/desman_amd/csrc/dsm_host.h b/desman_amd/csrc/dsm_host.h
--- a/desman_amd/csrc/dsm_host.h
+++ b/desman_amd/csrc/dsm_host.h
@@ -76,6 +76,14 @@
     unsigned long long *big_list = nullptr;
     uint32_t *big_count = nullptr;
     size_t big_cap = 0;
+    size_t big_seg = 0;
+    uint32_t *big_ctl = nullptr;
+    uint32_t *h_big = nullptr;
+    double *gamma_entry = nullptr;
+    size_t gamma_entry_len = 0;
+    int big_launch_mode = 0;
+    bool big_known = false;
+    uint64_t big_skipped = 0;
     int stats_grid = 0;
     int stats_grid_key = -1;
     int item_stride = 1;
@@ -188,12 +196,13 @@
 int k_tau_rare_count(dsm_ctx *c, bool wait);
 int tau_rare_from_host(const double *gamma, int S, int G);
 int k_stats(dsm_ctx *c, uint32_t iter);
-int k_stats_stage1(dsm_ctx *c, uint32_t iter);
+int k_stats_stage1(dsm_ctx *c, uint32_t iter, bool launch_big = true);
 int k_stats_stage2(dsm_ctx *c, uint32_t iter);
 int k_binom_test(dsm_ctx *c, int kind, uint32_t n, const double *w, uint64_t seed, int nsamp, uint32_t *d_out, int spec);
 int k_esum_fold(dsm_ctx *c);
 int k_dirichlet(dsm_ctx *c, uint32_t iter, double *gamma_out, double *gamma_trace, double *eta_out, double *eta_trace,
-                double *prior_out, int fin_it, int fin_nblocks, const double *fin_prior, int do_s2 = 0);
+                double *prior_out, int fin_it, int fin_nblocks, const double *fin_prior, int do_s2 = 0,
+                int big_record = 0, int items_done = 1, const double *gamma_prev = nullptr);
 int k_prior(dsm_ctx *c, const double *gamma, const double *eta, double *prior_out);
 int k_prior_batch(dsm_ctx *c, const double *gamma, const double *eta, int n, double *prior_out);
 struct TauFinalRider { int nblocks, it; const double *prior, *gamma_src, *eta_src; };
diff --git a/desman_amd/csrc/dsm_stage2.h b/desman_amd/csrc/dsm_stage2.h
--- a/desman_amd/csrc/dsm_stage2.h
+++ b/desman_amd/csrc/dsm_stage2.h
@@ -31,6 +31,75 @@
 
 #define S2_SMEM_BYTES (DSM_LOG_TAB_N * 16 + DSM_EXP_TAB_N * 8 + DSM_RCP_TAB_N * 8 + 32 * 8 + S2_TAB_ENTRIES * 4 + 32 * 4 + 5 * S2_MAX_NODES * 4)
 
+struct BigServe {
+    int items_done;
+    int V;
+    const unsigned long long *list;
+    size_t seg;
+    const int32_t *cnt_vs;
+    const uint64_t *tau;
+    const double *eta, *gamma_prev;
+    uint32_t *ctl;
+    uint32_t *host;
+};
+#define S2_SERVE_BYTES (512 * 4 + DSM_BIG_NT * DSM_BIG_NL * 4 + 4 * 4)
+static_assert(DSM_BIG_NT * DSM_BIG_NL <= 192, "the counters are read by the first three wavefronts of a 256-thread workgroup");
+
+template <int SPEC>
+__device__ __forceinline__ bool serve_item(const BigServe &sv, unsigned long long item, int S, int G, int only, const double *gam_own,
+                                           uint32_t k0, uint32_t k1, uint32_t iter, const double *rcp, const double2 *ltab,
+                                           uint32_t (&H)[4], uint32_t (&n)[4], int &b, int &s)
+{
+    const uint32_t cell = (uint32_t)(item >> 2);
+    b = (int)(item & 3ull);
+    s = (int)(cell / (uint32_t)sv.V);
+    const int v = (int)(cell - (uint32_t)s * (uint32_t)sv.V);
+    if (s >= S || (only >= 0 && s != only)) return false;
+    const double *gam = gam_own ? gam_own : sv.gamma_prev + (size_t)s * G;
+    const uint64_t t = sv.tau[v];
+    const uint32_t xb = (uint32_t)sv.cnt_vs[((size_t)v * S + s) * 4 + b];
+    double Gam[4] = {0.0, 0.0, 0.0, 0.0};
+    H[0] = H[1] = H[2] = H[3] = 0u;
+    for (int g = 0; g < G; ++g) {
+        const int a = (int)((t >> (2 * g)) & 3);
+        const double x = gam[g];
+#pragma unroll
+        for (int k = 0; k < 4; ++k) if (a == k) { H[k] |= 1u << g; Gam[k] = Gam[k] + x; }
+    }
+    double W[4];
+#pragma unroll
+    for (int a = 0; a < 4; ++a) W[a] = sv.eta[a * 4 + b] * Gam[a];
+    const double Wt = ((W[0] + W[1]) + W[2]) + W[3];
+    if (!(Wt > 0.0)) {
+#pragma unroll
+        for (int a = 0; a < 4; ++a) W[a] = Gam[a];
+    }
+    uint32_t cbase[4];
+    philox4x32_10(cell, 0u, iter, DSM_STREAM_STA1, k0, k1, cbase);
+    Xo128 rng = item_seed<SPEC>(cbase, (uint32_t)b, k0, k1);
+    bool defer = false;
+    mult4<true, SPEC>(rng, xb, W, n, rcp, ltab, defer);
+    return true;
+}
+
+__device__ __forceinline__ void serve_counts_load(const uint32_t *big_count, uint32_t *bcnt, uint32_t *bflag, int tid, uint32_t &my_cnt)
+{
+    my_cnt = (tid < DSM_BIG_NT * DSM_BIG_NL) ? big_count[tid * DSM_BIG_STRIDE] : 0u;
+}
+__device__ __forceinline__ void serve_counts_publish(uint32_t *bcnt, uint32_t *bflag, int tid, uint32_t my_cnt)
+{
+    if (tid < DSM_BIG_NT * DSM_BIG_NL) bcnt[tid] = my_cnt;
+    const unsigned long long m = __builtin_amdgcn_ballot_w64(my_cnt != 0u);
+    if ((tid & 63) == 0) bflag[tid >> 6] = m ? 1u : 0u;
+}
+__device__ __forceinline__ void serve_counts_retire(uint32_t *big_count, uint32_t *ctl, int nwg)
+{
+    if (atomicAdd(&ctl[2], 1u) == (uint32_t)(nwg - 1)) {
+        for (int k = 0; k < DSM_BIG_NT * DSM_BIG_NL; ++k) big_count[k * DSM_BIG_STRIDE] = 0u;
+        ctl[2] = 0u;
+    }
+}
+
 #ifdef DSM_AB_SWITCHES
 __device__ unsigned long long s2_clk[1024 * 8];
 #define S2_CLK(row, k) do { if (threadIdx.x == 0 && blockIdx.y == 0 && (row) < 1024) s2_clk[(size_t)(row) * 8 + (k)] = __builtin_amdgcn_s_memrealtime(); } while (0)
@@ -38,7 +107,8 @@
 #define S2_CLK(row, k) do { } while (0)
 #endif
 template <int SPEC>
-__device__ __forceinline__ const uint32_t *stage2_sample(const Stage2Params &p, const S2Plan &pl, int s, char *smem, bool to_global, int part = 0)
+__device__ __forceinline__ const uint32_t *stage2_sample(const Stage2Params &p, const S2Plan &pl, int s, char *smem, bool to_global, int part = 0,
+                                                         const BigServe &sv = BigServe{})
 {
     const int G = p.G, tid = threadIdx.x, nthr = blockDim.x;
     double2 *ltab = reinterpret_cast<double2 *>(smem);
@@ -62,7 +132,12 @@
             pre_ok = true;
         }
     }
-    if (s == 0 && part == 0 && tid < DSM_BIG_NT * DSM_BIG_NL && p.big_count) p.big_count[tid * DSM_BIG_STRIDE] = 0u;
+    const bool serve = sv.ctl && !sv.items_done;
+    const bool look = serve || (sv.ctl && s == 0);
+    uint32_t *stab = reinterpret_cast<uint32_t *>(smem + S2_SMEM_BYTES), *bcnt = stab + 512, *bflag = bcnt + DSM_BIG_NT * DSM_BIG_NL;
+    uint32_t my_cnt = 0;
+    if (look) serve_counts_load(p.big_count, bcnt, bflag, tid, my_cnt);
+    if (!serve && s == 0 && part == 0 && tid < DSM_BIG_NT * DSM_BIG_NL && p.big_count) p.big_count[tid * DSM_BIG_STRIDE] = 0u;
     if (tid < DSM_LOG_TAB_N) ltab[tid] = reinterpret_cast<const double2 *>(p.log_tab)[tid];
     if (tid < DSM_EXP_TAB_N) etab[tid] = p.log_tab[2 * DSM_LOG_TAB_N + tid];
     for (int k = tid; k < DSM_RCP_TAB_N; k += nthr) rcp[k] = k ? 1.0 / (double)k : 0.0;
@@ -72,7 +147,44 @@
         n_child[tid] = pl.child[tid];
     }
     for (int i = tid; i < S2_TAB_ENTRIES; i += nthr) tab[i] = 0u;
+    if (look) serve_counts_publish(bcnt, bflag, tid, my_cnt);
     __syncthreads();
+    bool own_items = false;
+    if (look) {
+        const bool any = (bflag[0] | bflag[1] | bflag[2]) != 0u;
+        if (s == 0 && tid == 0) {
+            const uint32_t q = any ? 0u : sv.ctl[0] + 1u;
+            sv.ctl[0] = q;
+            if (any) sv.ctl[1] = p.iter + 1u;
+            if (sv.host) {
+                __hip_atomic_store(sv.host, q, __ATOMIC_RELAXED, __HIP_MEMORY_SCOPE_SYSTEM);
+                if (any) __hip_atomic_store(sv.host + 1, p.iter + 1u, __ATOMIC_RELAXED, __HIP_MEMORY_SCOPE_SYSTEM);
+            }
+        }
+        if (serve && any) {
+            own_items = true;
+            for (int i = tid; i < (1 << G); i += nthr) stab[i] = 0u;
+            __syncthreads();
+            unsigned long long seen = 0;
+            for (int sub = 0; sub < DSM_BIG_NT * DSM_BIG_NL; ++sub) {
+                const uint32_t nb = min(bcnt[sub], (uint32_t)sv.seg);
+                seen += nb;
+                const unsigned long long *list = sv.list + (size_t)sub * sv.seg;
+                for (uint32_t i = tid; i < nb; i += nthr) {
+                    uint32_t H[4], n4[4];
+                    int b, si;
+                    if (!serve_item<SPEC>(sv, list[i], p.S, G, s, gs, p.k0, p.k1, p.iter, rcp, ltab, H, n4, b, si)) continue;
+#pragma unroll
+                    for (int a = 0; a < 4; ++a) if (n4[a]) atomicAdd(&stab[H[a]], n4[a]);
+                }
+            }
+            if (tid == 0) {
+                if (s == 0) *reinterpret_cast<unsigned long long *>(sv.ctl + 4) += seen;
+                serve_counts_retire(p.big_count, sv.ctl, p.S + 4);
+            }
+            __syncthreads();
+        }
+    }
     S2_CLK(s, 1);
 
     const int nlev = pl.nlevels > 1 ? pl.nlevels - 1 : pl.nlevels;
@@ -107,6 +219,7 @@
                         if (m) { cell[r * cstride] = 0u; n += m; }
                     }
                 }
+                if (own_items) n += stab[Hs];
             } else n = tab[base + j];
             if (w == 1) {
                 if (level == 0) leaf[lo] = n;
diff --git a/desman_amd/csrc/kernels_gibbs.hip b/desman_amd/csrc/kernels_gibbs.hip
--- a/desman_amd/csrc/kernels_gibbs.hip
+++ b/desman_amd/csrc/kernels_gibbs.hip
@@ -566,7 +566,35 @@
     Stage2Params s2;
 };
 
-__device__ __forceinline__ void dirichlet_body(const DirParams &q, const S2Plan &plan)
+template <int SPEC>
+__device__ __forceinline__ void serve_eta_items(const BigServe &sv, const Stage2Params &p, char *smem, const uint32_t *bcnt, unsigned long long *ef, int a_own)
+{
+    const int tid = threadIdx.x;
+    double2 *ltab = reinterpret_cast<double2 *>(smem);
+    double *etab = reinterpret_cast<double *>(ltab + DSM_LOG_TAB_N);
+    double *rcp = etab + DSM_EXP_TAB_N;
+    if (tid < DSM_LOG_TAB_N) ltab[tid] = reinterpret_cast<const double2 *>(p.log_tab)[tid];
+    if (tid < DSM_EXP_TAB_N) etab[tid] = p.log_tab[2 * DSM_LOG_TAB_N + tid];
+    for (int k = tid; k < DSM_RCP_TAB_N; k += 256) rcp[k] = k ? 1.0 / (double)k : 0.0;
+    __syncthreads();
+    unsigned long long e[4] = {0ull, 0ull, 0ull, 0ull};
+    for (int sub = 0; sub < DSM_BIG_NT * DSM_BIG_NL; ++sub) {
+        const uint32_t nb = min(bcnt[sub], (uint32_t)sv.seg);
+        const unsigned long long *list = sv.list + (size_t)sub * sv.seg;
+        for (uint32_t i = tid; i < nb; i += 256) {
+            uint32_t H[4], n4[4];
+            int b, si;
+            if (!serve_item<SPEC>(sv, list[i], p.S, p.G, -1, nullptr, p.k0, p.k1, p.iter, rcp, ltab, H, n4, b, si)) continue;
+            const uint32_t m = a_own == 0 ? n4[0] : a_own == 1 ? n4[1] : a_own == 2 ? n4[2] : n4[3];
+#pragma unroll
+            for (int bb = 0; bb < 4; ++bb) if (b == bb) e[bb] += m;
+        }
+    }
+#pragma unroll
+    for (int bb = 0; bb < 4; ++bb) if (e[bb]) atomicAdd(&ef[bb], e[bb]);
+}
+
+__device__ __forceinline__ void dirichlet_body(const DirParams &q, const S2Plan &plan, const BigServe &sv = BigServe{})
 {
     unsigned long long *__restrict__ sum_mu = q.sum_mu, *__restrict__ esum = q.esum;
     const int S = q.S, G = q.G;
@@ -578,7 +606,7 @@
     const int do_fin = q.do_fin, do_s2 = q.do_s2;
     const FinalParams &fin = q.fin;
     const Stage2Params &s2 = q.s2;
-    __shared__ __attribute__((aligned(16))) char smem_d[S2_SMEM_BYTES];
+    __shared__ __attribute__((aligned(16))) char smem_d[S2_SMEM_BYTES + S2_SERVE_BYTES];
     if (do_fin && (int)blockIdx.x == S + 4) {
         double *red = reinterpret_cast<double *>(smem_d), *redp = red + 256;
         int *flag = reinterpret_cast<int *>(redp + 256);
@@ -589,16 +617,25 @@
     const bool is_gamma = row < S;
     const uint32_t *leaf = nullptr;
     if (do_s2 && is_gamma)
-        leaf = do_s2 >= 3 ? stage2_sample<3>(s2, plan, row, smem_d, false) : stage2_sample<2>(s2, plan, row, smem_d, false);
+        leaf = do_s2 >= 3 ? stage2_sample<3>(s2, plan, row, smem_d, false, 0, sv) : stage2_sample<2>(s2, plan, row, smem_d, false, 0, sv);
     if (!is_gamma) {
         static_assert(DSM_ESUM_PARTS * 4 == 256, "one thread per (copy, observed base)");
-        unsigned long long *ef = reinterpret_cast<unsigned long long *>(smem_d);
+        unsigned long long *ef = reinterpret_cast<unsigned long long *>(smem_d + S2_SMEM_BYTES);
+        uint32_t *bcnt = reinterpret_cast<uint32_t *>(smem_d + S2_SMEM_BYTES) + 512, *bflag = bcnt + DSM_BIG_NT * DSM_BIG_NL;
+        const bool serve = do_s2 && sv.ctl && !sv.items_done;
+        uint32_t my_cnt = 0;
+        if (serve) { serve_counts_load(s2.big_count, bcnt, bflag, threadIdx.x, my_cnt); serve_counts_publish(bcnt, bflag, threadIdx.x, my_cnt); }
         if (threadIdx.x < 4) ef[threadIdx.x] = 0ull;
         __syncthreads();
         const int ob = threadIdx.x & 3, k = threadIdx.x >> 2;
         unsigned long long *pp = esum + 16 + k * 16 + ob * 4 + (row - S);
         const unsigned long long v = *pp;
         if (v) { *pp = 0ull; atomicAdd(&ef[ob], v); }
+        if (serve && (bflag[0] | bflag[1] | bflag[2]) != 0u) {
+            if (do_s2 >= 3) serve_eta_items<3>(sv, s2, smem_d, bcnt, ef, row - S);
+            else serve_eta_items<2>(sv, s2, smem_d, bcnt, ef, row - S);
+            if (threadIdx.x == 0) serve_counts_retire(s2.big_count, sv.ctl, S + 4);
+        }
         __syncthreads();
     }
     S2_CLK(row, 6);
@@ -611,7 +648,7 @@
         double shape;
         uint32_t vid;
         if (is_gamma) { vid = (uint32_t)(row * G + lane); shape = alpha + (double)(sum_mu[vid] + (leaf ? (unsigned long long)leaf[lane] : 0ull)); }
-        else { const int a = row - S; vid = (uint32_t)(SG + a * 4 + lane); shape = delta + (double)(esum[lane * 4 + a] + reinterpret_cast<const unsigned long long *>(smem_d)[lane]); }
+        else { const int a = row - S; vid = (uint32_t)(SG + a * 4 + lane); shape = delta + (double)(esum[lane * 4 + a] + reinterpret_cast<const unsigned long long *>(smem_d + S2_SMEM_BYTES)[lane]); }
         y = gamma_variate(shape, vid, iter, k0, k1);
         if (zero_after) { if (is_gamma) sum_mu[row * G + lane] = 0ull; else esum[lane * 4 + (row - S)] = 0ull; }
     }
@@ -639,7 +676,7 @@
 #endif
 
 struct DirBatch { DirParams p[DSM_MAX_BATCH]; S2Plan plan; };
-__global__ __launch_bounds__(256) void dirichlet_kernel(DirParams q, S2Plan plan) { dirichlet_body(q, plan); }
+__global__ __launch_bounds__(256) void dirichlet_kernel(DirParams q, S2Plan plan, BigServe sv) { dirichlet_body(q, plan, sv); }
 __global__ __launch_bounds__(256) void dirichlet_kernel_b(DirBatch b) { dirichlet_body(b.p[blockIdx.y], b.plan); }
 static_assert(sizeof(DirBatch) <= 4096, "kernarg segment");
 
@@ -1179,7 +1216,8 @@
 }
 
 int k_dirichlet(dsm_ctx *c, uint32_t iter, double *gamma_out, double *gamma_trace, double *eta_out, double *eta_trace,
-                double *prior_out, int fin_it, int fin_nblocks, const double *fin_prior, int do_s2)
+                double *prior_out, int fin_it, int fin_nblocks, const double *fin_prior, int do_s2, int big_record, int items_done,
+                const double *gamma_prev)
 {
     KTimer tm(c, DSM_K_DIRICH);
     double lg, le;
@@ -1204,7 +1242,14 @@
     q.do_fin = do_fin; q.fin = fin; q.do_s2 = do_s2 ? stats_draw_version(stats_spec(c)) : 0; q.s2 = s2;
     if (g_batch.K == 0) {
         const S2Plan plan = do_s2 ? make_stage2_plan(c->G) : S2Plan{};
-        hipLaunchKernelGGL(dirichlet_kernel, dim3(c->S + 4 + do_fin), dim3(256), 0, c->stream, q, plan);
+        BigServe sv = {};
+        sv.items_done = 1;
+        if (do_s2 && big_record && c->big_ctl && c->big_list && c->big_count) {
+            if (!items_done && (!gamma_prev || c->shard_on || c->G > 9)) { dsm_set_error("dirichlet: items_done = 0 outside its scope"); return DSM_ERR_STATE; }
+            sv.items_done = items_done ? 1 : 0; sv.V = c->V; sv.list = c->big_list; sv.seg = c->big_seg; sv.cnt_vs = c->cnt_vs; sv.tau = c->tau;
+            sv.eta = c->eta; sv.gamma_prev = gamma_prev; sv.ctl = c->big_ctl; sv.host = c->h_big;
+        } else if (!items_done) { dsm_set_error("dirichlet: items_done = 0 outside its scope"); return DSM_ERR_STATE; }
+        hipLaunchKernelGGL(dirichlet_kernel, dim3(c->S + 4 + do_fin), dim3(256), 0, c->stream, q, plan, sv);
     } else {
         static thread_local DirBatch acc;
         acc.p[g_batch.k] = q;
diff --git a/desman_amd/csrc/kernels_stats.hip b/desman_amd/csrc/kernels_stats.hip
--- a/desman_amd/csrc/kernels_stats.hip
+++ b/desman_amd/csrc/kernels_stats.hip
@@ -601,7 +601,7 @@
     return DSM_OK;
 }
 
-int k_stats_stage1(dsm_ctx *c, uint32_t iter)
+int k_stats_stage1(dsm_ctx *c, uint32_t iter, bool launch_big)
 {
     int r = ensure_ntab(c);
     if (r != DSM_OK) return r;
@@ -643,6 +643,7 @@
     const size_t seg = (size_t)std::min<long>((long)V * S * 4, ((grid + DSM_BIG_NL - 1) / DSM_BIG_NL) * per_wg);
     r = ensure_big_list(c, seg);
     if (r != DSM_OK) return r;
+    c->big_seg = seg;
     StatsAggParams p;
     p.cnt_vs = c->cnt_vs; p.tau = c->tau; p.gamma = c->gamma; p.eta = c->eta;
     p.V = V; p.S = S; p.G = G; p.big_seg = seg;
@@ -711,6 +712,7 @@
         void *args[] = {(void *)&p};
         HIP_TRY(hipLaunchKernel(fn, dim3(grid), dim3(256), args, sh, c->stream));
     }
+    if (!launch_big) return DSM_OK;
     KTimer tm(c, DSM_K_STATSBIG);
     if (spec >= 3) hipLaunchKernelGGL(stats_big_kernel<3>, dim3(big_grid), dim3(256), 0, c->stream, p);
     else hipLaunchKernelGGL(stats_big_kernel<2>, dim3(big_grid), dim3(256), 0, c->stream, p);
diff --git a/include/desman_hip.h b/include/desman_hip.h
--- a/include/desman_hip.h
+++ b/include/desman_hip.h
@@ -65,6 +65,9 @@
 int dsm_ctx_sample_stats(dsm_ctx *ctx, uint32_t iter, uint64_t *sum_mu, uint64_t *esum);
 int dsm_ctx_stats_spec(dsm_ctx *ctx);
 int dsm_ctx_force_stats_spec(dsm_ctx *ctx, int spec);
+int dsm_ctx_set_big_launch(dsm_ctx *ctx, int mode);
+int dsm_ctx_debug_big_served(dsm_ctx *ctx, uint64_t *items);
+int dsm_ctx_debug_big_skipped(dsm_ctx *ctx, uint64_t *iterations, uint32_t *quiet_run);
 int dsm_ctx_debug_stage1(dsm_ctx *ctx, uint32_t iter, uint32_t *ntab, uint64_t *esum);
 int dsm_ctx_debug_binom(dsm_ctx *ctx, int kind, uint32_t n, const double *w4, uint64_t seed, int nsamp,
                         uint32_t *out, int spec);
```

After: 6.386 billion V*S updates/s (median of 6 runs). No clear change (+0.7%).
